# Vandermode/TFPnP

Hardware: AMD Instinct MI355X
Metric: PnP-ADMM iters/sec (and images/sec) at env_batch=48, 256x256, 30 inner iters (higher is better)
Workload: dtype f32 (v_mfma_f32_32x32x2_f32; Winograd F(2x2,3x3) on the layers with cout % 32 == 0); 1 GPU; CS-MRI ADMM 256x256 env_batch=48/GPU radial x4 sigma_n=15, 6 solver calls x 5 inner iters + PSNR reward, no early stop; global_batch=48, parallelism=single GPU

## Files before the change

### tfpnp_amd/csrc/api.hip

```cpp
#include <cstring>

#include "common.h"
#include "conv3x3.h"
#include "conv_hs.h"

namespace pnpx {

static thread_local std::string g_err;

void set_error(const char* fmt, ...) {
  char buf[1024];
  va_list ap;
  va_start(ap, fmt);
  vsnprintf(buf, sizeof(buf), fmt, ap);
  va_end(ap);
  g_err = buf;
}

int hip_fail(hipError_t e, const char* what, const char* file, int line) {
  set_error("HIP error %d (%s) at %s:%d in %s", (int)e, hipGetErrorString(e), file, line, what);
  return PNPX_ERR_HIP;
}

int ctx_scratch(pnpx_ctx* ctx, size_t bytes, void** out) {
  if (ctx->scratch.bytes < bytes) {
    PNPX_HIP(hipDeviceSynchronize());
    if (ctx->scratch.p) PNPX_HIP(hipFree(ctx->scratch.p));
    ctx->scratch = DeviceBuf();
    void* p = nullptr;
    hipError_t e = hipMalloc(&p, bytes);
    if (e != hipSuccess) {
      set_error("scratch allocation of %zu bytes failed: %s", bytes, hipGetErrorString(e));
      return PNPX_ERR_ALLOC;
    }
    ctx->scratch.p = p;
    ctx->scratch.bytes = bytes;
  }
  *out = ctx->scratch.p;
  return PNPX_OK;
}

struct LayerSpec {
  int cin, cout;
};
static void unet_layers(LayerSpec out[27]) {
  const int blocks[9][2] = {{2, 32},    {32, 64},   {64, 128}, {128, 256}, {256, 512},
                            {768, 256}, {384, 128}, {192, 64}, {96, 32}};
  for (int b = 0; b < 9; ++b)
    for (int j = 0; j < 3; ++j) out[3 * b + j] = LayerSpec{j == 0 ? blocks[b][0] : blocks[b][1], blocks[b][1]};
}

constexpr int DRUNET_MAX_SHIFT = 8;
static int drunet_rescale(pnpx_ctx* ctx) {
  PNPX_HIP(hipDeviceSynchronize());
  if (ctx->drunet.shift < DRUNET_MAX_SHIFT) ctx->drunet.shift += 4;
  else ctx->conv_mode = CONV_F32;
  *ctx->range_flag_host = 0;
  return PNPX_OK;
}

void range_guard_enter(pnpx_ctx* ctx) {
  if (!ctx->opt_range_guard || !ctx->range_flag_host) return;
  if (*static_cast<volatile unsigned*>(ctx->range_flag_host) == 0 || ctx->range_tripped) return;
  ctx->range_tripped = true;
  if (ctx->drunet.loaded && ctx->conv_mode == CONV_HS) {
    if (drunet_rescale(ctx) != PNPX_OK) ctx->conv_mode = CONV_F32;
  } else ctx->conv_mode = CONV_F32;
}

int range_guard_strict(pnpx_ctx* ctx, hipStream_t s, bool* rerun) {
  *rerun = false;
  PNPX_HIP(hipStreamSynchronize(s));
  if (*static_cast<volatile unsigned*>(ctx->range_flag_host) == 0) return PNPX_OK;
  if (ctx->conv_mode != CONV_HS || ctx->range_tripped) {
    set_error("half-split range guard: the call's result is invalid and no fallback is left (conv_mode %d)", ctx->conv_mode);
    return PNPX_ERR_RANGE;
  }
  if (ctx->drunet.loaded) PNPX_TRY(drunet_rescale(ctx));
  else {
    ctx->conv_mode = CONV_F32;
    *ctx->range_flag_host = 0;
  }
  *rerun = true;
  return PNPX_OK;
}

}

using namespace pnpx;

#define LOCK_CTX(ctx)                         \
  if (!(ctx)) {                               \
    pnpx::set_error("null context");          \
    return PNPX_ERR_ARG;                      \
  }                                           \
  std::lock_guard<std::mutex> _lk((ctx)->mu); \
  PNPX_HIP(hipSetDevice((ctx)->device))

extern "C" {

const char* pnpx_version(void) { return "pnpx 0.1 (gfx950)"; }
const char* pnpx_last_error(void) { return g_err.c_str(); }

int pnpx_ctx_create(int device, pnpx_ctx** out) {
  if (!out) {
    set_error("pnpx_ctx_create: null out");
    return PNPX_ERR_ARG;
  }
  int n = 0;
  PNPX_HIP(hipGetDeviceCount(&n));
  if (device < 0 || device >= n) {
    set_error("pnpx_ctx_create: device %d out of range (%d visible)", device, n);
    return PNPX_ERR_ARG;
  }
  PNPX_HIP(hipSetDevice(device));
  pnpx_ctx* c = new pnpx_ctx();
  c->device = device;
  void* h = nullptr;
  hipError_t e = hipHostMalloc(&h, 64, hipHostMallocMapped);
  if (e != hipSuccess) {
    delete c;
    return hip_fail(e, "hipHostMalloc(range flag)", __FILE__, __LINE__);
  }
  c->range_flag_host = static_cast<unsigned*>(h);
  *c->range_flag_host = 0;
  void* d = nullptr;
  e = hipHostGetDevicePointer(&d, h, 0);
  if (e != hipSuccess) {
    (void)hipHostFree(h);
    delete c;
    return hip_fail(e, "hipHostGetDevicePointer(range flag)", __FILE__, __LINE__);
  }
  c->range_flag_dev = static_cast<unsigned*>(d);
  *out = c;
  return PNPX_OK;
}

int pnpx_ctx_destroy(pnpx_ctx* ctx) {
  if (!ctx) return PNPX_OK;
  (void)hipSetDevice(ctx->device);
  (void)hipDeviceSynchronize();
  if (ctx->weights.p) (void)hipFree(ctx->weights.p);
  for (pnpx::UNetArena* a : {&ctx->arena, &ctx->arena_grad})
    if (a->buf.p) (void)hipFree(a->buf.p);
  policy_free(ctx);
  pnpx::critic_free(ctx);
  pnpx::drunet_free(ctx);
  pnpx::train_cache_free(ctx);
  if (ctx->scratch.p) (void)hipFree(ctx->scratch.p);
  for (auto& t : ctx->twiddle)
    if (t.second) (void)hipFree(t.second);
  for (auto e : ctx->events) (void)hipEventDestroy(e);
  if (ctx->range_flag_host) (void)hipHostFree(ctx->range_flag_host);
  for (hipStream_t st : ctx->side_streams) (void)hipStreamDestroy(st);
  for (hipEvent_t ev : ctx->ev_pool) (void)hipEventDestroy(ev);
  delete ctx;
  return PNPX_OK;
}

size_t pnpx_policy_num_params(int num_inputs, int n_det, int spi_head) {
  return policy_num_params(num_inputs, n_det, spi_head);
}

int pnpx_policy_load(pnpx_ctx* ctx, const float* params_host, size_t n_params, int num_inputs, int n_det,
                     int spi_head) {
  LOCK_CTX(ctx);
  return policy_load(ctx, params_host, n_params, num_inputs, n_det, spi_head);
}

int pnpx_policy_forward(pnpx_ctx* ctx, const float* ob, float* probs, float* det, int B, int H, int W,
                        void* stream) {
  LOCK_CTX(ctx);
  if (!ob || !probs || !det) {
    set_error("pnpx_policy_forward: null pointer");
    return PNPX_ERR_ARG;
  }
  return policy_forward(ctx, ob, probs, det, B, H, W, static_cast<hipStream_t>(stream));
}

size_t pnpx_critic_num_params(int num_inputs) {
  return (num_inputs >= 1 && num_inputs <= 64) ? critic_num_params(num_inputs) : 0;
}

int pnpx_critic_load(pnpx_ctx* ctx, const float* params_host, size_t n_params, int num_inputs) {
  LOCK_CTX(ctx);
  return critic_load(ctx, params_host, n_params, num_inputs);
}

int pnpx_critic_forward(pnpx_ctx* ctx, const float* ob, float* value, int B, int H, int W, void* stream) {
  LOCK_CTX(ctx);
  if (!ob || !value) {
    set_error("pnpx_critic_forward: null pointer");
    return PNPX_ERR_ARG;
  }
  return critic_forward(ctx, ob, value, B, H, W, static_cast<hipStream_t>(stream));
}

int pnpx_critic_backward(pnpx_ctx* ctx, const float* ob, const float* grad_value, float* grad_ob, int B, int H, int W,
                         void* stream) {
  LOCK_CTX(ctx);
  if (!ob || !grad_value || !grad_ob) {
    set_error("pnpx_critic_backward: null pointer");
    return PNPX_ERR_ARG;
  }
  return critic_backward(ctx, ob, grad_value, grad_ob, B, H, W, static_cast<hipStream_t>(stream));
}

int pnpx_ctx_reserve(pnpx_ctx* ctx, int B, int H, int W) {
  LOCK_CTX(ctx);
  if (B <= 0 || H < 16 || W < 16) {
    set_error("pnpx_ctx_reserve: need B > 0 and H, W >= 16");
    return PNPX_ERR_SHAPE;
  }
  return ctx_reserve_unet(ctx, B, H, W);
}

int pnpx_ctx_set_option(pnpx_ctx* ctx, const char* key, int value) {
  LOCK_CTX(ctx);
  auto is = [&](const char* k) { return key && !std::strcmp(key, k); };
  if (is("conv_mode") && (value == CONV_F32 || value == CONV_HS)) {
    ctx->conv_mode = value;
    return PNPX_OK;
  }
  if (is("drunet_shift") && value >= 0 && value <= 8 && (value & 3) == 0) {
    ctx->drunet.shift = value;
    return PNPX_OK;
  }
  if (is("subbatch") && value >= 0) {
    ctx->opt_subbatch = value;
    return PNPX_OK;
  }
  if (is("fuse_pool") && (value == 0 || value == 1)) {
    ctx->opt_fuse_pool = value;
    return PNPX_OK;
  }
  if (is("fuse_outc") && (value == 0 || value == 1)) {
    ctx->opt_fuse_outc = value;
    return PNPX_OK;
  }
  if (is("fuse_first") && (value == 0 || value == 1)) {
    ctx->opt_fuse_first = value;
    return PNPX_OK;
  }
  if (is("policy_s2_hs") && (value == 0 || value == 1)) {
    PNPX_HIP(hipDeviceSynchronize());
    ctx->opt_policy_s2_hs = value;
    ctx->policy.capB = ctx->policy.capH = ctx->policy.capW = 0;
    return PNPX_OK;
  }
  if (is("fold_first") && (value == 0 || value == 1)) {
    ctx->opt_fold_first = value;
    return PNPX_OK;
  }
  if (is("fft_tile") && value >= 0 && value <= 8192) {
    ctx->opt_fft_tile = value;
    return PNPX_OK;
  }
  if (is("fp32_winograd") && (value == 0 || value == 1)) {
    ctx->opt_fp32_winograd = value;
    return PNPX_OK;
  }
  if (is("fp32_chains") && value >= 0 && value <= 8) {
    ctx->opt_fp32_chains = value;
    return PNPX_OK;
  }
  if (is("fp32_fuse_up") && (value == 0 || value == 1)) {
    ctx->opt_fp32_fuse_up = value;
    return PNPX_OK;
  }
  if (is("fp32_ksplit") && value >= 0 && value <= 2) {
    ctx->opt_fp32_ksplit = value;
    return PNPX_OK;
  }
  if (is("fp32_ksplit_rule") && value >= 1 && value < 256) {
    ctx->opt_ksplit_rule = value;
    return PNPX_OK;
  }
  if (is("fp32_wino8_layers") && value >= 0 && value < (1 << 27)) {
    ctx->opt_fp32_wino8 = value;
    return PNPX_OK;
  }
  if (is("fft_fast") && (value == 0 || value == 1)) {
    ctx->opt_fft_fast = value;
    return PNPX_OK;
  }
  if (is("fft_affine") && (value == 0 || value == 1)) {
    ctx->opt_fft_affine = value;
    return PNPX_OK;
  }
  if (is("chains") && value >= 0 && value <= 8) {
    ctx->opt_chains = value;
    return PNPX_OK;
  }
  if (is("wreg") && value >= 0 && value <= 2) {
    ctx->opt_wreg = value;
    return PNPX_OK;
  }
  if (is("fuse_up") && (value >= 0 && value <= 2)) {
    ctx->opt_fuse_up = value;
    return PNPX_OK;
  }
  if (is("range_guard") && value >= 0 && value <= 2) {
    PNPX_HIP(hipDeviceSynchronize());
    ctx->opt_range_guard = value;
    ctx->range_tripped = false;
    *ctx->range_flag_host = 0;
    return PNPX_OK;
  }
  if (is("train_cache_gb") && value >= -1) {
    ctx->opt_train_cache_gb = value;
    ctx->train_alloc_failed = false;
    ctx->train_budget_bytes = 0;
    if (value == 0) pnpx::train_cache_free(ctx);
    return PNPX_OK;
  }
  if (is("train_cache_release")) {
    pnpx::train_cache_free(ctx);
    ctx->train_alloc_failed = false;
    ctx->train_budget_bytes = 0;
    return PNPX_OK;
  }
  set_error("pnpx_ctx_set_option: unknown option '%s' or bad value %d", key ? key : "(null)", value);
  return PNPX_ERR_ARG;
}

int pnpx_ctx_get_option(pnpx_ctx* ctx, const char* key, int* value) {
  LOCK_CTX(ctx);
  auto is = [&](const char* k) { return key && !std::strcmp(key, k); };
  if (!value) {
    set_error("pnpx_ctx_get_option: null value pointer");
    return PNPX_ERR_ARG;
  }
  if (is("conv_mode")) *value = ctx->conv_mode;
  else if (is("drunet_shift")) *value = ctx->drunet.shift;
  else if (is("subbatch")) *value = ctx->opt_subbatch;
  else if (is("fuse_pool")) *value = ctx->opt_fuse_pool;
  else if (is("fuse_outc")) *value = ctx->opt_fuse_outc;
  else if (is("fuse_first")) *value = ctx->opt_fuse_first;
  else if (is("fuse_up")) *value = ctx->opt_fuse_up;
  else if (is("wreg")) *value = ctx->opt_wreg;
  else if (is("chains")) *value = ctx->opt_chains;
  else if (is("fold_first")) *value = ctx->opt_fold_first;
  else if (is("policy_s2_hs")) *value = ctx->opt_policy_s2_hs;
  else if (is("fft_affine")) *value = ctx->opt_fft_affine;
  else if (is("fft_fast")) *value = ctx->opt_fft_fast;
  else if (is("fp32_winograd")) *value = ctx->opt_fp32_winograd;
  else if (is("fp32_wino8_layers")) *value = ctx->opt_fp32_wino8;
  else if (is("fp32_fuse_up")) *value = ctx->opt_fp32_fuse_up;
  else if (is("fp32_ksplit")) *value = ctx->opt_fp32_ksplit;
  else if (is("fp32_ksplit_rule")) *value = ctx->opt_ksplit_rule;
  else if (is("fp32_chains")) *value = ctx->opt_fp32_chains;
  else if (is("fft_tile")) *value = ctx->opt_fft_tile;
  else if (is("range_guard")) *value = ctx->opt_range_guard;
  else if (is("train_cache_gb")) *value = ctx->opt_train_cache_gb;
  else {
    set_error("pnpx_ctx_get_option: unknown option '%s'", key ? key : "(null)");
    return PNPX_ERR_ARG;
  }
  return PNPX_OK;
}

int pnpx_ctx_status(pnpx_ctx* ctx) {
  LOCK_CTX(ctx);
  range_guard_enter(ctx);
  if (ctx->range_tripped) {
    if (ctx->drunet.loaded)
      set_error("half-split range guard tripped: an activation of an earlier DRUNet call left the f16 hi/lo range (|v| >= 4095 "
                "or NaN); that call's output is invalid.  The context now runs %s (the bias-free network is positively "
                "homogeneous: inputs scaled by 2^-%d, the tail multiplies back; a trip at 2^-8 selects exact fp32); acknowledge "
                "with pnpx_ctx_set_option(ctx, \"range_guard\", 1)", ctx->conv_mode == CONV_HS ? "re-scaled passes" : "conv_mode 0",
                ctx->drunet.shift);
    else
    set_error("half-split range guard tripped: an activation of an earlier call left the f16 hi/lo range (|v| >= 4095 or "
              "NaN); that call's output is invalid.  The context now runs conv_mode 0 (exact fp32 MFMA); re-arm with "
              "pnpx_ctx_set_option(ctx, \"range_guard\", 1)");
    return PNPX_ERR_RANGE;
  }
  return PNPX_OK;
}

size_t pnpx_ctx_bytes(const pnpx_ctx* ctx) {
  if (!ctx) return 0;
  size_t n = ctx->weights.bytes + ctx->arena.buf.bytes + ctx->arena_grad.buf.bytes + ctx->scratch.bytes +
             ctx->drunet.weights.bytes + ctx->drunet.arena.bytes + ctx->drunet.arena_grad.bytes + ctx->drunet.f32_weights.bytes +
             ctx->drunet.f32_arena.bytes + ctx->drunet.f32_weights_bwd.bytes + ctx->drunet.f32_arena_grad.bytes +
             ctx->policy.weights.bytes + ctx->policy.arena.bytes + ctx->critic.weights.bytes + ctx->critic.arena.bytes;
  for (const auto& sl : ctx->train_ring) n += sl.arena.buf.bytes + sl.pre.bytes;
  return n;
}

size_t pnpx_unet_num_params(void) {
  LayerSpec L[27];
  unet_layers(L);
  size_t n = 0;
  for (int i = 0; i < 27; ++i) n += (size_t)L[i].cin * L[i].cout * 9 + L[i].cout;
  return n + 32 + 1;
}

size_t pnpx_drunet_num_params(int nb) { return (nb >= 1 && nb <= 8) ? pnpx::drunet_num_params(nb) : 0; }

int pnpx_drunet_load(pnpx_ctx* ctx, const float* params_host, size_t n_params, int nb) {
  LOCK_CTX(ctx);
  return pnpx::drunet_load(ctx, params_host, n_params, nb);
}

int pnpx_unet_load(pnpx_ctx* ctx, const float* params_host, size_t n_params) {
  LOCK_CTX(ctx);
  pnpx::drunet_free(ctx);
  if (!params_host || n_params != pnpx_unet_num_params()) {
    set_error("pnpx_unet_load: expected %zu parameters, got %zu", pnpx_unet_num_params(), n_params);
    return PNPX_ERR_ARG;
  }
  LayerSpec L[27];
  unet_layers(L);
  std::vector<float> host;
  size_t woff[27], boff[27];
  auto align = [&]() { host.resize((host.size() + 255) & ~(size_t)255, 0.f); };
  const float* src = params_host;
  for (int i = 0; i < 27; ++i) {
    const int mt = conv_pack_mt(L[i].cout), cc = conv_pack_cc(L[i].cin);
    align();
    woff[i] = host.size();
    host.resize(host.size() + (size_t)L[i].cin * L[i].cout * 9);
    pack_conv_weights(src, L[i].cout, L[i].cin, mt, cc, host.data() + woff[i]);
    src += (size_t)L[i].cin * L[i].cout * 9;
    align();
    boff[i] = host.size();
    host.insert(host.end(), src, src + L[i].cout);
    src += L[i].cout;
    ctx->conv[i].cin = L[i].cin;
    ctx->conv[i].cout = L[i].cout;
    ctx->conv[i].mt = mt;
    ctx->conv[i].cc = cc;
  }
  size_t uoff[27];
  {
    const float* wsrc = params_host;
    for (int i = 0; i < 27; ++i) {
      uoff[i] = 0;
      if (conv3x3_wino_packs(L[i].cout, L[i].cin)) {
        align();
        uoff[i] = host.size();
        host.resize(host.size() + conv3x3_wino_floats(L[i].cout, L[i].cin));
        pack_conv_weights_wino(wsrc, L[i].cout, L[i].cin, host.data() + uoff[i]);
      }
      wsrc += (size_t)L[i].cin * L[i].cout * 9 + L[i].cout;
    }
  }
  size_t hoff[27];
  float hscale[27];
  for (int i = 0; i < 27; ++i) {
    const int mt = conv_hs_mt(L[i].cout);
    const int cin_pad = (L[i].cin + 15) / 16 * 16;
    align();
    hoff[i] = host.size();
    const size_t n16 = (size_t)L[i].cout * cin_pad * 9 * 2;
    host.resize(host.size() + (n16 + 1) / 2, 0.f);
    const float* wsrc = params_host;
    for (int k = 0; k < i; ++k) wsrc += (size_t)L[k].cin * L[k].cout * 9 + L[k].cout;
    hscale[i] = pack_conv_weights_hs(wsrc, L[i].cout, L[i].cin, mt, reinterpret_cast<uint16_t*>(host.data() + hoff[i]));
    ctx->conv_hs[i].cin = L[i].cin;
    ctx->conv_hs[i].cout = L[i].cout;
    ctx->conv_hs[i].cin_pad = cin_pad;
    ctx->conv_hs[i].mt = mt;
    ctx->conv_hs[i].inv_scale = 1.0f / (hscale[i] * HS_ASCALE);
  }
  size_t toff[27];
  for (int i = 0; i < 27; ++i) {
    const int cout_pad = (L[i].cin + 31) / 32 * 32;
    const int mt = (cout_pad % 64 == 0) ? 64 : 32;
    align();
    toff[i] = host.size();
    host.resize(host.size() + (size_t)cout_pad * L[i].cout * 9);
    const float* wsrc = params_host;
    for (int k = 0; k < i; ++k) wsrc += (size_t)L[k].cin * L[k].cout * 9 + L[k].cout;
    pack_conv_weights_transposed(wsrc, L[i].cout, L[i].cin, cout_pad, mt, 8, host.data() + toff[i]);
    ctx->conv_bwd[i].cin = L[i].cout;
    ctx->conv_bwd[i].cout = cout_pad;
    ctx->conv_bwd[i].mt = mt;
    ctx->conv_bwd[i].cc = 8;
  }
  size_t thoff[27], tuoff[27];
  float thscale[27];
  {
    std::vector<float> wt;
    for (int i = 0; i < 27; ++i) {
      const int cin_t = L[i].cout;
      const int cout_t = (L[i].cin + 31) / 32 * 32;
      const int mt = (cout_t % 64 == 0) ? 64 : 32;
      const float* wsrc = params_host;
      for (int k = 0; k < i; ++k) wsrc += (size_t)L[k].cin * L[k].cout * 9 + L[k].cout;
      wt.assign((size_t)cout_t * cin_t * 9, 0.f);
      for (int ci = 0; ci < L[i].cin; ++ci)
        for (int co = 0; co < cin_t; ++co)
          for (int tap = 0; tap < 9; ++tap)
            wt[((size_t)ci * cin_t + co) * 9 + tap] = wsrc[((size_t)co * L[i].cin + ci) * 9 + (8 - tap)];
      align();
      thoff[i] = host.size();
      const size_t n16 = (size_t)cout_t * cin_t * 9 * 2;
      host.resize(host.size() + (n16 + 1) / 2, 0.f);
      thscale[i] = pack_conv_weights_hs(wt.data(), cout_t, cin_t, mt, reinterpret_cast<uint16_t*>(host.data() + thoff[i]));
      tuoff[i] = 0;
      if (conv3x3_wino_packs(cout_t, cin_t)) {
        align();
        tuoff[i] = host.size();
        host.resize(host.size() + conv3x3_wino_floats(cout_t, cin_t));
        pack_conv_weights_wino(wt.data(), cout_t, cin_t, host.data() + tuoff[i]);
      }
      ctx->conv_hs_bwd[i].cin = cin_t;
      ctx->conv_hs_bwd[i].cout = cout_t;
      ctx->conv_hs_bwd[i].cin_pad = cin_t;
      ctx->conv_hs_bwd[i].mt = mt;
      ctx->conv_hs_bwd[i].inv_scale = 1.0f / (thscale[i] * HS_ASCALE);
    }
  }
  align();
  const size_t oc0 = host.size();
  host.insert(host.end(), params_host, params_host + 32 * 2 * 9);
  align();
  const size_t ozero = host.size();
  host.resize(host.size() + 768, 0.f);
  align();
  const size_t ow = host.size();
  host.insert(host.end(), src, src + 32);
  src += 32;
  align();
  const size_t ob = host.size();
  host.push_back(*src);
  host.resize(host.size() + 1024, 0.f);
  PNPX_HIP(hipDeviceSynchronize());
  if (ctx->weights.p) PNPX_HIP(hipFree(ctx->weights.p));
  ctx->weights = DeviceBuf();
  ctx->has_weights = false;
  void* p = nullptr;
  hipError_t e = hipMalloc(&p, host.size() * sizeof(float));
  if (e != hipSuccess) {
    set_error("weight allocation of %zu bytes failed: %s", host.size() * sizeof(float), hipGetErrorString(e));
    return PNPX_ERR_ALLOC;
  }
  PNPX_HIP(hipMemcpy(p, host.data(), host.size() * sizeof(float), hipMemcpyHostToDevice));
  float* d = static_cast<float*>(p);
  for (int i = 0; i < 27; ++i) {
    ctx->conv[i].w = d + woff[i];
    ctx->conv[i].b = d + boff[i];
    ctx->conv_wino_u[i] = uoff[i] ? d + uoff[i] : nullptr;
    ctx->conv_wino_u_bwd[i] = tuoff[i] ? d + tuoff[i] : nullptr;
    ctx->conv_hs[i].w = reinterpret_cast<char*>(d + hoff[i]);
    ctx->conv_bwd[i].w = d + toff[i];
    ctx->conv_bwd[i].b = nullptr;
    ctx->conv_hs_bwd[i].w = reinterpret_cast<char*>(d + thoff[i]);
  }
  ctx->conv0_w = d + oc0;
  ctx->zero_bias = d + ozero;
  ctx->outc_w = d + ow;
  ctx->outc_b = d + ob;
  ctx->weights.p = p;
  ctx->weights.bytes = host.size() * sizeof(float);
  ctx->has_weights = true;
  pnpx::train_cache_free(ctx);
  return PNPX_OK;
}

int pnpx_unet_denoise(pnpx_ctx* ctx, const float* x, const float* sigma, float* out, float* out_preclamp, int B,
                      int H, int W, void* stream) {
  LOCK_CTX(ctx);
  return pnpx::guarded(ctx, static_cast<hipStream_t>(stream), [&]() -> int {
  if (!x || !sigma || !out) {
    set_error("pnpx_unet_denoise: null pointer");
    return PNPX_ERR_ARG;
  }
  return unet_denoise(ctx, x, sigma, 1, out, out_preclamp, B, H, W, static_cast<hipStream_t>(stream), nullptr);
  });
}

int pnpx_unet_denoise_backward(pnpx_ctx* ctx, const float* x, const float* sigma, const float* grad_out, float* grad_x,
                               float* grad_sigma, int B, int H, int W, void* stream) {
  LOCK_CTX(ctx);
  return pnpx::guarded(ctx, static_cast<hipStream_t>(stream), [&]() -> int {
  if (!x || !sigma || !grad_out || !grad_x || !grad_sigma) {
    set_error("pnpx_unet_denoise_backward: null pointer");
    return PNPX_ERR_ARG;
  }
  return unet_denoise_backward(ctx, x, sigma, 1, grad_out, grad_x, grad_sigma, B, H, W, static_cast<hipStream_t>(stream));
  });
}

int pnpx_unet_denoise_train(pnpx_ctx* ctx, const float* x, const float* sigma, float* out, int B, int H, int W,
                            unsigned long long* ticket, void* stream) {
  LOCK_CTX(ctx);
  return pnpx::guarded(ctx, static_cast<hipStream_t>(stream), [&]() -> int {
    if (!x || !sigma || !out || !ticket) {
      set_error("pnpx_unet_denoise_train: null pointer");
      return PNPX_ERR_ARG;
    }
    return unet_denoise_train(ctx, x, sigma, 1, out, B, H, W, static_cast<hipStream_t>(stream), ticket);
  });
}

int pnpx_unet_denoise_backward_ticket(pnpx_ctx* ctx, const float* x, const float* sigma, const float* grad_out,
                                      float* grad_x, float* grad_sigma, int B, int H, int W, unsigned long long ticket,
                                      void* stream) {
  LOCK_CTX(ctx);
  return pnpx::guarded(ctx, static_cast<hipStream_t>(stream), [&]() -> int {
    if (!x || !sigma || !grad_out || !grad_x || !grad_sigma) {
      set_error("pnpx_unet_denoise_backward_ticket: null pointer");
      return PNPX_ERR_ARG;
    }
    return unet_denoise_backward_ticket(ctx, x, sigma, 1, grad_out, grad_x, grad_sigma, B, H, W,
                                        static_cast<hipStream_t>(stream), ticket);
  });
}

int pnpx_unet_profile(pnpx_ctx* ctx, const float* x, const float* sigma, float* out, int B, int H, int W,
                      void* stream, int cap, float* ms_out, double* flops_out, const char** names_out, int* n_out) {
  LOCK_CTX(ctx);
  if (!x || !sigma || !out || !ms_out || !flops_out || !names_out || !n_out || cap <= 0) {
    set_error("pnpx_unet_profile: null pointer");
    return PNPX_ERR_ARG;
  }
  hipStream_t s = static_cast<hipStream_t>(stream);
  PNPX_TRY(unet_denoise(ctx, x, sigma, 1, out, nullptr, B, H, W, s, nullptr));
  while (ctx->events.size() < 1024) {
    hipEvent_t e;
    PNPX_HIP(hipEventCreate(&e));
    ctx->events.push_back(e);
  }
  ProfileSink sink;
  sink.events = &ctx->events;
  PNPX_TRY(unet_denoise(ctx, x, sigma, 1, out, nullptr, B, H, W, s, &sink));
  PNPX_HIP(hipStreamSynchronize(s));
  int n = sink.n < cap ? sink.n : cap;
  for (int i = 0; i < n; ++i) {
    float ms = 0.f;
    PNPX_HIP(hipEventElapsedTime(&ms, ctx->events[i], ctx->events[i + 1]));
    ms_out[i] = ms;
    flops_out[i] = sink.flops[i];
    names_out[i] = sink.names[i];
  }
  *n_out = n;
  return PNPX_OK;
}

int pnpx_fft2(pnpx_ctx* ctx, const float* in, float* out, int n_img, int H, int W, int inverse, int centered,
              void* stream) {
  LOCK_CTX(ctx);
  if (!in || !out) {
    set_error("pnpx_fft2: null pointer");
    return PNPX_ERR_ARG;
  }
  return fft2(ctx, in, out, n_img, H, W, inverse != 0, centered != 0, static_cast<hipStream_t>(stream));
}
// ... 3 lines not shown
```

### tfpnp_amd/csrc/common.h

```cpp
#pragma once
#include <hip/hip_runtime.h>

#include <cstdarg>
#include <cstdint>
#include <cstdio>
#include <map>
#include <mutex>
#include <string>
#include <vector>

#include "pnpx.h"

namespace pnpx {

void set_error(const char* fmt, ...);
int hip_fail(hipError_t e, const char* what, const char* file, int line);

#define PNPX_HIP(expr)                                                       \
  do {                                                                       \
    hipError_t _e = (expr);                                                  \
    if (_e != hipSuccess) return ::pnpx::hip_fail(_e, #expr, __FILE__, __LINE__); \
  } while (0)
#define PNPX_TRY(expr)          \
  do {                          \
    int _s = (expr);            \
    if (_s != PNPX_OK) return _s; \
  } while (0)
#define PNPX_LAUNCH_CHECK() PNPX_HIP(hipGetLastError())

constexpr int PADL = 4;
__host__ __device__ inline int padded_w(int W) { return W + 2 * PADL; }
__host__ __device__ inline int padded_h(int H) { return H + 2; }

struct ActDesc {
  size_t off = 0;
  int C = 0, H = 0, W = 0;
  size_t per_image() const { return (size_t)C * padded_h(H) * padded_w(W); }
};

struct ConvLayer {
  int cin = 0, cout = 0;
  int mt = 0, cc = 0;
  float* w = nullptr;
  float* b = nullptr;
};

struct DeviceBuf {
  void* p = nullptr;
  size_t bytes = 0;
};

struct UNetArena {
  DeviceBuf buf;
  int capB = 0, capH = 0, capW = 0, mode = -1;
};

struct ConvLayerHsDev {
  int cin = 0, cout = 0, cin_pad = 0, mt = 0;
  char* w = nullptr;
  float inv_scale = 1.f;
};

enum ConvMode { CONV_F32 = 0, CONV_HS = 1 };

struct PolStep;
struct PolicyConv {
  const float* w = nullptr;
  const float* bias = nullptr;
  const PolStep* steps = nullptr;
  const int* nsteps = nullptr;
  int cin = 0;
  int cout = 0;
  int split_c = 0;
};
struct PolicyNet {
  bool loaded = false;
  int num_inputs = 0, cin_pad = 0, n_det = 0, spi_head = 0;
  PolicyConv conv[17];
  ConvLayerHsDev conv_hs[12];
  const float* bias_hs[12] = {};
  ConvLayerHsDev s2_hs[4][2];
  const float* s2_bias[4][2] = {};
  ConvLayerHsDev stem_hs;
  const float* stem_hs_bias = nullptr;
  const float* fc_sm_w = nullptr;
  const float* fc_sm_b = nullptr;
  const float* fc_det_w = nullptr;
  const float* fc_det_b = nullptr;
  const float* fc_det2_w = nullptr;
  const float* fc_det2_b = nullptr;
  DeviceBuf weights;
  DeviceBuf arena;
  int capB = 0, capH = 0, capW = 0;
};

struct CriticNet {
  bool loaded = false;
  int num_inputs = 0, cin_pad = 0;
  ConvLayerHsDev fwd[21], bwd[21];
  const float* bias[21] = {};
  float alpha[21] = {};
  const float* fc_w = nullptr;
  const float* fc_b = nullptr;
  const float* zero = nullptr;
  float fc_wmax = 0.f;
  DeviceBuf weights, arena;
  int capB = 0, capH = 0, capW = 0;
};

int launch_chains(const pnpx_ctx* ctx, int B, int H, int W);
void join_side_streams_after_failure(pnpx_ctx* ctx);
struct DruNet {
  bool loaded = false;
  int nb = 0;
  std::vector<ConvLayerHsDev> layers;
  std::vector<int> taps;
  const float* head_w = nullptr;
  const float* zero = nullptr;
  const float* e0 = nullptr;
  int shift = 0;
  std::vector<ConvLayerHsDev> layers_bwd;
  const float* tail_bwd_w = nullptr;
  DeviceBuf weights, arena, arena_grad;
  std::vector<float> params_host;
  bool f32_ready = false;
  std::vector<ConvLayer> f32_layers;
  std::vector<const float*> f32_wino;
  DeviceBuf f32_weights, f32_arena;
  int f32_capB = 0, f32_capH = 0, f32_capW = 0;
  bool f32_arena_keeps = false;
  bool f32_bwd_ready = false;
  std::vector<ConvLayer> f32_layers_bwd;
  std::vector<const float*> f32_wino_bwd;
  DeviceBuf f32_weights_bwd, f32_arena_grad;
  int f32_gcapB = 0, f32_gcapH = 0, f32_gcapW = 0;
  int capB = 0, capH = 0, capW = 0;
  bool arena_keeps = false;
  int gcapB = 0, gcapH = 0, gcapW = 0;
};

}

struct pnpx_ctx {
  int device = 0;
  std::mutex mu;
  bool has_weights = false;
  pnpx::ConvLayer conv[27];
  pnpx::ConvLayerHsDev conv_hs[27];
  int conv_mode = pnpx::CONV_F32;
  int opt_subbatch = 24;
  int opt_fuse_pool = 1;
  int opt_fuse_outc = 1;
  int opt_fuse_first = 1;
  int opt_fuse_up = 1;
  int opt_policy_s2_hs = 1;
  int opt_fold_first = 0;
  int opt_fft_tile = 0;
  int opt_fft_fast = 1;
  int opt_fft_affine = 1;
  int opt_chains = 0;
  std::vector<hipStream_t> side_streams;
  std::vector<hipEvent_t> ev_pool;
  size_t ev_next = 0;
  int opt_wreg = 2;
  int opt_range_guard = 1;
  int opt_train_cache_gb = -1;
  size_t train_budget_bytes = 0;
  unsigned* range_flag_host = nullptr;
  unsigned* range_flag_dev = nullptr;
  bool range_tripped = false;
  float* conv_wino_u[27] = {};
  float* conv_wino_u_bwd[27] = {};
  int opt_fp32_winograd = 1;
  int opt_fp32_wino8 = (1 << 27) - 1;
  int opt_fp32_chains = 2;
  int opt_fp32_ksplit = 1;
  int opt_ksplit_rule = 1;
  int opt_fp32_fuse_up = 1;
  pnpx::ConvLayer conv_bwd[27];
  pnpx::ConvLayerHsDev conv_hs_bwd[27];
  float* zero_bias = nullptr;
  float* conv0_w = nullptr;
  float* outc_w = nullptr;
  float* outc_b = nullptr;
  pnpx::DeviceBuf weights;
  pnpx::UNetArena arena, arena_grad;
  struct TrainSlot {
    pnpx::UNetArena arena;
    pnpx::DeviceBuf pre;
    unsigned long long ticket = 0;
    int B = 0;
  };
  std::vector<TrainSlot> train_ring;
  unsigned long long train_counter = 0;
  int train_H = 0, train_W = 0, train_mode = -1;
  bool train_alloc_failed = false;
  pnpx::PolicyNet policy;
  pnpx::CriticNet critic;
  pnpx::DruNet drunet;
  pnpx::DeviceBuf scratch;
  std::map<int, float2*> twiddle;
  std::vector<hipEvent_t> events;
};

namespace pnpx {

int chain_event(pnpx_ctx* ctx, hipEvent_t* ev);
int chain_streams(pnpx_ctx* ctx, int chains);
template <class F>
int fan_out_chains(pnpx_ctx* ctx, int chains, int B, hipStream_t s, F&& run_slice) {
  PNPX_TRY(chain_streams(ctx, chains));
  hipEvent_t fork = nullptr, joins[16] = {};
  PNPX_TRY(chain_event(ctx, &fork));
  PNPX_HIP(hipEventRecord(fork, s));
  auto fail = [&](int rc) {
    join_side_streams_after_failure(ctx);
    return rc;
  };
  auto hip = [&](hipError_t e, const char* what) { return e == hipSuccess ? PNPX_OK : hip_fail(e, what, __FILE__, __LINE__); };
  for (int c = chains - 1; c >= 0; --c) {
    const int lo = (int)((long long)B * c / chains), hi = (int)((long long)B * (c + 1) / chains);
    hipStream_t st = c ? ctx->side_streams[c - 1] : s;
    int rc = c ? hip(hipStreamWaitEvent(st, fork, 0), "hipStreamWaitEvent(fork)") : PNPX_OK;
    if (rc == PNPX_OK) rc = run_slice(lo, hi, st);
    if (rc == PNPX_OK && c) rc = chain_event(ctx, &joins[c]);
    if (rc == PNPX_OK && c) rc = hip(hipEventRecord(joins[c], st), "hipEventRecord(join)");
    if (rc != PNPX_OK) return fail(rc);
  }
  for (int c = 1; c < chains; ++c) {
    const int rc = hip(hipStreamWaitEvent(s, joins[c], 0), "hipStreamWaitEvent(join)");
    if (rc != PNPX_OK) return fail(rc);
  }
  return PNPX_OK;
}

int ctx_reserve_unet(pnpx_ctx* ctx, int B, int H, int W);
int reserve_arena(pnpx_ctx* ctx, UNetArena& ar, int mode, int B, int H, int W, size_t extra_bytes);
int ctx_scratch(pnpx_ctx* ctx, size_t bytes, void** out);
int ctx_twiddle(pnpx_ctx* ctx, int N, const float2** out);
void range_guard_enter(pnpx_ctx* ctx);
int range_guard_strict(pnpx_ctx* ctx, hipStream_t s, bool* rerun);
template <class F>
int guarded(pnpx_ctx* ctx, hipStream_t s, F&& body) {
  range_guard_enter(ctx);
  int st = body();
  for (int attempt = 0; attempt < 4 && st == PNPX_OK && ctx->opt_range_guard == 2 && ctx->conv_mode == CONV_HS; ++attempt) {
    bool rerun = false;
    PNPX_TRY(range_guard_strict(ctx, s, &rerun));
    if (!rerun) break;
    st = body();
  }
  return st;
}

struct ProfileSink {
  std::vector<hipEvent_t>* events = nullptr;
  std::vector<const char*> names;
  std::vector<double> flops;
  int n = 0;
};

int unet_denoise(pnpx_ctx* ctx, const float* x, const float* sigma, int sigma_stride, float* out, float* out_pre,
                 int B, int H, int W, hipStream_t s, ProfileSink* prof, UNetArena* arena = nullptr, int mode = -1,
                 bool keep_all = false);
int unet_denoise_backward(pnpx_ctx* ctx, const float* x, const float* sigma, int sigma_stride, const float* grad_out,
                          float* grad_x, float* grad_sigma, int B, int H, int W, hipStream_t s,
                          UNetArena* cached = nullptr, const float* cached_pre = nullptr);
size_t unet_arena_bytes(int mode, int B, int H, int W);
void train_cache_free(pnpx_ctx* ctx);
int unet_denoise_train(pnpx_ctx* ctx, const float* x, const float* sigma, int sigma_stride, float* out, int B, int H,
                       int W, hipStream_t s, unsigned long long* ticket);
int unet_denoise_backward_ticket(pnpx_ctx* ctx, const float* x, const float* sigma, int sigma_stride,
                                 const float* grad_out, float* grad_x, float* grad_sigma, int B, int H, int W,
                                 hipStream_t s, unsigned long long ticket);

size_t drunet_num_params(int nb);
int drunet_load(pnpx_ctx* ctx, const float* params, size_t n, int nb);
int drunet_denoise(pnpx_ctx* ctx, const float* x, const float* sigma, int sigma_stride, float* out, float* out_pre, int B,
                   int H, int W, hipStream_t s, bool keep_mids = false);
int drunet_denoise_backward(pnpx_ctx* ctx, const float* x, const float* sigma, int sigma_stride, const float* grad_out,
                            float* grad_x, float* grad_sigma, int B, int H, int W, hipStream_t s);
void drunet_free(pnpx_ctx* ctx);
int drunet_denoise_f32(pnpx_ctx* ctx, const float* x, const float* sigma, int sigma_stride, float* out, float* out_pre, int B, int H,
                       int W, hipStream_t s, bool keep_mids = false);
int drunet_denoise_backward_f32(pnpx_ctx* ctx, const float* x, const float* sigma, int sigma_stride, const float* grad_out, float* grad_x,
                                float* grad_sigma, int B, int H, int W, hipStream_t s);
void drunet_f32_free(pnpx_ctx* ctx);

size_t policy_num_params(int num_inputs, int n_det, int spi_head);
int policy_load(pnpx_ctx* ctx, const float* params, size_t n, int num_inputs, int n_det, int spi_head);
int policy_forward(pnpx_ctx* ctx, const float* ob, float* probs, float* det, int B, int H, int W, hipStream_t s);
void policy_free(pnpx_ctx* ctx);

size_t critic_num_params(int num_inputs);
int critic_load(pnpx_ctx* ctx, const float* params, size_t n, int num_inputs);
int critic_forward(pnpx_ctx* ctx, const float* ob, float* value, int B, int H, int W, hipStream_t s);
int critic_backward(pnpx_ctx* ctx, const float* ob, const float* grad_value, float* grad_ob, int B, int H, int W, hipStream_t s);
void critic_free(pnpx_ctx* ctx);

int fft2(pnpx_ctx* ctx, const float* in, float* out, int n_img, int H, int W, bool inverse, bool centered,
         hipStream_t s);

}
```

### tfpnp_amd/csrc/conv3x3.h

```cpp
#pragma once
#include "common.h"

namespace pnpx {

struct ConvArgs {
  const float* in0;
  const float* in1;
  const float* wpk;
  const float* bias;
  float* out;
  int C0, C1;
  int H, W, Hp, Wp;
  int tilesX, tilesY, nct;
  float slope;
  int mode;
  const float* dmask;
  const char* dmask_hs = nullptr;
  const float* res = nullptr;
};

int conv_pack_mt(int cout);
int conv_pack_cc(int cin);
void pack_conv_weights(const float* w, int cout, int cin, int mt, int cc, float* dst);
int launch_conv3x3(const ConvLayer& L, const float* in0, int C0, const float* in1, int C1, float* out, int B,
                   int H, int W, hipStream_t s);
int launch_conv3x3_act(const ConvLayer& L, const float* in0, int C0, const float* in1, int C1, float* out, int B,
                       int H, int W, float slope, const float* res, hipStream_t s);
int launch_conv1x1_act(const ConvLayer& L, const float* in0, float* out, int B, int H, int W, float slope, const float* res, hipStream_t s);
void pack_conv_weights_1x1(const float* w, int cout, int cin, float* dst);
int launch_conv3x3_grad(const ConvLayer& L, const float* gin, float* gout, const float* dmask, int B, int H, int W,
                        hipStream_t s, const char* dmask_hs = nullptr, float mask_slope = 0.2f);
bool conv3x3_wino_ok(int C0, int C1, int cout, int H, int W);
bool conv3x3_wino_packs(int cout, int cin);
size_t conv3x3_wino_floats(int cout, int cin);
void pack_conv_weights_wino(const float* w, int cout, int cin, float* dst);
int launch_conv3x3_wino(const float* u, const float* bias, int cout, const float* in0, int C0, const float* in1, int C1,
                        float* out, int B, int H, int W, hipStream_t s, float slope = 0.2f, const float* res = nullptr,
                        float* pool_out = nullptr);
bool conv3x3_wino_outc_ok(int cin, int cout, int H, int W);
int launch_conv3x3_wino_outc(const float* u, const float* bias, const float* in0, int cin, const float* outc_w, const float* outc_b,
                             const float* x_img, float* img, float* img_pre, int B, int H, int W, hipStream_t s);
bool conv3x3_wino8_ok(int C0, int C1, int cout, int H, int W);
int launch_conv3x3_wino8(const float* u, const float* bias, int cout, const float* in0, int C0, const float* in1, int C1,
                         float* out, int B, int H, int W, hipStream_t s, float slope = 0.2f, const float* res = nullptr,
                         float* pool_out = nullptr, float* ks_part = nullptr, int ks_rule = 1);
int conv3x3_wino8_ksplit(int C0, int C1, int cout, int H, int W, int rule = 1);
size_t conv3x3_wino8_ksplit_bytes_per_image();
int launch_conv3x3_wino8_grad(const float* u, const float* zero_bias, int cout, const float* gin, int cin, float* gout, const float* dmask,
                              float mask_slope, int B, int H, int W, hipStream_t s);
bool conv3x3_wino8_ups_ok(int C0, int C1, int cout, int H, int W);
int launch_conv3x3_wino8_ups(const float* u, const float* bias, int cout, const float* in0, int C0, const float* in1_lowres, int C1,
                             float* out, int B, int H, int W, hipStream_t s, float slope = 0.2f);
int launch_conv3x3_wino8_outc(const float* u, const float* bias, const float* in0, int cin, const float* outc_w, const float* outc_b,
                              const float* x_img, float* img, float* img_pre, int B, int H, int W, hipStream_t s);
void pack_conv_weights_transposed(const float* w, int cout, int cin, int cout_pad, int mt, int cc, float* dst);

}
```

### tfpnp_amd/csrc/conv3x3_wino8.hip

```cpp
#include <cmath>
#include <utility>
#include <vector>

#include "common.h"
#include "conv3x3.h"
#include "wino_common.h"

namespace pnpx {

namespace {

using namespace wino;

template <int CT_>
struct Cfg8 {
  static constexpr int CT = CT_;
  static constexpr int CK = (CT == 64) ? 16 : 8;
  static constexpr int HALVES = CK / 8;
  static constexpr int KS = CK / 2;
  static constexpr int RS = (CT == 64) ? 1 : 2;
  static constexpr int NSTG = 4 / RS;
  static constexpr int NPOS = 2 * RS;
  static constexpr int NM = NPOS * KS;
  static_assert(NM == 16, "the side-work schedule below is written for 16 MFMA slots per stage");
  static constexpr int RPXW = (CT == 64) ? 16 : 32;
  static constexpr int TX = RPXW / 2, NT = 8 * TX;
  static constexpr int RW = RPXW + 2, RPX = 18 * RW;
  static constexpr int RPXL = (CT == 64) ? 328 : RPX;
  static constexpr int RAW_ELEMS = CK * RPXL;
  static constexpr int RAW_INSTR = (RAW_ELEMS + 63) / 64;
  static constexpr int RAW_BYTES = RAW_INSTR * 256;
  static constexpr int RAW_PER_WAVE = (RAW_INSTR + 7) / 8;
  static constexpr int NRAW = RAW_INSTR / 8;
  static constexpr int UQ = 16 * CK * CT;
  static constexpr int USTG = RS * UQ;
  static constexpr int NUW = USTG / 8192;
  static constexpr int VROW = 16384;
  static constexpr int VSTG = RS * VROW;
  static constexpr int OFF_U = 0, OFF_V = 4 * USTG, OFF_RAW = OFF_V + 2 * VSTG;
  static constexpr int LDS_USED = OFF_RAW + 2 * RAW_BYTES;
  static constexpr int BAR = 12;
  static constexpr int NR = 11, NQP = (CT == 64) ? 12 : 20;
  static constexpr int QPLANE = NR * NQP * 16;
  static constexpr int ST_ELEMS = CK * NR * NQP;
  static constexpr int ST_INSTR = (ST_ELEMS + 63) / 64;
  static constexpr int ST_STRIDE = ST_INSTR * 256;
  static constexpr int ST_PER_WAVE = (ST_INSTR + 7) / 8, NSW = ST_INSTR / 8;
  static constexpr int OFF_ST = LDS_USED, OFF_TAB = OFF_ST + 2 * ST_STRIDE;
  static constexpr int LDS_USED_UPS = OFF_TAB + (18 + RW) * 16;
  static constexpr int NPOSI = 18 * RW;
};
constexpr int LDS_REQ8 = 160 * 1024;

#define WINO8_ACC \
  "a0", "a1", "a2", "a3", "a4", "a5", "a6", "a7", "a8", "a9", "a10", "a11", "a12", "a13", "a14", "a15", "a16", "a17", \
  "a18", "a19", "a20", "a21", "a22", "a23", "a24", "a25", "a26", "a27", "a28", "a29", "a30", "a31", "a32", "a33", \
  "a34", "a35", "a36", "a37", "a38", "a39", "a40", "a41", "a42", "a43", "a44", "a45", "a46", "a47", "a48", "a49", \
  "a50", "a51", "a52", "a53", "a54", "a55", "a56", "a57", "a58", "a59", "a60", "a61", "a62", "a63", "a64", "a65", \
  "a66", "a67", "a68", "a69", "a70", "a71", "a72", "a73", "a74", "a75", "a76", "a77", "a78", "a79", "a80", "a81", \
  "a82", "a83", "a84", "a85", "a86", "a87", "a88", "a89", "a90", "a91", "a92", "a93", "a94", "a95", "a96", "a97", \
  "a98", "a99", "a100", "a101", "a102", "a103", "a104", "a105", "a106", "a107", "a108", "a109", "a110", "a111", "a112", \
  "a113", "a114", "a115", "a116", "a117", "a118", "a119", "a120", "a121", "a122", "a123", "a124", "a125", "a126", "a127"
#ifdef WINO8_PRIO
#define WINO8_PRIO_UP "s_setprio 3\n\t"
#define WINO8_PRIO_DOWN "\n\ts_setprio 0"
#else
#define WINO8_PRIO_UP
#define WINO8_PRIO_DOWN
#endif
#define WINO8_MFMA(IDX, x, y) \
  asm volatile(WINO8_PRIO_UP "v_mfma_f32_32x32x2_f32 a[%2:%3], %0, %1, a[%2:%3]" WINO8_PRIO_DOWN ::"v"(x), "v"(y), "n"(16 * (IDX)), "n"(16 * (IDX) + 15) : WINO8_ACC)
#define WINO8_MFMA_FROM_ZERO(IDX, x, y) \
  asm volatile(WINO8_PRIO_UP "v_mfma_f32_32x32x2_f32 a[%2:%3], %0, %1, 0" WINO8_PRIO_DOWN ::"v"(x), "v"(y), "n"(16 * (IDX)), "n"(16 * (IDX) + 15) : WINO8_ACC)

#ifndef WINO8_ABL
#define WINO8_ABL 0
#endif
#ifdef WINO8_TRACE
__device__ unsigned long long wino8_trace_buf[2][2048];
__device__ __forceinline__ void wino8_stamp(int wave, int lane, int& n, int tag) {
  if (blockIdx.x == 0 && (wave & 3) == 0 && n < 2047) {
    const unsigned long long t = __builtin_readcyclecounter();
    if (lane == 0) wino8_trace_buf[wave >> 2][n] = (t << 8) | (unsigned)tag;
    n = __builtin_amdgcn_readfirstlane(n + 1);
    if (lane == 0) wino8_trace_buf[wave >> 2][2047] = n;
  }
}
#define WINO8_STAMP(tag) wino8_stamp(wave, lane, trace_n, tag)
#else
#define WINO8_STAMP(tag)
#endif

template <bool RAWDMA_, bool STDMA_, int IQ_>
struct StageKind {
  static constexpr bool RAWDMA = RAWDMA_, STDMA = STDMA_;
  static constexpr int IQ = IQ_;
};

using I0 = std::integral_constant<int, 0>;
using I1 = std::integral_constant<int, 1>;
using I2 = std::integral_constant<int, 2>;
using I3 = std::integral_constant<int, 3>;
using Yes = std::true_type;
using No = std::false_type;

template <int CT, bool FUSE_OUTC, bool RES, bool UPS, bool KSPLIT>
__global__ __launch_bounds__(512, 1) void conv3x3_wino8_f32_kernel(WinoArgs a) {
  static_assert(!FUSE_OUTC || CT == 32, "the fused out-conv needs all 32 couts of a pixel in one SIMD's wave pair");
  static_assert(!UPS || (!FUSE_OUTC && !RES), "the up-sampling instances are the UNet's plain decoder entries");
  static_assert(!KSPLIT || (CT == 64 && !FUSE_OUTC && !RES && !UPS), "K-split: the plain 64-cout instance (the deep levels' layers)");
  using C = Cfg8<CT>;
  constexpr int CK = C::CK, HALVES = C::HALVES, KS = C::KS, RS = C::RS, NSTG = C::NSTG, NPOS = C::NPOS;
  constexpr int TX = C::TX, NT = C::NT, RW = C::RW, RPX = C::RPX, RPXL = C::RPXL;
  constexpr int RAW_BYTES = C::RAW_BYTES, RAW_PER_WAVE = C::RAW_PER_WAVE;
  constexpr int UQ = C::UQ, USTG = C::USTG, NUW = C::NUW, VROW = C::VROW, VSTG = C::VSTG;
  constexpr int OFF_U = C::OFF_U, OFF_V = C::OFF_V, OFF_RAW = C::OFF_RAW, BAR = C::BAR;
  extern __shared__ __attribute__((aligned(16))) char lds[];
  const int tid = threadIdx.x, lane = tid & 63;
  const int wave = __builtin_amdgcn_readfirstlane(tid >> 6);
#ifdef WINO8_TRACE
  int trace_n = 0;
#endif
  const int sw = wave & 3;
  const int HpWp = a.Hp * a.Wp;
  const unsigned lds0 = (unsigned)(size_t)(lptr_t)lds;
  const int nregions = a.rx * a.ry * a.B;
  const int nx = (gridDim.x % 8 == 0 && nregions >= 32) ? 8 : 1;
  const int xcd = blockIdx.x % nx, slot = blockIdx.x / nx, nslot = gridDim.x / nx;

  struct Tile {
    int ct, b, x0, y0;
    const float* s0;
    const float* s1;
    const float* w;
    const float* s1u;
    int ok, rlo;
    int clo, c0;
    int item, g;
  };
  const int hpwp_lo = UPS ? (a.ups_h + 2) * (a.ups_w + 2 * PADL) : 0;
  auto decode = [&](int k) {
    Tile T;
    const int j = slot + nslot * k;
    const int vnct = KSPLIT ? a.nct * a.ksplit : a.nct;
    const int q = j / vnct;
    const int v = j - q * vnct;
    T.g = KSPLIT ? v / a.nct : 0;
    T.ct = KSPLIT ? v - T.g * a.nct : v;
    T.c0 = KSPLIT ? T.g * a.nch : 0;
    const int reg = nx * q + xcd;
    T.ok = reg < nregions;
    T.item = reg * a.nct + T.ct;
    T.rlo = T.clo = 0;
    T.s1u = nullptr;
    const int t1 = reg / a.rx;
    const int tx = reg - t1 * a.rx;
    const int t2 = t1 / a.ry;
    const int ty = t1 - t2 * a.ry;
    T.b = t2;
    T.x0 = tx * C::RPXW;
    T.y0 = ty * 16;
    const size_t pix = (size_t)T.y0 * a.Wp + T.x0 + (PADL - 1);
    T.s0 = a.in0 + (size_t)T.b * a.C0 * HpWp + pix;
    T.s1 = a.in1 + ((long long)T.b * a.C1 - a.C0) * (long long)HpWp + (long long)pix;
    T.w = a.u + ((size_t)T.ct * (KSPLIT ? a.nch_all : a.nch) + T.c0) * 4 * (UQ / 4);
    if (UPS) {
      const int ya = T.y0 > 0 ? T.y0 - 1 : 0, xa = T.x0 > 0 ? T.x0 - 1 : 0;
      const int rl = (int)(a.ups_sy * (float)ya), cl = (int)(a.ups_sx * (float)xa);
      const int rmax = a.ups_h + 1 - C::NR, cmax = a.ups_w + PADL - C::NQP;
      T.rlo = rl < rmax ? rl : rmax;
      T.clo = cl < cmax ? cl : cmax;
      T.s1u = a.in1 + ((long long)T.b * a.C1 - a.C0) * (long long)hpwp_lo + (long long)(T.rlo + 1) * (a.ups_w + 2 * PADL) + T.clo + PADL;
    }
    return T;
  };
  auto raw_of = [&](const Tile& X, int c) {
    const int ca = KSPLIT ? c + X.c0 : c;
    return ((CK * ca < a.C0) ? X.s0 : X.s1) + (size_t)CK * ca * HpWp;
  };

  const int wm = (CT == 64) ? (sw & 1) : 0, wn = (CT == 64) ? (sw >> 1) : sw;
  const int l31 = lane & 31, kg = lane >> 5;
  const int a_lane = ((kg * HALVES) * CT + wm * 32 + l31) * 16;
  const int b_lane = ((kg * HALVES) * NT + wn * 32 + l31) * 16;
  asm volatile("" ::: WINO8_ACC);

  auto wait_lds = [&]() { asm volatile("s_waitcnt lgkmcnt(0)" ::: "memory"); };
  auto barrier = [&]() { __builtin_amdgcn_s_barrier(); };
  auto sync_all = [&]() {
    asm volatile("s_waitcnt vmcnt(0) lgkmcnt(0)" ::: "memory");
    __builtin_amdgcn_s_barrier();
  };

  auto body = [&](auto role_tag) {
    constexpr int P = decltype(role_tag)::value;

    unsigned roff[RAW_PER_WAVE];
#pragma unroll
    for (int k = 0; k < RAW_PER_WAVE; ++k) {
      const int idx = (wave + 8 * k) * 64 + lane;
      const int c = idx / RPXL, r = idx - c * RPXL;
      const int hy = r / RW, hx = r - hy * RW;
      roff[k] = (c < CK && r < RPX) ? 4u * (unsigned)(c * HpWp + hy * a.Wp + hx) : 0u;
    }
    const unsigned uoff = lane * 16u;
    auto dma_u = [&](const float* src, int uslot) {
      if (WINO8_ABL & 4) return;
      const float* s = src + wave * 256;
#pragma unroll
      for (int k = 0; k < NUW; ++k) glds16(s + k * 2048, uoff, lds0 + OFF_U + uslot * USTG + (wave + 8 * k) * 1024);
    };
    auto dma_raw = [&](const float* src, int rbuf, int k0, int k1) {
      if (WINO8_ABL & 4) return;
      const unsigned dst = lds0 + OFF_RAW + rbuf * RAW_BYTES + wave * 256;
#pragma unroll
      for (int k = k0; k < k1; ++k)
        if (k < RAW_PER_WAVE) {
          if (k < C::NRAW || wave + 8 * k < C::RAW_INSTR) glds4(src, roff[k], dst + k * 2048);
        }
    };

    constexpr int NR = C::NR, NQP = C::NQP, QPLANE = C::QPLANE, ST_STRIDE = C::ST_STRIDE, SPW = C::ST_PER_WAVE;
    constexpr int OFF_ST = C::OFF_ST, OFF_TAB = C::OFF_TAB, NPOSI = C::NPOSI;
    unsigned soff[UPS ? SPW : 1];
    if (UPS) {
      const int wp_lo = a.ups_w + 2 * PADL;
#pragma unroll
      for (int k = 0; k < SPW; ++k) {
        const int idx = (wave + 8 * k) * 64 + lane;
        const int e = idx & 3, g = idx >> 2;
        const int q = g % NQP, g2 = g / NQP;
        const int rr = g2 % NR, Q = g2 / NR;
        soff[k] = (Q < CK / 4) ? 4u * (unsigned)((4 * Q + e) * hpwp_lo + rr * wp_lo + q) : 0u;
      }
    }
    auto dma_st = [&](const float* src, int sbuf) {
      if (!UPS || (WINO8_ABL & 4)) return;
      const unsigned dst = lds0 + OFF_ST + sbuf * ST_STRIDE + wave * 256;
#pragma unroll
      for (int k = 0; k < SPW; ++k)
        if (k < C::NSW || wave + 8 * k < C::ST_INSTR) glds4(src, soff[UPS ? k : 0], dst + k * 2048);
    };
    auto write_tables = [&](const Tile& X) {
      if (!UPS) return;
      if (tid < 18 + RW) {
        const bool row = tid < 18;
        const int i = row ? tid : tid - 18;
        const int g = (row ? X.y0 : X.x0) - 1 + i;
        const bool valid = g >= 0 && g < (row ? a.H : a.W);
        const float f = (row ? a.ups_sy : a.ups_sx) * (float)g;
        const int i0 = (int)f;
        const float l = f - (float)i0, h = 1.f - l;
        const int off = row ? (i0 - X.rlo) * NQP * 16 : (i0 - X.clo) * 16;
        f32x4 ent;
        ent[0] = __int_as_float(valid ? off : 0);
        ent[1] = valid ? h : 0.f;
        ent[2] = valid ? l : 0.f;
        ent[3] = 0.f;
        *reinterpret_cast<f32x4*>(lds + OFF_TAB + tid * 16) = ent;
      }
    };
    struct Ip {
      float hy, ly, hx, lx;
      int base;
      f32x4 v00, v01, v10, v11;
    };
    const int ipos = tid < NPOSI ? tid : NPOSI - 1;
    const int ipos_b = (512 + (tid >> 2) < NPOSI) ? 512 + (tid >> 2) : NPOSI - 1;
    auto interp_tables = [&](int pp, Ip& ip) {
      const int hyi = pp / RW, hxi = pp - hyi * RW;
      const f32x4 rt = *reinterpret_cast<const f32x4*>(lds + OFF_TAB + hyi * 16);
      const f32x4 ct = *reinterpret_cast<const f32x4*>(lds + OFF_TAB + (18 + hxi) * 16);
      ip.hy = rt[1];
      ip.ly = rt[2];
      ip.hx = ct[1];
      ip.lx = ct[2];
      ip.base = __float_as_int(rt[0]) + __float_as_int(ct[0]);
    };
    auto interp_slice = [&](auto q_tag, int sl, Ip& ip, int sbuf, int rbuf) {
      constexpr int Q = decltype(q_tag)::value;
      if (sl == 0) {
        interp_tables(ipos, ip);
      } else if (sl == 1) {
        const char* b = lds + OFF_ST + sbuf * ST_STRIDE + Q * QPLANE + ip.base;
        ip.v00 = *reinterpret_cast<const f32x4*>(b);
        ip.v01 = *reinterpret_cast<const f32x4*>(b + 16);
        ip.v10 = *reinterpret_cast<const f32x4*>(b + NQP * 16);
        ip.v11 = *reinterpret_cast<const f32x4*>(b + NQP * 16 + 16);
      } else {
        const int e = sl - 2;
        const float o = ip.hy * (ip.hx * ip.v00[e] + ip.lx * ip.v01[e]) + ip.ly * (ip.hx * ip.v10[e] + ip.lx * ip.v11[e]);
        *reinterpret_cast<float*>(lds + OFF_RAW + rbuf * RAW_BYTES + ((4 * Q + e) * RPXL + ipos) * 4) = o;
      }
    };
    auto interp_mini = [&](auto q_tag, int sl, Ip& ip, int sbuf, int rbuf) {
      constexpr int Q = decltype(q_tag)::value;
      const int e4 = (tid & 3) * 4;
      if (sl == 0) {
        interp_tables(ipos_b, ip);
      } else if (sl == 1) {
        const char* b = lds + OFF_ST + sbuf * ST_STRIDE + Q * QPLANE + ip.base + e4;
        ip.v00[0] = *reinterpret_cast<const float*>(b);
        ip.v01[0] = *reinterpret_cast<const float*>(b + 16);
        ip.v10[0] = *reinterpret_cast<const float*>(b + NQP * 16);
        ip.v11[0] = *reinterpret_cast<const float*>(b + NQP * 16 + 16);
      } else {
        const float o = ip.hy * (ip.hx * ip.v00[0] + ip.lx * ip.v01[0]) + ip.ly * (ip.hx * ip.v10[0] + ip.lx * ip.v11[0]);
        *reinterpret_cast<float*>(lds + OFF_RAW + rbuf * RAW_BYTES + (4 * Q * RPXL + ipos_b) * 4 + e4 * RPXL) = o;
      }
    };

    constexpr int TCH = (CT == 64) ? 2 : 4;
    const int cb = (CT == 64) ? (lane & 1) : 0;
    const int tt = (CT == 64) ? ((wave >> 2) * 32 + (lane >> 1)) : ((sw & 1) * 64 + lane);
    const int tkg = (CT == 64) ? (sw & 1) : (sw >> 1), thf = (CT == 64) ? (sw >> 1) : 0;
    const int tty = tt / TX, ttx = tt % TX;
    const int t_rd = (((tkg * (CK / 2) + thf * 4 + 2 * cb) * RPXL) + (2 * tty) * RW + 2 * ttx) * 4;
    const int t_wr = (((tkg * HALVES + thf) * NT) + tt) * 16 + cb * 8;
    struct Tr {
      float d[2][TCH][4];
      float r[4][TCH];
    };
    constexpr int NSL = 3 * TCH;
    auto transform_slice = [&](auto ta_tag, int sl, Tr& t, int rbuf, int vdst) {
      constexpr int A = decltype(ta_tag)::value;
      constexpr int RA = (A == 0) ? 0 : (A == 2 ? 2 : 1);
      constexpr int RB = (A == 0) ? 2 : (A == 1 ? 2 : (A == 2 ? 1 : 3));
      if (sl < TCH) {
        const int e = sl;
        const char* rb = lds + OFF_RAW + rbuf * RAW_BYTES + t_rd;
#pragma unroll
        for (int x = 0; x < 4; x += 2) {
          const f32x2 da = *reinterpret_cast<const f32x2*>(rb + (e * RPXL + RA * RW + x) * 4);
          const f32x2 db = *reinterpret_cast<const f32x2*>(rb + (e * RPXL + RB * RW + x) * 4);
          t.d[0][e][x] = da[0];
          t.d[0][e][x + 1] = da[1];
          t.d[1][e][x] = db[0];
          t.d[1][e][x + 1] = db[1];
        }
      } else if (sl < 2 * TCH) {
        const int e = sl - TCH;
#pragma unroll
        for (int x = 0; x < 4; ++x)
          t.r[x][e] = (A == 1) ? t.d[0][e][x] + t.d[1][e][x] : t.d[0][e][x] - t.d[1][e][x];
      } else if (CT == 64) {
        const int bb = (sl - 2 * TCH) >> 1, e = (sl - 2 * TCH) & 1;
        (void)e;
        if (((sl - 2 * TCH) & 1) == 0) return;
        f32x2 v;
#pragma unroll
        for (int q = 0; q < 2; ++q)
          v[q] = (bb == 0) ? t.r[0][q] - t.r[2][q] : (bb == 1) ? t.r[1][q] + t.r[2][q] : (bb == 2) ? t.r[2][q] - t.r[1][q] : t.r[1][q] - t.r[3][q];
        *reinterpret_cast<f32x2*>(lds + vdst + t_wr + bb * 4096) = v;
      } else {
        const int bb = sl - 2 * TCH;
        f32x4 v;
#pragma unroll
        for (int e = 0; e < 4; ++e)
          v[e] = (bb == 0) ? t.r[0][e] - t.r[2][e] : (bb == 1) ? t.r[1][e] + t.r[2][e] : (bb == 2) ? t.r[2][e] - t.r[1][e] : t.r[1][e] - t.r[3][e];
        *reinterpret_cast<f32x4*>(lds + vdst + t_wr + bb * 4096) = v;
      }
    };
    constexpr int NSLT = (CT == 64) ? 2 * TCH + 8 : NSL;
    auto vdst_of = [&](auto sn_tag) {
      constexpr int SN = decltype(sn_tag)::value;
      return OFF_V + ((CT == 64) ? (SN & 1) * VSTG : SN * VSTG + P * VROW);
    };

    f32x4 af[NPOS][HALVES], bf[NPOS][HALVES];
    auto read_operand = [&](auto s_tag, int uslot, int pos, int h) {
      constexpr int S = decltype(s_tag)::value;
      constexpr int VB = (CT == 64) ? (S & 1) : S;
      const int r = pos >> 1, b = 2 * P + (pos & 1);
      if (WINO8_ABL & 2) {
        af[pos][h] = bf[pos][h] = (f32x4){1.f, 1.f, 1.f, 1.f};
        return;
      }
      af[pos][h] = *reinterpret_cast<const f32x4*>(lds + OFF_U + uslot * USTG + r * UQ + b * (UQ / 4) + a_lane + h * (CT * 16));
      bf[pos][h] = *reinterpret_cast<const f32x4*>(lds + OFF_V + VB * VSTG + r * VROW + b * 4096 + b_lane + h * (NT * 16));
    };

    struct Side {
      int t_rbuf;
      int u_cur, u_next;
      const float* u_src;
      int u_dst;
      const float* raw_src;
      int raw_buf;
      const float* st_src;
      int st_buf;
      int i_sbuf, i_rbuf;
    };
    auto stage = [&](auto s_tag, auto zero_tag, auto wait_tag, auto prefetch_tag, auto kind_tag, const Side& sd) {
      using K = decltype(kind_tag);
      constexpr int S = decltype(s_tag)::value;
      constexpr bool PREFETCH = decltype(prefetch_tag)::value;
      constexpr int SN = (S + 1) % NSTG;
      constexpr bool ZERO = decltype(zero_tag)::value;
      constexpr int WAITN = decltype(wait_tag)::value;
      constexpr bool HALOST = (CT == 64) ? (S == 0) : (S == 1);
      constexpr bool RAWST = HALOST && K::RAWDMA;
      constexpr bool STST = UPS && HALOST && K::STDMA;
      constexpr int IQ = UPS ? K::IQ : -1;
      using IQt = std::integral_constant<int, IQ < 0 ? 0 : IQ>;
      Ip ipa, ipb;
      auto islice = [&](int q) {
        if (IQ >= 0) interp_slice(IQt{}, q, ipa, sd.i_sbuf, sd.i_rbuf);
      };
      auto imini = [&](int q) {
        if (IQ >= 0 && CT == 32) interp_mini(IQt{}, q, ipb, sd.i_sbuf, sd.i_rbuf);
      };
      using TA = std::integral_constant<int, (CT == 64) ? SN : 2 * SN + P>;
      using SNt = std::integral_constant<int, SN>;
      Tr t;
      auto operand = [&](int pos, int h) { read_operand(s_tag, sd.u_cur, pos, h); };
      auto tslice = [&](int q) {
        if (!(WINO8_ABL & 1)) transform_slice(TA{}, q, t, sd.t_rbuf, vdst_of(SNt{}));
      };
      auto side = [&](int sl) {
        if (CT == 64) {
          if (sl == 0) operand(0, 1);
          else if (sl == 1) operand(1, 1);
          if (sl < 2) tslice(sl);
          if (sl == 2) dma_u(sd.u_src, sd.u_dst);
          if (RAWST && sl >= 3 && sl < 9) dma_raw(sd.raw_src, sd.raw_buf, 2 * (sl - 3), 2 * (sl - 3) + 2);
          if (STST && sl == 9) dma_st(sd.st_src, sd.st_buf);
          if (IQ < 0) {
            if (sl == 4) tslice(2);
            if (sl == 5) tslice(3);
            if (sl >= 6 && sl < 10) tslice(5 + 2 * (sl - 6));
          } else {
            if (sl == 3) tslice(2), tslice(3);
            if (sl == 4) tslice(5), tslice(7);
            if (sl == 5) tslice(9), tslice(11), islice(0);
            if (sl == 6) islice(1);
            if (sl >= 8 && sl < 12) islice(2 + (sl - 8));
          }
        } else {
          if (sl == 0) tslice(0);
          else if (sl == 1) operand(2, 0);
          else if (sl == 2) tslice(1);
          else if (sl == 3) operand(3, 0);
          else if (sl == 4) tslice(4), tslice(2);
          else if (sl == 5) tslice(5), tslice(3);
          else if (sl == 6) tslice(6), tslice(7);
          else if (sl == 7) tslice(8), tslice(9), islice(0);
          else if (sl == 8) tslice(10), tslice(11), islice(1);
          else if (sl == 9) islice(2), islice(3), imini(0);
          else if (sl == 10) islice(4), islice(5), imini(1), dma_u(sd.u_src, sd.u_dst);
          else if (sl == 11) imini(2);
          if (RAWST && sl >= 6 && sl < 11) dma_raw(sd.raw_src, sd.raw_buf, 2 * (sl - 6), 2 * (sl - 6) + 2);
          if (STST && sl == 9) dma_st(sd.st_src, sd.st_buf);
        }
        if (sl == BAR) {
          if (!(WINO8_ABL & 8)) {
            WINO8_STAMP(32 + S);
            asm volatile("s_waitcnt vmcnt(%0) lgkmcnt(0)" ::"n"(WAITN) : "memory");
            WINO8_STAMP(48 + S);
            barrier();
          }
          WINO8_STAMP(S);
          if (PREFETCH) {
            read_operand(SNt{}, sd.u_next, 0, 0);
            read_operand(SNt{}, sd.u_next, 1, 0);
          }
        }
      };
#pragma unroll
      for (int pair = 0; pair < NPOS / 2; ++pair)
#pragma unroll
        for (int m = 0; m < KS; ++m)
#pragma unroll
          for (int bl = 0; bl < 2; ++bl) {
            const int pos = 2 * pair + bl;
            const int sl = pair * (2 * KS) + m * 2 + bl;
            const float x = af[pos][m >> 2][m & 3], y = bf[pos][m >> 2][m & 3];
            const bool from_zero = ZERO && m == 0;
            if (!(WINO8_ABL & 16)) switch (pos) {
              case 0: if (from_zero) WINO8_MFMA_FROM_ZERO(2 * (RS * S) + 0, x, y); else WINO8_MFMA(2 * (RS * S) + 0, x, y); break;
              case 1: if (from_zero) WINO8_MFMA_FROM_ZERO(2 * (RS * S) + 1, x, y); else WINO8_MFMA(2 * (RS * S) + 1, x, y); break;
              case 2: if (from_zero) WINO8_MFMA_FROM_ZERO((2 * (RS * S) + 2) & 7, x, y); else WINO8_MFMA((2 * (RS * S) + 2) & 7, x, y); break;
              default: if (from_zero) WINO8_MFMA_FROM_ZERO((2 * (RS * S) + 3) & 7, x, y); else WINO8_MFMA((2 * (RS * S) + 3) & 7, x, y); break;
            }
            side(sl);
            __builtin_amdgcn_sched_barrier(0);
          }
    };

    auto epilogue = [&](const Tile& T, int xsend, int xrecv, int zoff) {
      const int tile = wn * 32 + l31, ty = tile / TX, tx = tile % TX;
      const int cbase = T.ct * CT + wm * 32 + 4 * kg;
      float* ob = a.out + ((size_t)T.b * a.Cout) * HpWp + (size_t)(T.y0 + 2 * ty + 1) * a.Wp + T.x0 + 2 * tx + PADL;
      const int Hp_pool = padded_h(a.H / 2), Wp_pool = padded_w(a.W / 2);
      const size_t HpWp_pool = (size_t)Hp_pool * Wp_pool;
      float* pb = a.pool ? a.pool + (size_t)T.b * a.Cout * HpWp_pool + (size_t)(T.y0 / 2 + ty + 1) * Wp_pool + T.x0 / 2 + tx + PADL : nullptr;
      constexpr int R0 = 8 * P;
      constexpr int RX = 8 - R0;
      WINO8_STAMP(16);
      asm volatile("s_nop 15\n\ts_nop 15" ::: "memory", WINO8_ACC);
      float bias_r[8];
#pragma unroll
      for (int j = 0; j < 8; ++j) bias_r[j] = a.bias[cbase + ((R0 + j) & 3) + 8 * ((R0 + j) >> 2)];
      auto column_sums = [&](auto r_tag) {
        constexpr int R = decltype(r_tag)::value;
        f32x4 sv;
        static_for<2>([&](auto bl_tag) {
          constexpr int BL = decltype(bl_tag)::value;
          float m0, m1, m2, m3;
          asm volatile("v_accvgpr_read_b32 %0, a[%1]" : "=v"(m0) : "n"(16 * (0 + BL) + R) : WINO8_ACC);
          asm volatile("v_accvgpr_read_b32 %0, a[%1]" : "=v"(m1) : "n"(16 * (2 + BL) + R) : WINO8_ACC);
          asm volatile("v_accvgpr_read_b32 %0, a[%1]" : "=v"(m2) : "n"(16 * (4 + BL) + R) : WINO8_ACC);
          asm volatile("v_accvgpr_read_b32 %0, a[%1]" : "=v"(m3) : "n"(16 * (6 + BL) + R) : WINO8_ACC);
          sv[BL] = (m0 + m1) + m2;
          sv[2 + BL] = (m1 - m2) - m3;
        });
        return sv;
      };
      f32x4 theirs[8];
      {
        char* xs = lds + xsend + lane * 16;
        static_for<8>([&](auto j_tag) {
          *reinterpret_cast<f32x4*>(xs + decltype(j_tag)::value * 1024) = column_sums(std::integral_constant<int, RX + decltype(j_tag)::value>{});
        });
        wait_lds();
        barrier();
        WINO8_STAMP(17);
        const char* xr = lds + xrecv + lane * 16;
#pragma unroll
        for (int j = 0; j < 8; ++j) theirs[j] = *reinterpret_cast<const f32x4*>(xr + j * 1024);
      }
      f32x2 rs0[RES ? 4 : 1], rs1[RES ? 4 : 1];
      auto load_res = [&](int j0) {
        const float* rb = a.res + (ob - a.out);
#pragma unroll
        for (int q = 0; q < 4; ++q) {
          const float* rp = rb + (size_t)(cbase + ((R0 + j0 + q) & 3) + 8 * ((R0 + j0 + q) >> 2)) * HpWp;
          rs0[RES ? q : 0] = *reinterpret_cast<const f32x2*>(rp);
          rs1[RES ? q : 0] = *reinterpret_cast<const f32x2*>(rp + a.Wp);
        }
      };
      float ow[8];
      float s00 = 0.f, s01 = 0.f, s10 = 0.f, s11 = 0.f;
      if (FUSE_OUTC) {
#pragma unroll
        for (int j = 0; j < 8; ++j) ow[j] = a.outc_w[cbase + ((R0 + j) & 3) + 8 * ((R0 + j) >> 2)];
      }
      wait_lds();
      float* const part_tile = KSPLIT ? a.part + ((size_t)T.item * a.ksplit * 8 + wave) * 2048 + lane * 4 : nullptr;
      float* const part_mine = KSPLIT ? part_tile + (size_t)T.g * (8 * 2048) : nullptr;
      static_for<8>([&](auto j_tag) {
        constexpr int j = decltype(j_tag)::value;
        constexpr int R = R0 + j;
        if (RES && (j & 3) == 0) load_res(j);
        const int co = cbase + (R & 3) + 8 * (R >> 2);
        const f32x4 mine = column_sums(std::integral_constant<int, R>{});
        const f32x4 lo = (P == 0) ? mine : theirs[j], hi = (P == 0) ? theirs[j] : mine;
        const float bias = bias_r[j];
        float y00 = (lo[0] + lo[1]) + hi[0], y01 = (lo[1] - hi[0]) - hi[1];
        float y10 = (lo[2] + lo[3]) + hi[2], y11 = (lo[3] - hi[2]) - hi[3];
        if (KSPLIT) {
          *reinterpret_cast<f32x4*>(part_mine + j * 256) = (f32x4){y00, y01, y10, y11};
          return;
        }
        y00 += bias;
        y01 += bias;
        y10 += bias;
        y11 += bias;
        y00 = fmaxf(y00, y00 * a.slope);
        y01 = fmaxf(y01, y01 * a.slope);
        y10 = fmaxf(y10, y10 * a.slope);
        y11 = fmaxf(y11, y11 * a.slope);
        if (RES) {
          const f32x2 r0 = rs0[RES ? (j & 3) : 0], r1 = rs1[RES ? (j & 3) : 0];
          if (a.res_mask) {
            y00 *= r0[0] > 0.f ? 1.f : a.mask_slope;
            y01 *= r0[1] > 0.f ? 1.f : a.mask_slope;
            y10 *= r1[0] > 0.f ? 1.f : a.mask_slope;
            y11 *= r1[1] > 0.f ? 1.f : a.mask_slope;
          } else {
            y00 += r0[0];
            y01 += r0[1];
            y10 += r1[0];
            y11 += r1[1];
          }
        }
        if (FUSE_OUTC) {
          s00 = fmaf(ow[j], y00, s00);
          s01 = fmaf(ow[j], y01, s01);
          s10 = fmaf(ow[j], y10, s10);
          s11 = fmaf(ow[j], y11, s11);
        } else {
          float* o = ob + (size_t)co * HpWp;
          *reinterpret_cast<f32x2*>(o) = (f32x2){y00, y01};
          *reinterpret_cast<f32x2*>(o + a.Wp) = (f32x2){y10, y11};
          if (a.pool) pb[(size_t)co * HpWp_pool] = fmaxf(fmaxf(y00, y01), fmaxf(y10, y11));
        }
      });
      WINO8_STAMP(19);
      if (FUSE_OUTC) {
        s00 += __shfl_xor(s00, 32);
        s01 += __shfl_xor(s01, 32);
        s10 += __shfl_xor(s10, 32);
        s11 += __shfl_xor(s11, 32);
        char* zb = lds + zoff + lane * 16;
        if (P == 1) {
          *reinterpret_cast<f32x4*>(zb) = (f32x4){s00, s01, s10, s11};
          wait_lds();
        }
        barrier();
        f32x4 o = {0.f, 0.f, 0.f, 0.f};
        if (P == 0) {
          o = *reinterpret_cast<const f32x4*>(zb);
          wait_lds();
        }
        barrier();
        if (P == 0) {
          s00 += o[0];
          s01 += o[1];
          s10 += o[2];
          s11 += o[3];
          const size_t px0 = ((size_t)T.b * a.H + T.y0 + 2 * ty) * a.W + T.x0 + 2 * tx;
          const float ob0 = a.outc_b[0];
          const f32x2 xi0 = *reinterpret_cast<const f32x2*>(a.x_img + px0), xi1 = *reinterpret_cast<const f32x2*>(a.x_img + px0 + a.W);
          const float v00 = xi0[0] + (s00 + ob0), v01 = xi0[1] + (s01 + ob0), v10 = xi1[0] + (s10 + ob0), v11 = xi1[1] + (s11 + ob0);
          *reinterpret_cast<f32x2*>(a.img_pre + px0) = (f32x2){v00, v01};
          *reinterpret_cast<f32x2*>(a.img_pre + px0 + a.W) = (f32x2){v10, v11};
          *reinterpret_cast<f32x2*>(a.img + px0) = (f32x2){fminf(fmaxf(v00, 0.f), 1.f), fminf(fmaxf(v01, 0.f), 1.f)};
          *reinterpret_cast<f32x2*>(a.img + px0 + a.W) = (f32x2){fminf(fmaxf(v10, 0.f), 1.f), fminf(fmaxf(v11, 0.f), 1.f)};
        }
      } else {
        barrier();
      }
      WINO8_STAMP(20);
    };

    constexpr int NST = KSPLIT ? 8 : (FUSE_OUTC ? (P == 0 ? 4 : 0) : 16);
    constexpr int NRAW = C::NRAW;

    int k = 0;
    Tile T = decode(0);
    if (!T.ok) return;
    WINO8_STAMP(14);
    if (CT == 64) {
      dma_raw(raw_of(T, 0), 0, 0, RAW_PER_WAVE);
      dma_u(T.w, 0);
      dma_u(T.w + (UQ / 4), 1);
      dma_u(T.w + 2 * (UQ / 4), 2);
    } else {
      dma_raw(T.s0, 0, 0, RAW_PER_WAVE);
      dma_raw(raw_of(T, 1), 1, 0, RAW_PER_WAVE);
      dma_u(T.w, 0);
      dma_u(T.w + (USTG / 4), 1);
      dma_u(T.w + 2 * (USTG / 4), 2);
    }
    sync_all();
    {
      Tr t;
#pragma unroll
      for (int sl = 0; sl < NSLT; ++sl) transform_slice(std::integral_constant<int, (CT == 64) ? 0 : P>{}, sl, t, 0, vdst_of(I0{}));
    }
    sync_all();
    WINO8_STAMP(15);
    read_operand(I0{}, 0, 0, 0);
    read_operand(I0{}, 0, 1, 0);

    auto chunk = [&](auto first_tag, auto k1_tag, auto k2_tag, auto k3_tag, const float* w_c, const float* nu, const float* nu2,
                     const float* nraw, const float* nst, int cc) {
      constexpr int EPI = decltype(first_tag)::value ? NST : 0;
      constexpr bool K1 = UPS && decltype(k1_tag)::value, K2 = UPS && decltype(k2_tag)::value, K3 = UPS && decltype(k3_tag)::value;
      constexpr int NSW = C::NSW;
      using Pre = Yes;
      const int rcur = cc & 1, rnext = rcur ^ 1;
      if constexpr (CT == 64) {
        using S0k = StageKind<!K1, K2, K1 ? 1 : -1>;
        using S1k = StageKind<false, false, K1 ? 2 : -1>;
        using S2k = StageKind<false, false, K1 ? 3 : -1>;
        using S3k = StageKind<false, false, K2 ? 0 : -1>;
        constexpr int HALO = (K1 ? 0 : NRAW) + (K2 ? NSW : 0);
        stage(I0{}, first_tag, std::integral_constant<int, NUW + EPI + NUW + HALO>{}, Yes{}, S0k{},
              Side{rcur, 0, 1, w_c + 3 * (UQ / 4), 3, nraw, rnext, nst, rcur, rnext, rnext});
        stage(I1{}, first_tag, std::integral_constant<int, EPI + NUW + HALO + NUW>{}, Yes{}, S1k{},
              Side{rcur, 1, 2, nu, 0, nullptr, 0, nullptr, 0, rnext, rnext});
        stage(I2{}, first_tag, std::integral_constant<int, 2 * NUW>{}, Yes{}, S2k{}, Side{rcur, 2, 3, nu + (UQ / 4), 1, nullptr, 0, nullptr, 0, rnext, rnext});
        stage(I3{}, first_tag, std::integral_constant<int, 2 * NUW>{}, Pre{}, S3k{}, Side{rnext, 3, 0, nu + 2 * (UQ / 4), 2, nullptr, 0, nullptr, 0, rcur, rcur});
      } else {
        using S0k = StageKind<false, false, K1 ? 1 : -1>;
        using S1k = StageKind<!K2, K3, K2 ? 0 : -1>;
        const int u0 = 2 * rcur, n0 = 2 * rnext;
        stage(I0{}, first_tag, std::integral_constant<int, NUW + EPI>{}, Yes{}, S0k{},
              Side{rcur, u0, u0 + 1, nu + (USTG / 4), n0 + 1, nullptr, 0, nullptr, 0, rnext, rnext});
        stage(I1{}, first_tag, std::integral_constant<int, 2 * NUW + EPI + (K2 ? 0 : NRAW) + (K3 ? NSW : 0)>{}, Pre{}, S1k{},
              Side{rnext, u0 + 1, n0, nu2, u0, nraw, rcur, nst, rnext, rcur, rcur});
      }
    };

    int cc = 0;
    for (;;) {
      Tile Tn = decode(k + 1);
      const bool more = Tn.ok;
      if (!more) Tn = T;
      for (int c = 0; c < a.nch; ++c, ++cc) {
        const float* w_c = T.w + (size_t)c * 4 * (UQ / 4);
        const float* nu = (c + 1 < a.nch) ? w_c + 4 * (UQ / 4) : Tn.w;
        const float* nu2 = (c + 2 < a.nch) ? w_c + 8 * (UQ / 4) : Tn.w + (size_t)(c + 2 - a.nch) * 4 * (UQ / 4);
        constexpr int AH = (CT == 64) ? 1 : 2;
        const float* nraw = (c + AH < a.nch) ? raw_of(T, c + AH) : raw_of(Tn, c + AH - a.nch);
        if constexpr (!UPS) {
          if (c == 0) chunk(Yes{}, No{}, No{}, No{}, w_c, nu, nu2, nraw, nullptr, cc);
          else chunk(No{}, No{}, No{}, No{}, w_c, nu, nu2, nraw, nullptr, cc);
        } else {
          const int cu = a.C0 / CK;
          auto ups = [&](int j) { return c + j < a.nch && c + j >= cu; };
          const bool k1 = ups(1), k2 = ups(2), k3 = (CT == 32) && ups(3);
          const float* nst = T.s1u + (size_t)CK * (c + AH + 1) * hpwp_lo;
          if (c == 0) {
            write_tables(T);
            chunk(Yes{}, No{}, No{}, No{}, w_c, nu, nu2, nraw, nst, cc);
          } else if constexpr (CT == 64) {
            if (!k1 && !k2) chunk(No{}, No{}, No{}, No{}, w_c, nu, nu2, nraw, nst, cc);
            else if (!k1 && k2) chunk(No{}, No{}, Yes{}, No{}, w_c, nu, nu2, nraw, nst, cc);
            else if (k1 && k2) chunk(No{}, Yes{}, Yes{}, No{}, w_c, nu, nu2, nraw, nst, cc);
            else chunk(No{}, Yes{}, No{}, No{}, w_c, nu, nu2, nraw, nst, cc);
          } else {
            if (!k1 && !k2 && !k3) chunk(No{}, No{}, No{}, No{}, w_c, nu, nu2, nraw, nst, cc);
            else if (!k1 && !k2) chunk(No{}, No{}, No{}, Yes{}, w_c, nu, nu2, nraw, nst, cc);
            else if (!k1 && k3) chunk(No{}, No{}, Yes{}, Yes{}, w_c, nu, nu2, nraw, nst, cc);
            else if (k1 && k2 && k3) chunk(No{}, Yes{}, Yes{}, Yes{}, w_c, nu, nu2, nraw, nst, cc);
            else if (k1 && k2) chunk(No{}, Yes{}, Yes{}, No{}, w_c, nu, nu2, nraw, nst, cc);
            else if (k1) chunk(No{}, Yes{}, No{}, No{}, w_c, nu, nu2, nraw, nst, cc);
            else chunk(No{}, No{}, Yes{}, No{}, w_c, nu, nu2, nraw, nst, cc);
          }
        }
      }
      const int rl = (cc - 1) & 1;
      const int bufA = (CT == 64) ? ((sw < 2) ? OFF_U + 3 * USTG + sw * 8192 : OFF_V + VSTG + (sw - 2) * 8192) : OFF_V + VSTG + sw * 8192;
      const int bufB = (CT == 64) ? ((sw < 2) ? OFF_RAW + rl * RAW_BYTES + sw * 8192 : C::LDS_USED + (sw - 2) * 8192)
                                  : ((sw < 1) ? OFF_U + (2 * rl + 1) * USTG : C::LDS_USED + (sw - 1) * 8192);
      static_assert(C::LDS_USED + (CT == 64 ? 2 : 3) * 8192 <= LDS_REQ8 && 2 * 8192 <= RAW_BYTES && USTG >= 8192, "exchange buffers");
      epilogue(T, P == 1 ? bufA : bufB, P == 1 ? bufB : bufA, bufB);
      if (!more) break;
      T = Tn;
      ++k;
    }
    sync_all();
  };

  if (wave < 4) body(I0{});
  else body(I1{});
}

__global__ __launch_bounds__(512) void wino8_ksplit_finish_kernel(WinoArgs a) {
  using C = Cfg8<64>;
  const int item = blockIdx.x, tid = threadIdx.x, lane = tid & 63, wave = tid >> 6;
  const int reg = item / a.nct, ct = item - reg * a.nct;
  const int t1 = reg / a.rx, txr = reg - t1 * a.rx, b = t1 / a.ry, tyr = t1 - b * a.ry;
  const int x0 = txr * C::RPXW, y0 = tyr * 16;
  const int P = wave >> 2, sw = wave & 3, wm = sw & 1, wn = sw >> 1, l31 = lane & 31, kg = lane >> 5;
  const int tile = wn * 32 + l31, ty = tile / C::TX, tx = tile % C::TX;
  const int cbase = ct * 64 + wm * 32 + 4 * kg;
  const size_t HpWp = (size_t)a.Hp * a.Wp;
  float* ob = a.out + ((size_t)b * a.Cout) * HpWp + (size_t)(y0 + 2 * ty + 1) * a.Wp + x0 + 2 * tx + PADL;
  const int Hp_pool = padded_h(a.H / 2), Wp_pool = padded_w(a.W / 2);
  const size_t HpWp_pool = (size_t)Hp_pool * Wp_pool;
  float* pb = a.pool ? a.pool + (size_t)b * a.Cout * HpWp_pool + (size_t)(y0 / 2 + ty + 1) * Wp_pool + x0 / 2 + tx + PADL : nullptr;
  const float* part = a.part + ((size_t)item * a.ksplit * 8 + wave) * 2048 + lane * 4;
#pragma unroll
  for (int j = 0; j < 8; ++j) {
    const int R = 8 * P + j;
    const int co = cbase + (R & 3) + 8 * (R >> 2);
    f32x4 y = *reinterpret_cast<const f32x4*>(part + j * 256);
    for (int g = 1; g < a.ksplit; ++g) {
      const f32x4 pg = *reinterpret_cast<const f32x4*>(part + (size_t)g * (8 * 2048) + j * 256);
      y[0] += pg[0];
      y[1] += pg[1];
      y[2] += pg[2];
      y[3] += pg[3];
    }
    const float bias = a.bias[co];
    float y00 = y[0] + bias, y01 = y[1] + bias, y10 = y[2] + bias, y11 = y[3] + bias;
    y00 = fmaxf(y00, y00 * a.slope);
    y01 = fmaxf(y01, y01 * a.slope);
    y10 = fmaxf(y10, y10 * a.slope);
    y11 = fmaxf(y11, y11 * a.slope);
    float* o = ob + (size_t)co * HpWp;
    *reinterpret_cast<f32x2*>(o) = (f32x2){y00, y01};
    *reinterpret_cast<f32x2*>(o + a.Wp) = (f32x2){y10, y11};
    if (a.pool) pb[(size_t)co * HpWp_pool] = fmaxf(fmaxf(y00, y01), fmaxf(y10, y11));
  }
}

}

static int wino8_ct(int C0, int C1, int cout, int H, int W) {
  if (C0 <= 0 || H < 16 || H % 16 != 0) return 0;
  if (cout % 64 == 0) return (C0 % 16 == 0 && C1 % 16 == 0 && W % 16 == 0) ? 64 : 0;
  if (cout % 32 == 0) return (C0 % 8 == 0 && C1 % 8 == 0 && W % 32 == 0 && C0 + C1 >= 16) ? 32 : 0;
  return 0;
}
bool conv3x3_wino8_ok(int C0, int C1, int cout, int H, int W) { return wino8_ct(C0, C1, cout, H, W) != 0; }

int conv3x3_wino8_ksplit(int C0, int C1, int cout, int H, int W, int rule) {
  if (wino8_ct(C0, C1, cout, H, W) != 64 || rule <= 0) return 1;
  const int t = (H / 16) * (W / 16) * (cout / 64), nch = (C0 + C1) / 16;
  const int g8 = rule == 1 ? 4 : (rule & 15), g16 = rule == 1 ? 2 : ((rule >> 4) & 15);
  int g = t <= 8 ? g8 : (t <= 16 ? g16 : 1);
  if (g != 1 && g != 2 && g != 4) g = 1;
  while (g > 1 && g * t > 32) g /= 2;
  while (g > 1 && (nch % g != 0 || nch / g < 4)) g /= 2;
  return g;
}
size_t conv3x3_wino8_ksplit_bytes_per_image() { return (size_t)32 * 8 * 2048 * sizeof(float); }

template <int CT, bool FUSE_OUTC, bool RES, bool UPS = false, bool KSPLIT = false>
static int launch_wino8(WinoArgs a, hipStream_t s) {
  using C = Cfg8<CT>;
  static_assert(C::LDS_USED <= LDS_REQ8 && C::LDS_USED_UPS <= LDS_REQ8, "LDS budget");
  a.nct = a.Cout / CT;
  a.nch = (a.C0 + a.C1) / C::CK;
  a.nch_all = a.nch;
  if (KSPLIT) a.nch /= a.ksplit;
  else a.ksplit = 1;
  a.rx = a.W / C::RPXW;
  a.ry = a.H / 16;
  static std::once_flag attr_once[64];
  int dev = 0;
  PNPX_HIP(hipGetDevice(&dev));
  if (dev >= 0 && dev < 64) {
    hipError_t e = hipSuccess;
    std::call_once(attr_once[dev], [&] {
      e = hipFuncSetAttribute(reinterpret_cast<const void*>(&conv3x3_wino8_f32_kernel<CT, FUSE_OUTC, RES, UPS, KSPLIT>), hipFuncAttributeMaxDynamicSharedMemorySize, LDS_REQ8);
    });
    PNPX_HIP(e);
  }
  const int vnct = a.nct * a.ksplit;
  const long long nreg = (long long)a.rx * a.ry * a.B, ntiles = nreg * vnct;
  long long grid = 256;
  if (grid >= ntiles) grid = ntiles;
  else if ((grid / 8) % vnct != 0 && grid >= 8LL * vnct) grid -= grid % (8 * vnct);
  hipLaunchKernelGGL((conv3x3_wino8_f32_kernel<CT, FUSE_OUTC, RES, UPS, KSPLIT>), dim3((unsigned)grid), dim3(512), LDS_REQ8, s, a);
  PNPX_LAUNCH_CHECK();
  if (KSPLIT) {
    hipLaunchKernelGGL(wino8_ksplit_finish_kernel, dim3((unsigned)(nreg * a.nct)), dim3(512), 0, s, a);
    PNPX_LAUNCH_CHECK();
  }
  return PNPX_OK;
}

int launch_conv3x3_wino8_outc(const float* u, const float* bias, const float* in0, int cin, const float* outc_w, const float* outc_b,
                              const float* x_img, float* img, float* img_pre, int B, int H, int W, hipStream_t s) {
  if (wino8_ct(cin, 0, 32, H, W) != 32) {
    set_error("conv3x3_wino8_outc: unsupported geometry (%d -> 32 channels, %d x %d)", cin, H, W);
    return PNPX_ERR_SHAPE;
  }
  WinoArgs a{};
  a.in0 = in0;
  a.in1 = in0;
  a.u = u;
  a.bias = bias;
  a.out = nullptr;
  a.outc_w = outc_w;
  a.outc_b = outc_b;
  a.x_img = x_img;
  a.img = img;
  a.img_pre = img_pre ? img_pre : img;
  a.B = B;
  a.H = H;
  a.W = W;
  a.Hp = padded_h(H);
  a.Wp = padded_w(W);
  a.C0 = cin;
  a.C1 = 0;
  a.Cout = 32;
  a.slope = 0.2f;
  return launch_wino8<32, true, false>(a, s);
}

bool conv3x3_wino8_ups_ok(int C0, int C1, int cout, int H, int W) {
  const int ct = wino8_ct(C0, C1, cout, H, W);
  if (!ct || C1 <= 0 || H % 2 || W % 2) return false;
  const int h = H / 2, w = W / 2;
  if (ct == 64) return C0 / 16 >= 3 && h + 1 >= Cfg8<64>::NR && w + PADL >= Cfg8<64>::NQP;
  return C0 / 8 >= 4 && h + 1 >= Cfg8<32>::NR && w + PADL >= Cfg8<32>::NQP;
}

int launch_conv3x3_wino8_ups(const float* u, const float* bias, int cout, const float* in0, int C0, const float* in1_lowres, int C1,
                             float* out, int B, int H, int W, hipStream_t s, float slope) {
  if (!conv3x3_wino8_ups_ok(C0, C1, cout, H, W)) {
    set_error("conv3x3_wino8_ups: unsupported geometry (%d + up(%d) -> %d channels, %d x %d)", C0, C1, cout, H, W);
    return PNPX_ERR_SHAPE;
  }
  WinoArgs a{};
  a.in0 = in0;
  a.in1 = in1_lowres;
  a.u = u;
  a.bias = bias;
  a.out = out;
  a.B = B;
  a.H = H;
  a.W = W;
  a.Hp = padded_h(H);
  a.Wp = padded_w(W);
  a.C0 = C0;
  a.C1 = C1;
  a.Cout = cout;
  a.slope = slope;
  a.ups_h = H / 2;
  a.ups_w = W / 2;
  a.ups_sy = (H > 1) ? (float)(H / 2 - 1) / (float)(H - 1) : 0.f;
  a.ups_sx = (W > 1) ? (float)(W / 2 - 1) / (float)(W - 1) : 0.f;
  return wino8_ct(C0, C1, cout, H, W) == 64 ? launch_wino8<64, false, false, true>(a, s) : launch_wino8<32, false, false, true>(a, s);
}

int launch_conv3x3_wino8_grad(const float* u, const float* zero_bias, int cout, const float* gin, int cin, float* gout, const float* dmask,
                              float mask_slope, int B, int H, int W, hipStream_t s) {
  const int ct = wino8_ct(cin, 0, cout, H, W);
  if (!ct) {
    set_error("conv3x3_wino8_grad: unsupported geometry (%d -> %d channels, %d x %d)", cin, cout, H, W);
    return PNPX_ERR_SHAPE;
  }
  WinoArgs a{};
  a.in0 = gin;
  a.in1 = gin;
  a.u = u;
  a.bias = zero_bias;
  a.res = dmask;
  a.res_mask = 1;
  a.mask_slope = mask_slope;
  a.out = gout;
  a.B = B;
  a.H = H;
  a.W = W;
  a.Hp = padded_h(H);
  a.Wp = padded_w(W);
  a.C0 = cin;
  a.C1 = 0;
  a.Cout = cout;
  a.slope = 1.0f;
  if (dmask) return ct == 64 ? launch_wino8<64, false, true>(a, s) : launch_wino8<32, false, true>(a, s);
  return ct == 64 ? launch_wino8<64, false, false>(a, s) : launch_wino8<32, false, false>(a, s);
}

int launch_conv3x3_wino8(const float* u, const float* bias, int cout, const float* in0, int C0, const float* in1, int C1,
                         float* out, int B, int H, int W, hipStream_t s, float slope, const float* res, float* pool_out, float* ks_part,
                         int ks_rule) {
  const int ct = wino8_ct(C0, C1, cout, H, W);
  if (!ct) {
    set_error("conv3x3_wino8: unsupported geometry (%d + %d -> %d channels, %d x %d)", C0, C1, cout, H, W);
    return PNPX_ERR_SHAPE;
  }
  WinoArgs a{};
  a.in0 = in0;
  a.in1 = in1 ? in1 : in0;
  a.u = u;
  a.bias = bias;
  a.res = res;
  a.pool = pool_out;
  a.out = out;
  a.B = B;
  a.H = H;
  a.W = W;
  a.Hp = padded_h(H);
  a.Wp = padded_w(W);
  a.C0 = C0;
  a.C1 = C1;
  a.Cout = cout;
  a.slope = slope;
  if (res) return ct == 64 ? launch_wino8<64, false, true>(a, s) : launch_wino8<32, false, true>(a, s);
  const int g = ks_part ? conv3x3_wino8_ksplit(C0, C1, cout, H, W, ks_rule) : 1;
  if (g > 1) {
    a.ksplit = g;
    a.part = ks_part;
    return launch_wino8<64, false, false, false, true>(a, s);
  }
  return ct == 64 ? launch_wino8<64, false, false>(a, s) : launch_wino8<32, false, false>(a, s);
}

}

#ifdef WINO8_TRACE
extern "C" int pnpx_debug_wino8_trace(unsigned long long* host_out) {
  return (int)hipMemcpyFromSymbol(host_out, HIP_SYMBOL(pnpx::wino8_trace_buf), sizeof(unsigned long long) * 2 * 2048);
}
#endif
```

### tfpnp_amd/csrc/drunet_f32.hip

```cpp
#include <cstring>
#include <vector>

#include "common.h"
#include "conv3x3.h"
#include "conv_first.h"
#include "grad_common.h"

namespace pnpx {

namespace {

constexpr int NC[4] = {64, 128, 256, 512};

inline dim3 g1(size_t n) { return dim3((unsigned)((n + 255) / 256)); }

__global__ void f32_prep_kernel(const float* __restrict__ x, const float* __restrict__ sigma, int sigma_stride, float* __restrict__ dst,
                                int H, int W, int Hp, int Wp) {
  const int b = blockIdx.z, y = blockIdx.y;
  const int xx = blockIdx.x * blockDim.x + threadIdx.x;
  if (xx >= W) return;
  float* d = dst + (size_t)b * 2 * Hp * Wp + (size_t)(y + 1) * Wp + xx + PADL;
  d[0] = x[((size_t)b * H + y) * W + xx];
  d[(size_t)Hp * Wp] = sigma[(size_t)b * sigma_stride];
}
// ... 59 lines not shown
  std::vector<LayerDesc> L;
  L.push_back({0, 2, NC[0]});
  auto res = [&](int c) {
    for (int i = 0; i < nb; ++i) {
      L.push_back({1, c, c});
      L.push_back({2, c, c});
    }
  };
  for (int l = 0; l < 3; ++l) {
    res(NC[l]);
    L.push_back({3, NC[l], NC[l + 1]});
  }
  res(NC[3]);
  for (int l = 2; l >= 0; --l) {
    L.push_back({4, NC[l + 1], NC[l]});
    res(NC[l]);
  }
  L.push_back({5, NC[0], 1});
  return L;
}

size_t plane(int C, int h, int w) { return (size_t)C * padded_h(h) * padded_w(w); }

struct Plan {
  size_t in2, S[4], P[4], Q[4], M[4], U[4], DT[4], T32, total;
  std::vector<size_t> MK[4];
};
Plan plan_of(int B, int H, int W, int nb_keep = 0) {
  Plan P{};
  size_t off = 0;
  auto add = [&](size_t& o, size_t floats_per_image) {
    o = off;
    off += floats_per_image * B;
    off = (off + 63) & ~(size_t)63;
  };
  add(P.in2, plane(2, H, W));
  for (int l = 0; l < 4; ++l) {
    const int h = H >> l, w = W >> l, c = NC[l];
    add(P.S[l], plane(c, h, w));
    add(P.P[l], plane(c, h, w));
    add(P.Q[l], plane(c, h, w));
    add(P.M[l], plane(c, h, w));
    if (l <= 2) add(P.U[l], plane(c, h, w));
    if (l >= 1) add(P.DT[l], plane(2 * c, h, w));
  }
  add(P.T32, plane(32, H, W));
  for (int l = 0; l < 4 && nb_keep > 0; ++l) {
    P.MK[l].resize(l == 3 ? nb_keep : 2 * nb_keep);
    for (size_t& o : P.MK[l]) add(o, plane(NC[l], H >> l, W >> l));
  }
  P.total = off + 4096;
  return P;
}

void layer_w3(const LayerDesc& d, const float* w, int* cin_o, int* cout_o, std::vector<float>& w3) {
  int cin = d.cin, cout = d.cout;
  if (d.kind == 3) {
    cin = 4 * d.cin;
    w3.assign((size_t)cout * cin * 9, 0.f);
    for (int co = 0; co < cout; ++co)
      for (int ci = 0; ci < d.cin; ++ci)
        for (int ph = 0; ph < 4; ++ph) w3[((size_t)co * cin + ph * d.cin + ci) * 9 + 4] = w[((size_t)co * d.cin + ci) * 4 + ph];
  } else if (d.kind == 4) {
    cout = 4 * d.cout;
    w3.assign((size_t)cout * cin * 9, 0.f);
    for (int ci = 0; ci < cin; ++ci)
      for (int co = 0; co < d.cout; ++co)
        for (int ph = 0; ph < 4; ++ph) w3[((size_t)(ph * d.cout + co) * cin + ci) * 9 + 4] = w[((size_t)ci * d.cout + co) * 4 + ph];
  } else if (d.kind == 5) {
    cout = 32;
    w3.assign((size_t)cout * cin * 9, 0.f);
    std::memcpy(w3.data(), w, sizeof(float) * (size_t)cin * 9);
  } else {
    w3.assign(w, w + (size_t)cout * cin * 9);
  }
  *cin_o = cin;
  *cout_o = cout;
}

int prepare_weights(pnpx_ctx* ctx) {
  DruNet& N = ctx->drunet;
  if (N.f32_ready) return PNPX_OK;
  const std::vector<LayerDesc> L = layers_of(N.nb);
  std::vector<float> host, w3;
  auto align = [&]() { host.resize((host.size() + 63) & ~(size_t)63, 0.f); };
  std::vector<size_t> woff(L.size()), uoff(L.size(), 0);
  std::vector<ConvLayer> lay(L.size());
  const float* src = N.params_host.data();
  for (size_t i = 0; i < L.size(); ++i) {
    const LayerDesc& d = L[i];
    const size_t np = (size_t)d.cin * d.cout * ((d.kind == 3 || d.kind == 4) ? 4 : 9);
    int cin, cout;
    layer_w3(d, src, &cin, &cout, w3);
    src += np;
    const int cc = conv_pack_cc(cin), mt = (cc == 2) ? 32 : conv_pack_mt(cout);
    align();
    woff[i] = host.size();
    if (d.kind == 3 || d.kind == 4) {
      std::vector<float> w1((size_t)cout * cin);
      for (size_t q = 0; q < w1.size(); ++q) w1[q] = w3[q * 9 + 4];
      host.resize(host.size() + w1.size());
      pack_conv_weights_1x1(w1.data(), cout, cin, host.data() + woff[i]);
    } else {
      host.resize(host.size() + (size_t)cout * cin * 9);
      pack_conv_weights(w3.data(), cout, cin, mt, cc, host.data() + woff[i]);
    }
    lay[i].cin = cin;
    lay[i].cout = cout;
    lay[i].mt = mt;
    lay[i].cc = cc;
    if ((d.kind == 1 || d.kind == 2) && conv3x3_wino_packs(cout, cin)) {
      align();
      uoff[i] = host.size();
      host.resize(host.size() + conv3x3_wino_floats(cout, cin));
      pack_conv_weights_wino(w3.data(), cout, cin, host.data() + uoff[i]);
    }
  }
  align();
  const size_t zoff = host.size();
  host.resize(host.size() + 1024 + 4096, 0.f);
  void* p = nullptr;
  hipError_t e = hipMalloc(&p, host.size() * sizeof(float));
  if (e != hipSuccess) {
    set_error("DRUNet fp32 weight allocation of %zu bytes failed: %s", host.size() * sizeof(float), hipGetErrorString(e));
    return PNPX_ERR_ALLOC;
  }
  PNPX_HIP(hipMemcpy(p, host.data(), host.size() * sizeof(float), hipMemcpyHostToDevice));
  float* d = static_cast<float*>(p);
  N.f32_wino.assign(L.size(), nullptr);
  for (size_t i = 0; i < L.size(); ++i) {
    lay[i].w = d + woff[i];
    lay[i].b = d + zoff;
    if (uoff[i]) N.f32_wino[i] = d + uoff[i];
  }
  N.f32_layers = lay;
  N.f32_weights.p = p;
  N.f32_weights.bytes = host.size() * sizeof(float);
  N.f32_ready = true;
  return PNPX_OK;
}

__global__ __launch_bounds__(256) void f32_tail_mask_kernel(const float* __restrict__ g_out, const float* __restrict__ pre, float* __restrict__ g_pre,
                                                            size_t n) {
  const size_t i = (size_t)blockIdx.x * blockDim.x + threadIdx.x;
  if (i >= n) return;
  const float p = pre[i];
  g_pre[i] = (p >= 0.f && p <= 1.f) ? g_out[i] : 0.f;
}
__global__ __launch_bounds__(256) void f32_input_grad_kernel(const float* __restrict__ g_in0, int Cg, float* __restrict__ gx,
                                                             float* __restrict__ part, int H, int W) {
  const int b = blockIdx.y, chunk = blockIdx.x;
  const int n = H * W, per = (n + SIG_CHUNKS - 1) / SIG_CHUNKS;
  const int lo = chunk * per, hi = min(n, lo + per);
  const int Hp = padded_h(H), Wp = padded_w(W);
  const float* g0 = g_in0 + (size_t)b * Cg * Hp * Wp;
  const float* g1c = g0 + (size_t)Hp * Wp;
  float acc = 0.f;
  for (int i = lo + threadIdx.x; i < hi; i += blockDim.x) {
    const int y = i / W, x = i - y * W;
    const size_t o = (size_t)(y + 1) * Wp + x + PADL;
    gx[(size_t)b * n + i] = g0[o];
    acc += g1c[o];
  }
  for (int off = 32; off > 0; off >>= 1) acc += __shfl_down(acc, off, 64);
  __shared__ float w[4];
  if ((threadIdx.x & 63) == 0) w[threadIdx.x >> 6] = acc;
  __syncthreads();
  if (threadIdx.x == 0) part[b * SIG_CHUNKS + chunk] = (w[0] + w[1]) + (w[2] + w[3]);
}

int prepare_weights_bwd(pnpx_ctx* ctx) {
  DruNet& N = ctx->drunet;
  if (N.f32_bwd_ready) return PNPX_OK;
  const std::vector<LayerDesc> L = layers_of(N.nb);
  std::vector<float> host, w3, wa;
  auto align = [&]() { host.resize((host.size() + 63) & ~(size_t)63, 0.f); };
  std::vector<size_t> woff(L.size(), 0), uoff(L.size(), 0);
  std::vector<ConvLayer> lay(L.size());
  const float* src = N.params_host.data();
  for (size_t i = 0; i < L.size(); ++i) {
    const LayerDesc& d = L[i];
    const size_t np = (size_t)d.cin * d.cout * ((d.kind == 3 || d.kind == 4) ? 4 : 9);
    int cin, cout;
    layer_w3(d, src, &cin, &cout, w3);
    src += np;
    if (d.kind == 5) continue;
    const int ca_in = cout, ca_out = (cin < 32) ? 32 : cin;
    wa.assign((size_t)ca_out * ca_in * 9, 0.f);
    for (int ci = 0; ci < cin; ++ci)
      for (int co = 0; co < cout; ++co)
        for (int tap = 0; tap < 9; ++tap) wa[((size_t)ci * ca_in + co) * 9 + tap] = w3[((size_t)co * cin + ci) * 9 + (8 - tap)];
    align();
    woff[i] = host.size();
    const int mt = conv_pack_mt(ca_out);
    if (d.kind == 3 || d.kind == 4) {
      std::vector<float> w1((size_t)ca_out * ca_in);
      for (size_t q = 0; q < w1.size(); ++q) w1[q] = wa[q * 9 + 4];
      host.resize(host.size() + w1.size());
      pack_conv_weights_1x1(w1.data(), ca_out, ca_in, host.data() + woff[i]);
    } else {
      host.resize(host.size() + (size_t)ca_out * ca_in * 9);
      pack_conv_weights(wa.data(), ca_out, ca_in, mt, 8, host.data() + woff[i]);
    }
    lay[i].cin = ca_in;
    lay[i].cout = ca_out;
    lay[i].mt = (d.kind == 3 || d.kind == 4) ? 64 : mt;
    lay[i].cc = 8;
    if ((d.kind == 1 || d.kind == 2) && conv3x3_wino_packs(ca_out, ca_in)) {
      align();
      uoff[i] = host.size();
      host.resize(host.size() + conv3x3_wino_floats(ca_out, ca_in));
      pack_conv_weights_wino(wa.data(), ca_out, ca_in, host.data() + uoff[i]);
    }
  }
  align();
  const size_t zoff = host.size();
  host.resize(host.size() + 1024 + 4096, 0.f);
  void* p = nullptr;
  hipError_t e = hipMalloc(&p, host.size() * sizeof(float));
  if (e != hipSuccess) {
    set_error("DRUNet fp32 adjoint-weight allocation of %zu bytes failed: %s", host.size() * sizeof(float), hipGetErrorString(e));
    return PNPX_ERR_ALLOC;
  }
  PNPX_HIP(hipMemcpy(p, host.data(), host.size() * sizeof(float), hipMemcpyHostToDevice));
  float* d = static_cast<float*>(p);
  N.f32_wino_bwd.assign(L.size(), nullptr);
  for (size_t i = 0; i < L.size(); ++i) {
    lay[i].w = d + woff[i];
    lay[i].b = d + zoff;
    if (uoff[i]) N.f32_wino_bwd[i] = d + uoff[i];
  }
  N.f32_layers_bwd = lay;
  N.f32_weights_bwd.p = p;
  N.f32_weights_bwd.bytes = host.size() * sizeof(float);
  N.f32_bwd_ready = true;
  return PNPX_OK;
}

}

void drunet_f32_free(pnpx_ctx* ctx) {
  DruNet& N = ctx->drunet;
  if (N.f32_weights.p) (void)hipFree(N.f32_weights.p);
  if (N.f32_arena.p) (void)hipFree(N.f32_arena.p);
  N.f32_weights = DeviceBuf();
  N.f32_arena = DeviceBuf();
  N.f32_ready = false;
  N.f32_capB = N.f32_capH = N.f32_capW = 0;
  N.f32_arena_keeps = false;
  if (N.f32_weights_bwd.p) (void)hipFree(N.f32_weights_bwd.p);
  if (N.f32_arena_grad.p) (void)hipFree(N.f32_arena_grad.p);
  N.f32_weights_bwd = DeviceBuf();
  N.f32_arena_grad = DeviceBuf();
  N.f32_bwd_ready = false;
  N.f32_gcapB = N.f32_gcapH = N.f32_gcapW = 0;
}

int drunet_denoise_f32(pnpx_ctx* ctx, const float* x, const float* sigma, int sigma_stride, float* out, float* out_pre, int B, int H,
                       int W, hipStream_t s, bool keep_mids) {
  DruNet& N = ctx->drunet;
  if (B <= 0 || H < 8 || W < 8 || (H & 7) || (W & 7)) {
    set_error("DRUNet: need B > 0 and H, W positive multiples of 8 (three 2x2 strided convolutions; got B=%d H=%d W=%d)", B, H, W);
    return PNPX_ERR_SHAPE;
  }
  PNPX_TRY(prepare_weights(ctx));
  if (B > N.f32_capB || H != N.f32_capH || W != N.f32_capW || (keep_mids && !N.f32_arena_keeps)) {
    const bool keeps = keep_mids;
    const int nb_img = (!keeps && H == N.f32_capH && W == N.f32_capW && N.f32_capB > B) ? N.f32_capB : B;
    const Plan Pl = plan_of(nb_img, H, W, keeps ? N.nb : 0);
    PNPX_HIP(hipDeviceSynchronize());
    if (N.f32_arena.bytes < Pl.total * sizeof(float)) {
      if (N.f32_arena.p) PNPX_HIP(hipFree(N.f32_arena.p));
      N.f32_arena = DeviceBuf();
      N.f32_capB = N.f32_capH = N.f32_capW = 0;
      void* p = nullptr;
      hipError_t e = hipMalloc(&p, Pl.total * sizeof(float));
      if (e != hipSuccess) {
        set_error("DRUNet fp32 arena allocation of %zu bytes failed: %s", Pl.total * sizeof(float), hipGetErrorString(e));
        return PNPX_ERR_ALLOC;
      }
      N.f32_arena.p = p;
      N.f32_arena.bytes = Pl.total * sizeof(float);
    }
    PNPX_HIP(hipMemset(N.f32_arena.p, 0, N.f32_arena.bytes));
    N.f32_capB = nb_img;
    N.f32_capH = H;
    N.f32_capW = W;
    N.f32_arena_keeps = keeps;
  }
  const Plan Pl = plan_of(N.f32_capB, H, W, N.f32_arena_keeps ? N.nb : 0);
  float* const A = static_cast<float*>(N.f32_arena.p);
  const std::vector<LayerDesc> L = layers_of(N.nb);
  size_t li = 0;

  auto conv = [&](const float* in, float* outp, int h, int w, float slope, const float* res) -> int {
    const ConvLayer& Lc = N.f32_layers[li];
    const float* u = N.f32_wino[li];
    const int kind = L[li].kind;
    ++li;
    if (kind == 3 || kind == 4) return launch_conv1x1_act(Lc, in, outp, B, h, w, slope, res, s);
    if (u && ctx->opt_fp32_winograd && conv3x3_wino_ok(Lc.cin, 0, Lc.cout, h, w))
    {
      if (ctx->opt_fp32_wino8 && conv3x3_wino8_ok(Lc.cin, 0, Lc.cout, h, w))
        return launch_conv3x3_wino8(u, Lc.b, Lc.cout, in, Lc.cin, nullptr, 0, outp, B, h, w, s, slope, res, nullptr);
      return launch_conv3x3_wino(u, Lc.b, Lc.cout, in, Lc.cin, nullptr, 0, outp, B, h, w, s, slope, res, nullptr);
    }
    return launch_conv3x3_act(Lc, in, Lc.cin, nullptr, 0, outp, B, h, w, slope, res, s);
  };
  auto resblocks = [&](int l, int dec, float* cur, float** result) -> int {
    const int h = H >> l, w = W >> l;
    float* pq[2] = {A + Pl.P[l], A + Pl.Q[l]};
    int k = 0;
    for (int i = 0; i < N.nb; ++i) {
      float* mid = keep_mids ? A + Pl.MK[l][dec * N.nb + i] : A + Pl.M[l];
      PNPX_TRY(conv(cur, mid, h, w, 0.f, nullptr));
      float* dst = pq[k];
      if (dst == cur) dst = pq[k ^= 1];
      PNPX_TRY(conv(mid, dst, h, w, 1.f, cur));
      cur = dst;
      k ^= 1;
    }
    *result = cur;
    return PNPX_OK;
  };

  hipLaunchKernelGGL(f32_prep_kernel, dim3((W + 63) / 64, H, B), dim3(64), 0, s, x, sigma, sigma_stride, A + Pl.in2, H, W, padded_h(H),
                     padded_w(W));
  PNPX_LAUNCH_CHECK();
  PNPX_TRY(conv(A + Pl.in2, A + Pl.S[0], H, W, 1.f, nullptr));
  float* cur = A + Pl.S[0];
  for (int l = 0; l < 3; ++l) {
    PNPX_TRY(resblocks(l, 0, cur, &cur));
    const int h = H >> l, w = W >> l;
    const size_t n = (size_t)B * 4 * NC[l] * (h / 2) * (w / 2);
    hipLaunchKernelGGL(f32_s2d_kernel, g1(n), dim3(256), 0, s, cur, A + Pl.DT[l + 1], NC[l], h, w, n);
    PNPX_LAUNCH_CHECK();
    PNPX_TRY(conv(A + Pl.DT[l + 1], A + Pl.S[l + 1], h / 2, w / 2, 1.f, nullptr));
    cur = A + Pl.S[l + 1];
  }
  PNPX_TRY(resblocks(3, 0, cur, &cur));
  for (int l = 2; l >= 0; --l) {
    const int h = H >> (l + 1), w = W >> (l + 1);
    const size_t na = (size_t)B * NC[l + 1] * h * w;
    hipLaunchKernelGGL(f32_add_kernel, g1(na), dim3(256), 0, s, cur, A + Pl.S[l + 1], A + Pl.M[l + 1], h, w, na);
    PNPX_LAUNCH_CHECK();
    PNPX_TRY(conv(A + Pl.M[l + 1], A + Pl.DT[l + 1], h, w, 1.f, nullptr));
    const size_t nd = (size_t)B * NC[l] * (2 * h) * (2 * w);
    hipLaunchKernelGGL(f32_d2s_kernel, g1(nd), dim3(256), 0, s, A + Pl.DT[l + 1], A + Pl.U[l], NC[l], h, w, nd);
    PNPX_LAUNCH_CHECK();
    PNPX_TRY(resblocks(l, 1, A + Pl.U[l], &cur));
  }
  {
    const size_t na = (size_t)B * NC[0] * H * W;
    hipLaunchKernelGGL(f32_add_kernel, g1(na), dim3(256), 0, s, cur, A + Pl.S[0], A + Pl.M[0], H, W, na);
    PNPX_LAUNCH_CHECK();
  }
  PNPX_TRY(conv(A + Pl.M[0], A + Pl.T32, H, W, 1.f, nullptr));
  hipLaunchKernelGGL(f32_out_kernel, dim3((W + 63) / 64, H, B), dim3(64), 0, s, A + Pl.T32, out, out_pre, H, W);
  PNPX_LAUNCH_CHECK();
  if (li != L.size()) {
    set_error("DRUNet fp32: internal layer walk mismatch (%zu of %zu)", li, L.size());
    return PNPX_ERR_ARG;
  }
  return PNPX_OK;
}

int drunet_denoise_backward_f32(pnpx_ctx* ctx, const float* x, const float* sigma, int sigma_stride, const float* grad_out, float* grad_x,
                                float* grad_sigma, int B, int H, int W, hipStream_t s) {
  DruNet& N = ctx->drunet;
  const size_t npix = (size_t)B * H * W;
  void* sp;
  PNPX_TRY(ctx_scratch(ctx, (3 * npix + (size_t)B * SIG_CHUNKS) * sizeof(float) + 8192, &sp));
  float* out_tmp = static_cast<float*>(sp);
  float* pre = out_tmp + npix;
  float* g_pre = pre + npix;
  float* part = g_pre + npix;
  PNPX_TRY(drunet_denoise_f32(ctx, x, sigma, sigma_stride, out_tmp, pre, B, H, W, s, true));
  PNPX_TRY(prepare_weights_bwd(ctx));
  const Plan F = plan_of(N.f32_capB, H, W, N.nb);
  const float* const FA = static_cast<const float*>(N.f32_arena.p);
  if (B > N.f32_gcapB || H != N.f32_gcapH || W != N.f32_gcapW) {
    const int nb_img = (H == N.f32_gcapH && W == N.f32_gcapW && N.f32_gcapB > B) ? N.f32_gcapB : B;
    const Plan Gp = plan_of(nb_img, H, W);
    PNPX_HIP(hipDeviceSynchronize());
    if (N.f32_arena_grad.bytes < Gp.total * sizeof(float)) {
      if (N.f32_arena_grad.p) PNPX_HIP(hipFree(N.f32_arena_grad.p));
      N.f32_arena_grad = DeviceBuf();
      N.f32_gcapB = N.f32_gcapH = N.f32_gcapW = 0;
      void* p = nullptr;
      hipError_t e = hipMalloc(&p, Gp.total * sizeof(float));
      if (e != hipSuccess) {
        set_error("DRUNet fp32 gradient arena allocation of %zu bytes failed: %s", Gp.total * sizeof(float), hipGetErrorString(e));
        return PNPX_ERR_ALLOC;
      }
      N.f32_arena_grad.p = p;
      N.f32_arena_grad.bytes = Gp.total * sizeof(float);
    }
    PNPX_HIP(hipMemset(N.f32_arena_grad.p, 0, N.f32_arena_grad.bytes));
    N.f32_gcapB = nb_img;
    N.f32_gcapH = H;
    N.f32_gcapW = W;
  }
  const Plan G = plan_of(N.f32_gcapB, H, W);
  float* const GA = static_cast<float*>(N.f32_arena_grad.p);
  const int nb = N.nb;
  const std::vector<LayerDesc> L = layers_of(nb);
  auto idx_down = [&](int l) { return 1 + l * (2 * nb + 1); };
  auto idx_strided = [&](int l) { return idx_down(l) + 2 * nb; };
  const int idx_body = 1 + 3 * (2 * nb + 1);
  auto idx_convT = [&](int l) { return idx_body + 2 * nb + (2 - l) * (2 * nb + 1); };
  auto idx_up = [&](int l) { return idx_convT(l) + 1; };

  auto conv = [&](int li, const float* in, float* outp, int h, int w, const float* dmask, const float* res) -> int {
    const ConvLayer& Lc = N.f32_layers_bwd[li];
    const int kind = L[li].kind;
    if (kind == 3 || kind == 4) return launch_conv1x1_act(Lc, in, outp, B, h, w, 1.f, res, s);
    const float* u = N.f32_wino_bwd[li];
    if (u && ctx->opt_fp32_winograd && ctx->opt_fp32_wino8 && conv3x3_wino8_ok(Lc.cin, 0, Lc.cout, h, w)) {
      if (dmask) return launch_conv3x3_wino8_grad(u, Lc.b, Lc.cout, in, Lc.cin, outp, dmask, 0.f, B, h, w, s);
      return launch_conv3x3_wino8(u, Lc.b, Lc.cout, in, Lc.cin, nullptr, 0, outp, B, h, w, s, 1.f, res, nullptr);
    }
    if (dmask) return launch_conv3x3_grad(Lc, in, outp, dmask, B, h, w, s, nullptr, 0.f);
    return launch_conv3x3_act(Lc, in, Lc.cin, nullptr, 0, outp, B, h, w, 1.f, res, s);
  };
  auto resblocks_bwd = [&](int l, int dec, int idx0, float* cur, float** result) -> int {
    const int h = H >> l, w = W >> l;
    float* pq[2] = {GA + G.P[l], GA + G.Q[l]};
    int k = 0;
    for (int i = nb - 1; i >= 0; --i) {
      const float* mid = FA + F.MK[l][dec * nb + i];
      PNPX_TRY(conv(idx0 + 2 * i + 1, cur, GA + G.M[l], h, w, mid, nullptr));
      float* dst = pq[k];
      if (dst == cur) dst = pq[k ^= 1];
      PNPX_TRY(conv(idx0 + 2 * i, GA + G.M[l], dst, h, w, nullptr, cur));
      cur = dst;
      k ^= 1;
    }
    *result = cur;
    return PNPX_OK;
  };
  auto add = [&](const float* a, const float* b, float* o, int l) -> int {
    const int h = H >> l, w = W >> l;
    const size_t n = (size_t)B * NC[l] * h * w;
    hipLaunchKernelGGL(f32_add_kernel, g1(n), dim3(256), 0, s, a, b, o, h, w, n);
    PNPX_LAUNCH_CHECK();
    return PNPX_OK;
  };

  hipLaunchKernelGGL(f32_tail_mask_kernel, g1(npix), dim3(256), 0, s, grad_out, pre, g_pre, npix);
  PNPX_LAUNCH_CHECK();
  hipLaunchKernelGGL(conv_first_f32_kernel, dim3((H * (W / 4) + 255) / 256, NC[0] / 8, B), dim3(256), 0, s, g_pre, N.zero, 0, N.tail_bwd_w,
                     N.zero, GA + G.S[0], H, W, 1.0f);
  PNPX_LAUNCH_CHECK();
  float* cur = GA + G.S[0];
  for (int l = 0; l <= 2; ++l) {
    PNPX_TRY(resblocks_bwd(l, 1, idx_up(l), cur, &cur));
    const int h = H >> l, w = W >> l;
    const size_t n = (size_t)B * 4 * NC[l] * (h / 2) * (w / 2);
    hipLaunchKernelGGL(f32_s2d_kernel, g1(n), dim3(256), 0, s, cur, GA + G.DT[l + 1], NC[l], h, w, n);
    PNPX_LAUNCH_CHECK();
    PNPX_TRY(conv(idx_convT(l), GA + G.DT[l + 1], GA + G.S[l + 1], h / 2, w / 2, nullptr, nullptr));
    cur = GA + G.S[l + 1];
  }
  PNPX_TRY(resblocks_bwd(3, 0, idx_body, cur, &cur));
  PNPX_TRY(add(cur, GA + G.S[3], GA + G.M[3], 3));
  for (int l = 2; l >= 0; --l) {
    const int h = H >> (l + 1), w = W >> (l + 1);
    PNPX_TRY(conv(idx_strided(l), GA + G.M[l + 1], GA + G.DT[l + 1], h, w, nullptr, nullptr));
    const size_t n = (size_t)B * NC[l] * (2 * h) * (2 * w);
    hipLaunchKernelGGL(f32_d2s_kernel, g1(n), dim3(256), 0, s, GA + G.DT[l + 1], GA + G.U[l], NC[l], h, w, n);
    PNPX_LAUNCH_CHECK();
    PNPX_TRY(resblocks_bwd(l, 0, idx_down(l), GA + G.U[l], &cur));
    PNPX_TRY(add(cur, GA + G.S[l], GA + G.M[l], l));
  }
  PNPX_TRY(conv(0, GA + G.M[0], GA + G.T32, H, W, nullptr, nullptr));
  hipLaunchKernelGGL(f32_input_grad_kernel, dim3(SIG_CHUNKS, B), dim3(256), 0, s, GA + G.T32, 32, grad_x, part, H, W);
  PNPX_LAUNCH_CHECK();
  hipLaunchKernelGGL(sigma_grad_final_kernel, dim3((B + 63) / 64), dim3(64), 0, s, part, grad_sigma, B);
  PNPX_LAUNCH_CHECK();
  return PNPX_OK;
}

}
```

### tfpnp_amd/csrc/unet.hip

```cpp
#include <cstdlib>

#include "common.h"
#include "conv3x3.h"
#include "conv_hs.h"
#include "conv_first.h"
#include "hs_rec.h"
#include "unet_plan.h"

namespace pnpx {

__global__ void prep_input_kernel(const float* __restrict__ x, const float* __restrict__ sigma, int sigma_stride,
                                  float* __restrict__ dst, int H, int W, int Hp, int Wp) {
  const int b = blockIdx.z;
  const int y = blockIdx.y;
  const int xx = blockIdx.x * blockDim.x + threadIdx.x;
  if (xx >= W) return;
  const float v = x[((size_t)b * H + y) * W + xx];
  float* d = dst + (size_t)b * 2 * Hp * Wp + (size_t)(y + 1) * Wp + xx + PADL;
  d[0] = v;
  d[(size_t)Hp * Wp] = sigma[(size_t)b * sigma_stride];
}

__global__ __launch_bounds__(256) void maxpool2_kernel(const float* __restrict__ src, float* __restrict__ dst,
                                                       size_t n_out, int H, int W) {
// ... 245 lines not shown

size_t unet_arena_bytes(int mode, int B, int H, int W) { return make_plan(mode, B, H, W).total; }

void train_cache_free(pnpx_ctx* ctx) {
  (void)hipDeviceSynchronize();
  for (auto& sl : ctx->train_ring) {
    if (sl.arena.buf.p) (void)hipFree(sl.arena.buf.p);
    if (sl.pre.p) (void)hipFree(sl.pre.p);
  }
  ctx->train_ring.clear();
  ctx->train_H = ctx->train_W = 0;
  ctx->train_mode = -1;
}

static pnpx_ctx::TrainSlot* train_slot_acquire(pnpx_ctx* ctx, int B, int H, int W) {
  if (ctx->opt_train_cache_gb == 0 || ctx->train_alloc_failed) return nullptr;
  const int mode = ctx->conv_mode;
  int capB = B;
  for (const auto& sl : ctx->train_ring) capB = sl.arena.capB > capB ? sl.arena.capB : capB;
  const size_t per = unet_arena_bytes(mode, capB, H, W) + sizeof(float) * (size_t)capB * H * W;
  if (ctx->opt_train_cache_gb < 0 && ctx->train_budget_bytes == 0) {
    size_t free_b = 0, total_b = 0;
    if (hipMemGetInfo(&free_b, &total_b) != hipSuccess) {
      (void)hipGetLastError();
      free_b = 0;
    }
    size_t held = 0;
    for (const auto& sl : ctx->train_ring) held += sl.arena.buf.bytes + sl.pre.bytes;
    ctx->train_budget_bytes = std::min<size_t>((free_b + held) / 4, (size_t)96 << 30);
    if (ctx->train_budget_bytes == 0) ctx->train_budget_bytes = 1;
  }
  const size_t budget = ctx->opt_train_cache_gb < 0 ? ctx->train_budget_bytes : ((size_t)ctx->opt_train_cache_gb << 30);
  size_t n = budget / per;
  if (n == 0) return nullptr;
  if (n > 64) n = 64;
  if (H != ctx->train_H || W != ctx->train_W || mode != ctx->train_mode || n != ctx->train_ring.size()) {
    train_cache_free(ctx);
    ctx->train_ring.resize(n);
    ctx->train_H = H;
    ctx->train_W = W;
    ctx->train_mode = mode;
  }
  pnpx_ctx::TrainSlot& sl = ctx->train_ring[ctx->train_counter % ctx->train_ring.size()];
  sl.ticket = 0;
  const size_t need = sizeof(float) * (size_t)B * H * W;
  if (sl.pre.bytes < need) {
    (void)hipDeviceSynchronize();
    if (sl.pre.p) (void)hipFree(sl.pre.p);
    sl.pre = DeviceBuf();
    void* q = nullptr;
    if (hipMalloc(&q, need) != hipSuccess) {
      (void)hipGetLastError();
      ctx->train_alloc_failed = true;
      train_cache_free(ctx);
      return nullptr;
    }
    sl.pre.p = q;
    sl.pre.bytes = need;
  }
  return &sl;
}

int unet_denoise_train(pnpx_ctx* ctx, const float* x, const float* sigma, int sigma_stride, float* out, int B, int H,
                       int W, hipStream_t s, unsigned long long* ticket) {
  *ticket = 0;
  if (ctx->drunet.loaded)
    return unet_denoise(ctx, x, sigma, sigma_stride, out, nullptr, B, H, W, s, nullptr);
  if (pnpx_ctx::TrainSlot* sl = train_slot_acquire(ctx, B, H, W)) {
    const int st = unet_denoise(ctx, x, sigma, sigma_stride, out, static_cast<float*>(sl->pre.p), B, H, W, s, nullptr,
                                &sl->arena, ctx->conv_mode, true);
    if (st == PNPX_OK) {
      sl->ticket = *ticket = ++ctx->train_counter;
      sl->B = B;
      return PNPX_OK;
    }
    if (st != PNPX_ERR_ALLOC) return st;
    ctx->train_alloc_failed = true;
    train_cache_free(ctx);
  }
  return unet_denoise(ctx, x, sigma, sigma_stride, out, nullptr, B, H, W, s, nullptr);
}

int unet_denoise_backward_ticket(pnpx_ctx* ctx, const float* x, const float* sigma, int sigma_stride,
                                 const float* grad_out, float* grad_x, float* grad_sigma, int B, int H, int W,
                                 hipStream_t s, unsigned long long ticket) {
  if (ticket != 0 && !ctx->train_ring.empty() && H == ctx->train_H && W == ctx->train_W) {
    pnpx_ctx::TrainSlot& sl = ctx->train_ring[(ticket - 1) % ctx->train_ring.size()];
    if (sl.ticket == ticket && sl.B == B)
      return unet_denoise_backward(ctx, x, sigma, sigma_stride, grad_out, grad_x, grad_sigma, B, H, W, s, &sl.arena,
                                   static_cast<const float*>(sl.pre.p));
  }
  return unet_denoise_backward(ctx, x, sigma, sigma_stride, grad_out, grad_x, grad_sigma, B, H, W, s);
}

int ctx_reserve_unet(pnpx_ctx* ctx, int B, int H, int W) {
  return reserve_arena(ctx, ctx->arena, ctx->conv_mode, B, H, W, 0);
}

namespace {

struct Recorder {
  ProfileSink* sink;
  hipStream_t s;
  int mark(const char* name, double flops) {
    if (!sink) return PNPX_OK;
    if ((size_t)sink->n + 1 >= sink->events->size()) return PNPX_OK;
    PNPX_HIP(hipEventRecord((*sink->events)[sink->n + 1], s));
    sink->names.push_back(name);
    sink->flops.push_back(flops);
    sink->n++;
    return PNPX_OK;
  }
  void credit(double flops) {
    if (sink && !sink->flops.empty()) sink->flops.back() += flops;
  }
};

inline dim3 g1d(size_t n) { return dim3((unsigned)((n + 255) / 256)); }

}

static int unet_forward_hs(pnpx_ctx* ctx, UNetArena& ar, const UNetPlan& P, const float* x, const float* sigma,
                           int sigma_stride, float* out, float* out_pre, int B, int H, int W, hipStream_t s,
                           Recorder& rec, bool keep_all, int b_base = 0, int share = 1) {
  char* A = static_cast<char*>(ar.buf.p);
  auto bpi = [&](const Act& d) { return act_bytes_per_image(CONV_HS, d.C, d.H, d.W); };
  auto at = [&](const Act& d, int b0) { return A + d.off + (size_t)(b0 + b_base) * bpi(d); };
  auto rat = [&](const Act& d, int b0) { return reinterpret_cast<HsRec*>(at(d, b0)); };
  const bool no_pool_fuse = !ctx->opt_fuse_pool, no_outc_fuse = keep_all || !ctx->opt_fuse_outc;
  unsigned* const range_flag = ctx->opt_range_guard ? ctx->range_flag_dev : nullptr;
  const int sub_default = ctx->opt_subbatch;
  auto sub_of = [&](int level) {
    if (sub_default <= 0 || level > 1) return B;
    const int sb = sub_default * (level == 1 ? 2 : 1) * (256 * 256) / ((H * W) > 0 ? (H * W) : 1);
    return sb < 1 ? 1 : (sb > B ? B : sb);
  };
  auto pool_fused = [&](int l) { return !no_pool_fuse && l < 4 && conv_hs_can_pool(P.x[l].H, P.x[l].W); };

  const size_t npix = (size_t)B * H * W;
  const bool first_fused = ctx->opt_fuse_first != 0;
  if (!first_fused) {
    hipLaunchKernelGGL(prep_input_hs_kernel, g1d(npix), dim3(256), 0, s, x, sigma, sigma_stride, rat(P.in0, 0), H, W, npix);
    PNPX_LAUNCH_CHECK();
    PNPX_TRY(rec.mark("prep_input", 0));
  }

  auto conv = [&](int li, const Act& i0, const Act* i1, const Act& o, int b0, int nb, const ConvHsFuse& fuse) -> int {
    const ConvLayer& L = ctx->conv[li];
    const ConvLayerHsDev& D = ctx->conv_hs[li];
    ConvLayerHs Lh;
    Lh.cin = D.cin;
    Lh.cout = D.cout;
    Lh.cin_pad = D.cin_pad;
    Lh.mt = D.mt;
    Lh.w = D.w;
    Lh.b = L.b;
    Lh.inv_scale = D.inv_scale;
    ConvHsFuse fz = fuse;
    fz.range_flag = range_flag;
    fz.wreg = ctx->opt_wreg;
    fz.share = share;
    PNPX_TRY(launch_conv_hs(Lh, at(i0, b0), i0.C / 8, i1 ? at(*i1, b0) : nullptr, i1 ? i1->C / 8 : 0, at(o, b0), nb, o.H,
                            o.W, fz, s));
    return rec.mark("conv3x3", 2.0 * 9.0 * L.cin * L.cout * (double)o.H * o.W * nb);
  };
  auto block = [&](int li, const Act& i0, const Act* i1, int lvl, const Act& o, int b0, int nb,
                   const ConvHsFuse& fuse, const ConvHsFuse& first_fuse = ConvHsFuse()) -> int {
    const Act& ta = i1 ? P.da[lvl] : P.a[lvl];
    const Act& tb = i1 ? P.db[lvl] : P.b[lvl];
    bool folded = false;
    if (li == 0 && first_fused && ctx->opt_fold_first && !keep_all) {
      const ConvLayerHsDev& D1 = ctx->conv_hs[1];
      ConvLayerHs L1;
      L1.cin = D1.cin;
      L1.cout = D1.cout;
      L1.mt = D1.mt;
      ConvHsFuse f1;
      f1.wreg = ctx->opt_wreg;
      if (conv_hs_can_fold_first(L1, ta.C / 8, nb, H, W, f1)) {
        f1.first_x = x + (size_t)b0 * H * W;
        f1.first_sigma = sigma + (size_t)b0 * sigma_stride;
        f1.first_sigma_stride = sigma_stride;
        f1.first_w = ctx->conv0_w;
        f1.first_b = ctx->conv[0].b;
        f1.first_zero = ctx->zero_bias;
        f1.first_slope = 0.2f;
        PNPX_TRY(conv(1, ta, nullptr, tb, b0, nb, f1));
        rec.credit(2.0 * 9.0 * 2 * 32 * (double)H * W * nb);
        folded = true;
      }
    }
    if (folded) {
    } else if (li == 0 && first_fused) {
      hipLaunchKernelGGL(conv_first_hs_kernel, dim3((H * W + 255) / 256, 4, nb), dim3(256), 0, s, x + (size_t)b0 * H * W,
                         sigma + (size_t)b0 * sigma_stride, sigma_stride, ctx->conv0_w, ctx->conv[0].b, rat(ta, b0), H, W,
                         0.2f, HS_ASCALE);
      PNPX_LAUNCH_CHECK();
      PNPX_TRY(rec.mark("conv3x3", 2.0 * 9.0 * 2 * 32 * (double)H * W * nb));
    } else
    PNPX_TRY(conv(li, i0, i1, ta, b0, nb, first_fuse));
    if (!folded) PNPX_TRY(conv(li + 1, ta, nullptr, tb, b0, nb, ConvHsFuse()));
    return conv(li + 2, tb, nullptr, o, b0, nb, fuse);
  };

  for (int l = 0; l < 5; ++l) {
    const Act& in = (l == 0) ? P.in0 : P.p[l];
    const int sb = sub_of(l);
    for (int b0 = 0; b0 < B; b0 += sb) {
      const int nb = (B - b0 < sb) ? (B - b0) : sb;
      if (l > 0 && !pool_fused(l - 1)) {
        const Act& src = P.x[l - 1];
        const size_t n_pool = (size_t)nb * (src.C / 8) * (src.H / 2) * (src.W / 2);
        hipLaunchKernelGGL(maxpool2_hs_kernel, g1d(n_pool), dim3(256), 0, s, rat(src, b0), rat(P.p[l], b0), n_pool, src.H,
                           src.W);
        PNPX_LAUNCH_CHECK();
        PNPX_TRY(rec.mark("maxpool2", 0));
      }
      ConvHsFuse f;
      if (pool_fused(l)) f.pool_out = at(P.p[l + 1], b0);
      PNPX_TRY(block(3 * l, in, nullptr, l, P.x[l], b0, nb, f));
    }
  }
  const Act* below = &P.x[4];
  for (int l = 3; l >= 0; --l) {
    const int h = below->H, w = below->W;
    const float sy = (2 * h > 1) ? (float)(h - 1) / (float)(2 * h - 1) : 0.f;
    const float sx = (2 * w > 1) ? (float)(w - 1) / (float)(2 * w - 1) : 0.f;
    const int sb = sub_of(l);
    for (int b0 = 0; b0 < B; b0 += sb) {
      const int nb = (B - b0 < sb) ? (B - b0) : sb;
      ConvHsFuse f;
      ConvHsFuse f_first;
      bool ups_fused = false;
      if (ctx->opt_fuse_up >= (l == 0 ? 1 : 2)) {
        const ConvLayerHsDev& D0 = ctx->conv_hs[15 + 3 * (3 - l)];
        ConvLayerHs L0;
        L0.cout = D0.cout;
        L0.mt = D0.mt;
        ups_fused = P.u[l].H == 2 * h && P.u[l].W == 2 * w && P.x[l].H == 2 * h && P.x[l].W == 2 * w &&
                    conv_hs_can_fuse_upsample(L0, P.x[l].C / 8, below->C / 8, 2 * h, 2 * w);
      }
      if (ups_fused) {
        f_first.ups_h = h;
        f_first.ups_w = w;
      } else {
        const unsigned nbg = (unsigned)(nb * (below->C / 8));
        const int Wo = 2 * w, Ho = 2 * h;
        if (Wo > 32) {
          hipLaunchKernelGGL((upsample2x_hs_kernel<64, 4>), dim3((Wo + 63) / 64, (Ho + 15) / 16, nbg), dim3(256), 0, s,
                             rat(*below, b0), rat(P.u[l], b0), h, w, P.u[l].H, P.u[l].W, sy, sx);
        } else {
          hipLaunchKernelGGL((upsample2x_hs_kernel<32, 2>), dim3((Wo + 31) / 32, (Ho + 15) / 16, nbg), dim3(256), 0, s,
                             rat(*below, b0), rat(P.u[l], b0), h, w, P.u[l].H, P.u[l].W, sy, sx);
        }
        PNPX_LAUNCH_CHECK();
        PNPX_TRY(rec.mark("upsample2x", 0));
      }
      if (l == 0 && !no_outc_fuse) {
        f.outc_w = ctx->outc_w;
        f.outc_b = ctx->outc_b;
        f.x_in = x + (size_t)b0 * H * W;
        f.out_img = out + (size_t)b0 * H * W;
        f.out_pre = out_pre ? out_pre + (size_t)b0 * H * W : nullptr;
      }
      PNPX_TRY(block(15 + 3 * (3 - l), P.x[l], ups_fused ? below : &P.u[l], l, P.y[l], b0, nb, f, f_first));
    }
    below = &P.y[l];
  }
  if (no_outc_fuse) {
    hipLaunchKernelGGL(outc_residual_hs_kernel, g1d(npix), dim3(256), 0, s, rat(P.y[0], 0), x, ctx->outc_w, ctx->outc_b,
                       out, out_pre, H, W, npix);
    PNPX_LAUNCH_CHECK();
    PNPX_TRY(rec.mark("outc_residual_clamp", 2.0 * 32 * (double)H * W * B));
  }
  return PNPX_OK;
}

static int unet_forward_f32(pnpx_ctx* ctx, UNetArena& ar, const UNetPlan& P, const float* x, const float* sigma, int sigma_stride, float* out,
                            float* out_pre, int B, int H, int W, hipStream_t s, Recorder& rec, bool keep_all, bool level_chains, int b_base = 0, int B_call = 0) {
  if (B_call <= 0) B_call = B;
  char* A = static_cast<char*>(ar.buf.p);
  auto fptr = [&](const Act& d) { return reinterpret_cast<float*>(A + d.off + (size_t)b_base * act_bytes_per_image(CONV_F32, d.C, d.H, d.W)); };
  float* const ks_part0 = reinterpret_cast<float*>(A + P.ks_part + (size_t)b_base * P.ks_part_per_image);
  auto ks_on = [&](int cout, int h, int w) {
    if (ctx->opt_fp32_ksplit == 2) return true;
    return ctx->opt_fp32_ksplit == 1 && (long long)(h / 16) * (w / 16) * (cout / 64) * B_call < 256;
  };
  const bool first_valu = ctx->opt_fuse_first && W % 4 == 0 && ctx->conv[0].cout == 32;
  if (!first_valu) {
    hipLaunchKernelGGL(prep_input_kernel, dim3((W + 63) / 64, H, B), dim3(64), 0, s, x, sigma, sigma_stride, fptr(P.in0), H,
                       W, padded_h(H), padded_w(W));
    PNPX_LAUNCH_CHECK();
    PNPX_TRY(rec.mark("prep_input", 0));
  }
  auto conv = [&](int li, const Act& i0, const Act* i1, const Act& o, const Act* pooled = nullptr, bool* pooled_done = nullptr) -> int {
    const ConvLayer& L = ctx->conv[li];
    const int C1 = i1 ? i1->C : 0;
    if (pooled_done) *pooled_done = false;
    if (ctx->opt_fp32_winograd && ctx->conv_wino_u[li] && conv3x3_wino_ok(i0.C, C1, L.cout, o.H, o.W)) {
      const bool w8 = ((ctx->opt_fp32_wino8 >> li) & 1) && conv3x3_wino8_ok(i0.C, C1, L.cout, o.H, o.W);
      if (w8) {
        const bool ks = ks_on(L.cout, o.H, o.W);
        PNPX_TRY(launch_conv3x3_wino8(ctx->conv_wino_u[li], L.b, L.cout, fptr(i0), i0.C, i1 ? fptr(*i1) : nullptr, C1, fptr(o), B, o.H, o.W, s, 0.2f,
                                      nullptr, pooled ? fptr(*pooled) : nullptr, ks ? ks_part0 : nullptr, ctx->opt_ksplit_rule));
      }
      else
        PNPX_TRY(launch_conv3x3_wino(ctx->conv_wino_u[li], L.b, L.cout, fptr(i0), i0.C, i1 ? fptr(*i1) : nullptr, C1, fptr(o), B, o.H, o.W, s, 0.2f,
                                     nullptr, pooled ? fptr(*pooled) : nullptr));
      if (pooled_done) *pooled_done = pooled != nullptr;
      return rec.mark("conv3x3_wino", 2.0 * 9.0 * L.cin * L.cout * (double)o.H * o.W * B);
    } else {
      PNPX_TRY(launch_conv3x3(L, fptr(i0), i0.C, i1 ? fptr(*i1) : nullptr, C1, fptr(o), B, o.H, o.W, s));
    }
    return rec.mark("conv3x3", 2.0 * 9.0 * L.cin * L.cout * (double)o.H * o.W * B);
  };
  auto block = [&](int li, const Act& i0, const Act* i1, int lvl, const Act& o, const Act* pooled = nullptr, bool* pooled_done = nullptr) -> int {
    const Act& ta = i1 ? P.da[lvl] : P.a[lvl];
    const Act& tb = i1 ? P.db[lvl] : P.b[lvl];
    if (li == 0 && first_valu) {
      hipLaunchKernelGGL(conv_first_f32_kernel, dim3((H * (W / 4) + 255) / 256, 4, B), dim3(256), 0, s, x, sigma, sigma_stride, ctx->conv0_w,
                         ctx->conv[0].b, fptr(ta), H, W, 0.2f);
      PNPX_LAUNCH_CHECK();
      PNPX_TRY(rec.mark("conv3x3", 2.0 * 9.0 * 2 * 32 * (double)H * W * B));
    } else
    PNPX_TRY(conv(li, i0, i1, ta));
    PNPX_TRY(conv(li + 1, ta, nullptr, tb));
    return conv(li + 2, tb, nullptr, o, pooled, pooled_done);
  };
  bool pooled = false;
  PNPX_TRY(block(0, P.in0, nullptr, 0, P.x[0], &P.p[1], &pooled));
  for (int l = 1; l < 5; ++l) {
    const Act& src = P.x[l - 1];
    if (!pooled) {
      const size_t n_pool = (size_t)B * src.C * (src.H / 2) * (src.W / 2);
      hipLaunchKernelGGL(maxpool2_kernel, g1d(n_pool), dim3(256), 0, s, fptr(src), fptr(P.p[l]), n_pool, src.H, src.W);
      PNPX_LAUNCH_CHECK();
      PNPX_TRY(rec.mark("maxpool2", 0));
    }
    if (l == 4 && level_chains && B >= 2) {
      const Act& o4 = P.x[4];
      bool all8 = ctx->opt_fp32_winograd != 0;
      for (int li = 12; li < 15; ++li)
        all8 = all8 && ctx->conv_wino_u[li] && ((ctx->opt_fp32_wino8 >> li) & 1) && conv3x3_wino8_ok(ctx->conv[li].cin, 0, ctx->conv[li].cout, o4.H, o4.W);
      const long long ntiles = (long long)(o4.H / 16) * (o4.W / 16) * B * (ctx->conv[13].cout / 64);
      if (all8 && ntiles > 256 && ntiles < 768 && ntiles % 256 != 0) {
        PNPX_TRY(fan_out_chains(ctx, 2, B, s, [&](int lo, int hi, hipStream_t st) -> int {
          auto slice = [&](int li, const Act& i, const Act& o) -> int {
            const ConvLayer& L = ctx->conv[li];
            return launch_conv3x3_wino8(ctx->conv_wino_u[li], L.b, L.cout, fptr(i) + (size_t)lo * i.C * padded_h(i.H) * padded_w(i.W), i.C, nullptr, 0,
                                        fptr(o) + (size_t)lo * o.C * padded_h(o.H) * padded_w(o.W), hi - lo, o.H, o.W, st, 0.2f, nullptr, nullptr,
                                        ks_on(o.C, o.H, o.W) ? ks_part0 + (size_t)lo * (P.ks_part_per_image / sizeof(float)) : nullptr,
                                        ctx->opt_ksplit_rule);
          };
          PNPX_TRY(slice(12, P.p[4], P.a[4]));
          PNPX_TRY(slice(13, P.a[4], P.b[4]));
          return slice(14, P.b[4], P.x[4]);
        }));
        pooled = false;
        continue;
      }
    }
    PNPX_TRY(block(3 * l, P.p[l], nullptr, l, P.x[l], l < 4 ? &P.p[l + 1] : nullptr, &pooled));
  }
  const Act* below = &P.x[4];
  for (int l = 3; l >= 0; --l) {
    const int h = below->H, w = below->W;
    const float sy = (2 * h > 1) ? (float)(h - 1) / (float)(2 * h - 1) : 0.f;
    const float sx = (2 * w > 1) ? (float)(w - 1) / (float)(2 * w - 1) : 0.f;
    const size_t n_up = (size_t)B * below->C * (2 * h) * (2 * w);
    const int li0 = 15 + 3 * (3 - l);
    const bool entry_splits = ks_on(ctx->conv[li0].cout, 2 * h, 2 * w) &&
                              conv3x3_wino8_ksplit(P.x[l].C, below->C, ctx->conv[li0].cout, 2 * h, 2 * w, ctx->opt_ksplit_rule) > 1;
    const bool ups_fused = !entry_splits && ctx->opt_fp32_fuse_up && ctx->opt_fp32_winograd && ctx->conv_wino_u[li0] && ((ctx->opt_fp32_wino8 >> li0) & 1) &&
                           P.x[l].H == 2 * h && P.x[l].W == 2 * w && conv3x3_wino8_ups_ok(P.x[l].C, below->C, ctx->conv[li0].cout, 2 * h, 2 * w);
    if (ups_fused) {
    } else if ((2 * w) % 4 == 0 && (size_t)B * below->C <= 65535) {
      const int quads = w / 2, bx = quads >= 64 ? 64 : quads, by = 256 / bx;
      hipLaunchKernelGGL(upsample2x_v4_kernel, dim3((quads + bx - 1) / bx, (2 * h + by * UPS_ROWS - 1) / (by * UPS_ROWS), B * below->C), dim3(bx, by), 0, s,
                         fptr(*below), fptr(P.u[l]), h, w, P.u[l].H, P.u[l].W, sy, sx);
    } else {
      hipLaunchKernelGGL(upsample2x_kernel, g1d(n_up), dim3(256), 0, s, fptr(*below), fptr(P.u[l]), n_up, h, w, P.u[l].H,
                         P.u[l].W, sy, sx);
    }
    if (!ups_fused) {
      PNPX_LAUNCH_CHECK();
      PNPX_TRY(rec.mark("upsample2x", 0));
    }
    auto entry = [&](const Act& ta) -> int {
      if (!ups_fused) return conv(li0, P.x[l], &P.u[l], ta);
      const ConvLayer& L = ctx->conv[li0];
      PNPX_TRY(launch_conv3x3_wino8_ups(ctx->conv_wino_u[li0], L.b, L.cout, fptr(P.x[l]), P.x[l].C, fptr(*below), below->C, fptr(ta), B, 2 * h, 2 * w, s));
      return rec.mark("conv3x3_wino", 2.0 * 9.0 * L.cin * L.cout * (double)(2 * h) * (2 * w) * B);
    };
    const bool fuse_outc = l == 0 && !keep_all && ctx->opt_fuse_outc && ctx->opt_fp32_winograd && ctx->conv_wino_u[26] &&
                           conv3x3_wino_outc_ok(ctx->conv[26].cin, ctx->conv[26].cout, H, W);
    if (fuse_outc) {
      PNPX_TRY(entry(P.da[0]));
      PNPX_TRY(conv(25, P.da[0], nullptr, P.db[0]));
      const bool w8 = ((ctx->opt_fp32_wino8 >> 26) & 1) && conv3x3_wino8_ok(ctx->conv[26].cin, 0, ctx->conv[26].cout, H, W);
      PNPX_TRY((w8 ? launch_conv3x3_wino8_outc : launch_conv3x3_wino_outc)(ctx->conv_wino_u[26], ctx->conv[26].b, fptr(P.db[0]), ctx->conv[26].cin,
                                                                          ctx->outc_w, ctx->outc_b, x, out, out_pre, B, H, W, s));
      return rec.mark("conv3x3_wino", 2.0 * 9.0 * ctx->conv[26].cin * ctx->conv[26].cout * (double)H * W * B);
    }
    PNPX_TRY(entry(P.da[l]));
    PNPX_TRY(conv(li0 + 1, P.da[l], nullptr, P.db[l]));
    PNPX_TRY(conv(li0 + 2, P.db[l], nullptr, P.y[l]));
    below = &P.y[l];
  }
  hipLaunchKernelGGL(outc_residual_kernel, dim3((W + 63) / 64, H, B), dim3(64), 0, s, fptr(P.y[0]), x, ctx->outc_w,
                     ctx->outc_b, out, out_pre, H, W);
  PNPX_LAUNCH_CHECK();
  PNPX_TRY(rec.mark("outc_residual_clamp", 2.0 * 32 * (double)H * W * B));
  return PNPX_OK;
}

int launch_chains(const pnpx_ctx* ctx, int B, int H, int W) {
  int n = ctx->opt_chains;
  if (n == 0) {
    const long long q = (long long)B * H * W / (256 * 256);
    n = (q >= 5 && q != 8) ? 2 : 1;
  }
  if (n > 8) n = 8;
  return n > B ? B : (n < 1 ? 1 : n);
}

void join_side_streams_after_failure(pnpx_ctx* ctx) {
  for (hipStream_t st : ctx->side_streams) (void)hipStreamSynchronize(st);
}
int chain_streams(pnpx_ctx* ctx, int chains) {
  if (chains > 16) {
    set_error("launch chains: at most 16 slices");
    return PNPX_ERR_ARG;
  }
  while ((int)ctx->side_streams.size() < chains - 1) {
    hipStream_t st = nullptr;
    PNPX_HIP(hipStreamCreateWithFlags(&st, hipStreamNonBlocking));
    ctx->side_streams.push_back(st);
  }
  return PNPX_OK;
}
int chain_event(pnpx_ctx* ctx, hipEvent_t* ev) {
  constexpr size_t POOL = 256;
  if (ctx->ev_pool.size() < POOL) {
    hipEvent_t e = nullptr;
    PNPX_HIP(hipEventCreateWithFlags(&e, hipEventDisableTiming));
    ctx->ev_pool.push_back(e);
    *ev = e;
    return PNPX_OK;
  }
  *ev = ctx->ev_pool[ctx->ev_next++ % POOL];
  return PNPX_OK;
}

int unet_denoise(pnpx_ctx* ctx, const float* x, const float* sigma, int sigma_stride, float* out, float* out_pre,
                 int B, int H, int W, hipStream_t s, ProfileSink* prof, UNetArena* arena, int mode, bool keep_all) {
  if (ctx->drunet.loaded) {
    if (arena || keep_all || prof) {
      set_error("the DRUNet denoiser keeps its activations in its own arena (drunet_denoise_backward re-computes them) and has no per-launch profile");
      return PNPX_ERR_ARG;
    }
    return drunet_denoise(ctx, x, sigma, sigma_stride, out, out_pre, B, H, W, s);
  }
  if (!ctx->has_weights) {
    set_error("denoiser called before pnpx_unet_load");
    return PNPX_ERR_NO_WEIGHTS;
  }
  if (B <= 0 || H < 16 || W < 16) {
    set_error("denoiser: need B > 0 and H, W >= 16 (four 2x2 poolings; got B=%d H=%d W=%d)", B, H, W);
    return PNPX_ERR_SHAPE;
  }
  UNetArena& ar = arena ? *arena : ctx->arena;
  if (mode < 0) mode = ctx->conv_mode;
  PNPX_TRY(reserve_arena(ctx, ar, mode, B, H, W, 0));
  const bool hs = (mode == CONV_HS);
  const UNetPlan P = make_plan(mode, ar.capB, H, W);
  Recorder rec{prof, s};
  if (prof) PNPX_HIP(hipEventRecord((*prof->events)[0], s));
  const int chains = hs && !prof ? launch_chains(ctx, B, H, W) : 1;
  if (chains > 1) {
    const size_t px = (size_t)H * W;
    return fan_out_chains(ctx, chains, B, s, [&](int lo, int hi, hipStream_t st) -> int {
      Recorder none{nullptr, st};
      return unet_forward_hs(ctx, ar, P, x + lo * px, sigma + (size_t)lo * sigma_stride, sigma_stride, out + lo * px,
                             out_pre ? out_pre + lo * px : nullptr, hi - lo, H, W, st, none, keep_all, lo, chains);
    });
  }
  if (hs) return unet_forward_hs(ctx, ar, P, x, sigma, sigma_stride, out, out_pre, B, H, W, s, rec, keep_all);

  if (!prof && ctx->opt_fp32_chains >= 2 && B >= ctx->opt_fp32_chains) {
    const size_t px = (size_t)H * W;
    return fan_out_chains(ctx, ctx->opt_fp32_chains, B, s, [&](int lo, int hi, hipStream_t st) -> int {
      Recorder none{nullptr, st};
      return unet_forward_f32(ctx, ar, P, x + lo * px, sigma + (size_t)lo * sigma_stride, sigma_stride, out + lo * px,
                              out_pre ? out_pre + lo * px : nullptr, hi - lo, H, W, st, none, keep_all, false, lo, B);
    });
  }
  return unet_forward_f32(ctx, ar, P, x, sigma, sigma_stride, out, out_pre, B, H, W, s, rec, keep_all, !prof && ctx->opt_fp32_chains == 1);
}

}
```

### tfpnp_amd/csrc/unet_bwd.hip

```cpp
#include "common.h"
#include "conv3x3.h"
#include "conv_hs.h"
#include "hs_rec.h"
#include "unet_plan.h"
#include "grad_common.h"

namespace pnpx {
namespace {

inline dim3 g1(size_t n) { return dim3((unsigned)((n + 255) / 256)); }

__device__ __forceinline__ float dlrelu(float a) { return a > 0.f ? 1.f : 0.2f; }

struct SavedAct {
  const void* p;
  int hs;
};
__device__ __forceinline__ float act_at(const SavedAct& A, size_t b, int C, int c, int H, int W, int y, int x) {
  if (A.hs) {
    const size_t rec = ((b * (C >> 3) + (c >> 3)) * (H + 2) + (y + 1)) * (size_t)(W + 2) + (x + 1);
    const _Float16* r = reinterpret_cast<const _Float16*>(static_cast<const char*>(A.p) + rec * 32);
    return (float)r[c & 7] + (float)r[8 + (c & 7)];
  }
  return static_cast<const float*>(A.p)[((b * C + c) * (size_t)padded_h(H) + (y + 1)) * padded_w(W) + x + PADL];
// ... 276 lines not shown
  }
  __syncthreads();
  const int xs = xs0 + (threadIdx.x % UB_T), ys = ys0 + (threadIdx.x / UB_T);
  if (xs >= w || ys >= h) return;
  auto window = [&](int ry, int rx, float v[8]) {
    HsRec r;
    r.hi = *reinterpret_cast<const h8v*>(&win[((rx & 1) * UB_W + ry) * (UB_W / 2) + (rx >> 1)]);
    r.lo = *reinterpret_cast<const h8v*>(&win[((2 + (rx & 1)) * UB_W + ry) * (UB_W / 2) + (rx >> 1)]);
    hs_unpack(r, v);
  };
  float wyv[7], wxv[7];
#pragma unroll
  for (int i = 0; i < 7; ++i) {
    const int yd = 2 * ys - 3 + i, xd = 2 * xs - 3 + i;
    wyv[i] = wxv[i] = 0.f;
    if (yd >= 0 && yd < H) {
      const float fy = sy * yd;
      const int y0 = (int)fy;
      const int y1 = y0 + (y0 < h - 1 ? 1 : 0);
      const float ly = fy - y0;
      if (y0 == ys) wyv[i] += 1.f - ly;
      if (y1 == ys) wyv[i] += ly;
    }
    if (xd >= 0 && xd < W) {
      const float fx = sx * xd;
      const int x0 = (int)fx;
      const int x1 = x0 + (x0 < w - 1 ? 1 : 0);
      const float lx = fx - x0;
      if (x0 == xs) wxv[i] += 1.f - lx;
      if (x1 == xs) wxv[i] += lx;
    }
  }
  float acc[8];
#pragma unroll
  for (int k = 0; k < 8; ++k) acc[k] = 0.f;
  const int oy = 2 * (ys - ys0), ox = 2 * (xs - xs0);
#pragma unroll
  for (int i = 0; i < 7; ++i) {
#pragma unroll
    for (int j = 0; j < 7; ++j) {
      if (wyv[i] != 0.f && wxv[j] != 0.f) {
        float v[8];
        window(oy + i, ox + j, v);
#pragma unroll
        for (int k = 0; k < 8; ++k) acc[k] += wyv[i] * wxv[j] * v[k];
      }
    }
  }
  const size_t r = ((b * Gs + g) * (h + 2) + (ys + 1)) * (size_t)(w + 2) + (xs + 1);
  float a[8];
  hs_unpack(src_act[r], a);
#pragma unroll
  for (int k = 0; k < 8; ++k) acc[k] *= dlrelu(a[k]);
  g_src[r] = hs_pack(acc);
}

__global__ __launch_bounds__(256) void skip_pool_merge_hs_kernel(const HsRec* __restrict__ gcat, int Gcat,
                                                                 const HsRec* __restrict__ g_pool,
                                                                 const HsRec* __restrict__ xact, HsRec* __restrict__ g_x,
                                                                 int G, int H, int W, size_t n) {
  const size_t i = (size_t)blockIdx.x * blockDim.x + threadIdx.x;
  if (i >= n) return;
  const int x = (int)(i % W);
  size_t t = i / W;
  const int y = (int)(t % H);
  t /= H;
  const int g = (int)(t % G);
  const size_t b = t / G;
  const size_t plane = (size_t)(H + 2) * (W + 2);
  const size_t r = (b * G + g) * plane + (size_t)(y + 1) * (W + 2) + (x + 1);
  float gv[8], a[8];
  if (gcat) {
    hs_unpack(gcat[(b * Gcat + g) * plane + (size_t)(y + 1) * (W + 2) + (x + 1)], gv);
  } else {
#pragma unroll
    for (int k = 0; k < 8; ++k) gv[k] = 0.f;
  }
  hs_unpack(xact[r], a);
  if (g_pool) {
    const int Ho = H / 2, Wo = W / 2, yo = y >> 1, xo = x >> 1;
    if (yo < Ho && xo < Wo) {
      const HsRec* w0 = xact + (b * G + g) * plane + (size_t)(2 * yo + 1) * (W + 2) + (2 * xo + 1);
      float v00[8], v01[8], v10[8], v11[8], gp[8];
      hs_unpack(w0[0], v00);
      hs_unpack(w0[1], v01);
      hs_unpack(w0[W + 2], v10);
      hs_unpack(w0[W + 3], v11);
      hs_unpack(g_pool[((b * G + g) * (Ho + 2) + (yo + 1)) * (size_t)(Wo + 2) + (xo + 1)], gp);
      const int me = (y & 1) * 2 + (x & 1);
#pragma unroll
      for (int k = 0; k < 8; ++k) {
        int arg = 0;
        float m = v00[k];
        if (v01[k] > m) { m = v01[k]; arg = 1; }
        if (v10[k] > m) { m = v10[k]; arg = 2; }
        if (v11[k] > m) { m = v11[k]; arg = 3; }
        if (arg == me) gv[k] += gp[k];
      }
    }
  }
#pragma unroll
  for (int k = 0; k < 8; ++k) gv[k] *= dlrelu(a[k]);
  g_x[r] = hs_pack(gv);
}

struct GradPlan {
  Act in0;
  Act a[5], b[5], x[5], p[5], y[4], cat[4];
  size_t total = 0;
};
GradPlan make_grad_plan(int mode, int capB, int H, int W) {
  GradPlan P;
  size_t off = 0;
  auto add = [&](Act& d, int C, int h, int w) {
    d.off = off;
    d.C = C;
    d.H = h;
    d.W = w;
    off += act_bytes_per_image(mode, C, h, w) * (size_t)capB;
    off = (off + 255) & ~(size_t)255;
  };
  add(P.in0, 32, H, W);
  for (int l = 0; l < 5; ++l) {
    const int h = H >> l, w = W >> l, c = 32 << l;
    add(P.a[l], c, h, w);
    add(P.b[l], c, h, w);
    add(P.x[l], c, h, w);
    if (l >= 1) add(P.p[l], c / 2, h, w);
    if (l <= 3) {
      add(P.y[l], c, h, w);
      add(P.cat[l], 3 * c, h, w);
    }
  }
  P.total = off + (1u << 20);
  return P;
}

}

int unet_denoise_backward(pnpx_ctx* ctx, const float* x, const float* sigma, int sigma_stride, const float* grad_out,
                          float* grad_x, float* grad_sigma, int B, int H, int W, hipStream_t s, UNetArena* cached,
                          const float* cached_pre) {
  if (ctx->drunet.loaded) {
    if (B <= 0 || !grad_out || !grad_x || !grad_sigma) {
      set_error("denoiser backward: need B > 0 and non-null gradients");
      return PNPX_ERR_ARG;
    }
    return drunet_denoise_backward(ctx, x, sigma, sigma_stride, grad_out, grad_x, grad_sigma, B, H, W, s);
  }
  if (!ctx->has_weights) {
    set_error("denoiser backward called before pnpx_unet_load");
    return PNPX_ERR_NO_WEIGHTS;
  }
  if (B <= 0 || H < 16 || W < 16) {
    set_error("denoiser backward: need B > 0 and H, W >= 16");
    return PNPX_ERR_SHAPE;
  }
  const size_t npix = (size_t)B * H * W;
  void* sp;
  PNPX_TRY(ctx_scratch(ctx, (3 * npix + (size_t)B * SIG_CHUNKS) * sizeof(float) + 8192, &sp));
  float* out_tmp = static_cast<float*>(sp);
  float* pre = out_tmp + npix;
  float* g_res = pre + npix;
  float* part = g_res + npix;
  float2* gscale = reinterpret_cast<float2*>(part + (((size_t)B * SIG_CHUNKS + 63) & ~(size_t)63));
  unsigned* gmax_bits = reinterpret_cast<unsigned*>(gscale + 1);

  const int fmode = cached ? cached->mode : ctx->conv_mode;
  const bool hs = (fmode == CONV_HS);
  UNetArena& fa = cached ? *cached : ctx->arena;
  if (cached) {
    if (!(B <= cached->capB && H == cached->capH && W == cached->capW && cached_pre)) {
      set_error("denoiser backward: the cached activations do not belong to a %dx%dx%d forward", B, H, W);
      return PNPX_ERR_ARG;
    }
    pre = const_cast<float*>(cached_pre);
  } else {
    PNPX_TRY(unet_denoise(ctx, x, sigma, sigma_stride, out_tmp, pre, B, H, W, s, nullptr, &ctx->arena, fmode, true));
  }
  const UNetPlan F = make_plan(fmode, fa.capB, H, W);
  char* FA = static_cast<char*>(fa.buf.p);

  {
    UNetArena& ga = ctx->arena_grad;
    if (!(B <= ga.capB && H == ga.capH && W == ga.capW && ga.mode == fmode)) {
      const bool same = (H == ga.capH && W == ga.capW);
      const int nb = same ? (B > ga.capB ? B : ga.capB) : B;
      const GradPlan GP = make_grad_plan(fmode, nb, H, W);
      PNPX_HIP(hipDeviceSynchronize());
      if (ga.buf.bytes < GP.total) {
        if (ga.buf.p) PNPX_HIP(hipFree(ga.buf.p));
        ga = UNetArena();
        void* p = nullptr;
        hipError_t e = hipMalloc(&p, GP.total);
        if (e != hipSuccess) {
          set_error("gradient arena allocation of %zu bytes failed: %s", GP.total, hipGetErrorString(e));
          return PNPX_ERR_ALLOC;
        }
        ga.buf.p = p;
        ga.buf.bytes = GP.total;
      }
      PNPX_HIP(hipMemset(ga.buf.p, 0, GP.total));
      PNPX_HIP(hipDeviceSynchronize());
      ga.capB = nb;
      ga.capH = H;
      ga.capW = W;
      ga.mode = fmode;
    }
  }
  const GradPlan G = make_grad_plan(fmode, ctx->arena_grad.capB, H, W);
  char* GA = static_cast<char*>(ctx->arena_grad.buf.p);

  if (hs) {
    PNPX_HIP(hipMemsetAsync(gmax_bits, 0, sizeof(unsigned), s));
    hipLaunchKernelGGL(absmax_kernel, dim3(512), dim3(256), 0, s, grad_out, npix, gmax_bits);
    hipLaunchKernelGGL(grad_scale_kernel, dim3(1), dim3(1), 0, s, gmax_bits, gscale);
    auto run_hs = [&](int lo, int B, hipStream_t s, int share) -> int {
    const size_t npix = (size_t)B * H * W, px0 = (size_t)lo * H * W;
    auto grec = [&](const Act& d) { return reinterpret_cast<HsRec*>(GA + d.off + (size_t)lo * act_bytes_per_image(CONV_HS, d.C, d.H, d.W)); };
    auto frec = [&](const Act& d) { return reinterpret_cast<const HsRec*>(FA + d.off + (size_t)lo * act_bytes_per_image(CONV_HS, d.C, d.H, d.W)); };
    hipLaunchKernelGGL(outc_bwd_hs_kernel, g1(npix * 4), dim3(256), 0, s, grad_out + px0, pre + px0, ctx->outc_w, frec(F.y[0]),
                       grec(G.y[0]), g_res + px0, gscale, H, W, npix * 4);
    PNPX_LAUNCH_CHECK();
    auto convH = [&](int li, const Act& gin, const Act& gout, const Act* saved) -> int {
      const ConvLayerHsDev& D = ctx->conv_hs_bwd[li];
      ConvLayerHs Lh;
      Lh.cin = D.cin;
      Lh.cout = D.cout;
      Lh.cin_pad = D.cin_pad;
      Lh.mt = D.mt;
      Lh.w = D.w;
      Lh.b = ctx->zero_bias;
      Lh.inv_scale = D.inv_scale;
      if (gin.C != D.cin || gout.C != D.cout) {
        set_error("backward: gradient tensor channels %d -> %d do not match adjoint layer %d (%d -> %d)", gin.C, gout.C,
                  li, D.cin, D.cout);
        return PNPX_ERR_SHAPE;
      }
      ConvHsFuse f;
      f.dmask = saved ? FA + saved->off + (size_t)lo * act_bytes_per_image(CONV_HS, saved->C, saved->H, saved->W) : nullptr;
      f.share = share;
      f.slope = saved ? 0.2f : 1.0f;
      f.range_flag = ctx->opt_range_guard ? ctx->range_flag_dev : nullptr;
      return launch_conv_hs(Lh, reinterpret_cast<const char*>(grec(gin)), gin.C / 8, nullptr, 0, reinterpret_cast<char*>(grec(gout)), B, gout.H,
                            gout.W, f, s);
    };
    for (int l = 0; l <= 3; ++l) {
      const int li = 15 + 3 * (3 - l);
      PNPX_TRY(convH(li + 2, G.y[l], G.b[l], &F.db[l]));
      PNPX_TRY(convH(li + 1, G.b[l], G.a[l], &F.da[l]));
      PNPX_TRY(convH(li, G.a[l], G.cat[l], nullptr));
      const Act& below_f = (l == 3) ? F.x[4] : F.y[l + 1];
      const Act& below_g = (l == 3) ? G.x[4] : G.y[l + 1];
      const int h = below_f.H, w = below_f.W, Gs = below_f.C / 8;
      const float sy = (2 * h > 1) ? (float)(h - 1) / (float)(2 * h - 1) : 0.f;
      const float sx = (2 * w > 1) ? (float)(w - 1) / (float)(2 * w - 1) : 0.f;
      hipLaunchKernelGGL(upsample_bwd_hs_kernel, dim3((w + UB_T - 1) / UB_T, (h + UB_T - 1) / UB_T, (unsigned)(B * Gs)), dim3(256),
                         0, s, grec(G.cat[l]), G.cat[l].C / 8, F.x[l].C / 8, frec(below_f), grec(below_g), Gs, h, w,
                         G.cat[l].H, G.cat[l].W, sy, sx);
      PNPX_LAUNCH_CHECK();
    }
    for (int l = 4; l >= 0; --l) {
      if (l < 4) {
        const size_t n = (size_t)B * (F.x[l].C / 8) * F.x[l].H * F.x[l].W;
        hipLaunchKernelGGL(skip_pool_merge_hs_kernel, g1(n), dim3(256), 0, s, grec(G.cat[l]), G.cat[l].C / 8,
                           grec(G.p[l + 1]), frec(F.x[l]), grec(G.x[l]), F.x[l].C / 8, F.x[l].H, F.x[l].W, n);
        PNPX_LAUNCH_CHECK();
      }
      PNPX_TRY(convH(3 * l + 2, G.x[l], G.b[l], &F.b[l]));
      PNPX_TRY(convH(3 * l + 1, G.b[l], G.a[l], &F.a[l]));
      PNPX_TRY(convH(3 * l, G.a[l], l == 0 ? G.in0 : G.p[l], nullptr));
    }
    hipLaunchKernelGGL(input_grad_hs_kernel, dim3(SIG_CHUNKS, B), dim3(256), 0, s, grec(G.in0), g_res + px0, grad_x + px0,
                       part + (size_t)lo * SIG_CHUNKS, gscale, H, W);
    PNPX_LAUNCH_CHECK();
    hipLaunchKernelGGL(sigma_grad_final_kernel, dim3((B + 63) / 64), dim3(64), 0, s, part + (size_t)lo * SIG_CHUNKS, grad_sigma + lo, B);
    PNPX_LAUNCH_CHECK();
    return PNPX_OK;
    };
    const int chains = launch_chains(ctx, B, H, W);
    if (chains <= 1) return run_hs(0, B, s, 1);
    return fan_out_chains(ctx, chains, B, s, [&](int lo, int hi, hipStream_t st) -> int { return run_hs(lo, hi - lo, st, chains); });
  }

  auto run = [&](int lo, int B, hipStream_t s) -> int {
  const size_t npix = (size_t)B * H * W, px0 = (size_t)lo * H * W;
  const float* const grad_out_s = grad_out + px0;
  const float* const pre_s = pre + px0;
  float* const g_res_s = g_res + px0;
  float* const grad_x_s = grad_x ? grad_x + px0 : nullptr;
  float* const part_s = part + (size_t)lo * SIG_CHUNKS;
  float* const grad_sigma_s = grad_sigma ? grad_sigma + lo : nullptr;
  auto gp = [&](const Act& d) { return reinterpret_cast<float*>(GA + d.off + (size_t)lo * act_bytes_per_image(fmode, d.C, d.H, d.W)); };
  auto sa = [&](const Act& d) { return SavedAct{FA + d.off + (size_t)lo * act_bytes_per_image(fmode, d.C, d.H, d.W), 0}; };
  hipLaunchKernelGGL(outc_bwd_kernel, g1(npix), dim3(256), 0, s, grad_out_s, pre_s, ctx->outc_w, sa(F.y[0]), gp(G.y[0]),
                     g_res_s, H, W, npix);
  PNPX_LAUNCH_CHECK();

  auto convT = [&](int li, const Act& gin, const Act& gout, const Act* saved) -> int {
    const float* dm = saved ? reinterpret_cast<const float*>(FA + saved->off + (size_t)lo * act_bytes_per_image(fmode, saved->C, saved->H, saved->W)) : nullptr;
    const char* dmh = nullptr;
    if (!hs && ctx->opt_fp32_winograd && ((ctx->opt_fp32_wino8 >> li) & 1) && ctx->conv_wino_u_bwd[li] && gout.C == ctx->conv_bwd[li].cout &&
        conv3x3_wino8_ok(gin.C, 0, gout.C, gout.H, gout.W))
      return launch_conv3x3_wino8_grad(ctx->conv_wino_u_bwd[li], ctx->zero_bias, gout.C, gp(gin), gin.C, gp(gout), dm, 0.2f, B, gout.H, gout.W, s);
    return launch_conv3x3_grad(ctx->conv_bwd[li], gp(gin), gp(gout), dm, B, gout.H, gout.W, s, dmh);
  };

  for (int l = 0; l <= 3; ++l) {
    const int li = 15 + 3 * (3 - l);
    PNPX_TRY(convT(li + 2, G.y[l], G.b[l], &F.db[l]));
    PNPX_TRY(convT(li + 1, G.b[l], G.a[l], &F.da[l]));
    PNPX_TRY(convT(li, G.a[l], G.cat[l], nullptr));
    const Act& below_f = (l == 3) ? F.x[4] : F.y[l + 1];
    const Act& below_g = (l == 3) ? G.x[4] : G.y[l + 1];
    const int h = below_f.H, w = below_f.W, Cb = below_f.C;
    const float sy = (2 * h > 1) ? (float)(h - 1) / (float)(2 * h - 1) : 0.f;
    const float sx = (2 * w > 1) ? (float)(w - 1) / (float)(2 * w - 1) : 0.f;
    const size_t n = (size_t)B * Cb * h * w;
    if (!hs && (size_t)B * Cb <= 65535) {
      if (w >= 64)
        hipLaunchKernelGGL(upsample_bwd_lds_kernel<64>, dim3((w + 63) / 64, (h + UBF_T - 1) / UBF_T, (unsigned)(B * Cb)), dim3(256), 0, s, gp(G.cat[l]),
                           G.cat[l].C, F.x[l].C, static_cast<const float*>(sa(below_f).p), gp(below_g), Cb, h, w, G.cat[l].H, G.cat[l].W, sy, sx);
      else
        hipLaunchKernelGGL(upsample_bwd_lds_kernel<16>, dim3((w + 15) / 16, (h + UBF_T - 1) / UBF_T, (unsigned)(B * Cb)), dim3(256), 0, s, gp(G.cat[l]),
                           G.cat[l].C, F.x[l].C, static_cast<const float*>(sa(below_f).p), gp(below_g), Cb, h, w, G.cat[l].H, G.cat[l].W, sy, sx);
    } else {
      hipLaunchKernelGGL(upsample_bwd_kernel, g1(n), dim3(256), 0, s, gp(G.cat[l]), G.cat[l].C, F.x[l].C, sa(below_f),
                         gp(below_g), Cb, h, w, G.cat[l].H, G.cat[l].W, sy, sx, n);
    }
    PNPX_LAUNCH_CHECK();
  }
  for (int l = 4; l >= 0; --l) {
    if (l < 4) {
      const size_t n = (size_t)B * F.x[l].C * F.x[l].H * F.x[l].W;
      if (F.x[l].H % 2 == 0 && F.x[l].W % 2 == 0) {
        hipLaunchKernelGGL(skip_pool_merge_f32_kernel, g1(n / 4), dim3(256), 0, s, gp(G.cat[l]), G.cat[l].C, gp(G.p[l + 1]),
                           static_cast<const float*>(sa(F.x[l]).p), gp(G.x[l]), F.x[l].C, F.x[l].H, F.x[l].W, n / 4);
      } else {
        hipLaunchKernelGGL(skip_pool_merge_kernel, g1(n), dim3(256), 0, s, gp(G.cat[l]), G.cat[l].C, gp(G.p[l + 1]),
                           sa(F.x[l]), gp(G.x[l]), F.x[l].C, F.x[l].H, F.x[l].W, n);
      }
      PNPX_LAUNCH_CHECK();
    }
    PNPX_TRY(convT(3 * l + 2, G.x[l], G.b[l], &F.b[l]));
    PNPX_TRY(convT(3 * l + 1, G.b[l], G.a[l], &F.a[l]));
    PNPX_TRY(convT(3 * l, G.a[l], l == 0 ? G.in0 : G.p[l], nullptr));
  }
  hipLaunchKernelGGL(input_grad_kernel, dim3(SIG_CHUNKS, B), dim3(256), 0, s, gp(G.in0), G.in0.C, g_res_s, grad_x_s, part_s, H,
                     W);
  PNPX_LAUNCH_CHECK();
  hipLaunchKernelGGL(sigma_grad_final_kernel, dim3((B + 63) / 64), dim3(64), 0, s, part_s, grad_sigma_s, B);
  PNPX_LAUNCH_CHECK();
  return PNPX_OK;
  };
  if (ctx->opt_fp32_chains >= 2 && B >= 2)
    return fan_out_chains(ctx, 2, B, s, [&](int lo, int hi, hipStream_t st) -> int { return run(lo, hi - lo, st); });
  return run(0, B, s);
}

}
```

Before: 114.1 iters/s.

## Use 16-byte halo gathers and reschedule weight DMA in 32-cout Winograd kernel

Adds an H16 variant of the 32-cout Winograd F(2x2,3x3) conv kernel. It pads the raw halo row width by two so the input tile can be staged with 16-byte global-to-LDS loads instead of 4-byte ones, cutting the number of DMA instructions. The raw DMA moves to earlier slots, and the next tile's weight (U) DMA is deferred to after the epilogue on the last chunk, with the exchange buffers remapped to fit. The path is on by default through a new fp32_halo16 option. It costs extra LDS per row, and the loads may be misaligned or over-read at the padded row edge.

New measurement: 115.5 iters/s (median of 3 runs). No clear change (+1.3%).

```diff
diff --git a/tfpnp_amd/csrc/api.hip b/tfpnp_amd/csrc/api.hip
--- a/tfpnp_amd/csrc/api.hip
+++ b/tfpnp_amd/csrc/api.hip
@@ -268,6 +268,10 @@
     ctx->opt_fp32_fuse_up = value;
     return PNPX_OK;
   }
+  if (is("fp32_halo16") && (value == 0 || value == 1)) {
+    ctx->opt_fp32_halo16 = value;
+    return PNPX_OK;
+  }
   if (is("fp32_ksplit") && value >= 0 && value <= 2) {
     ctx->opt_fp32_ksplit = value;
     return PNPX_OK;
@@ -347,6 +351,7 @@
   else if (is("fp32_winograd")) *value = ctx->opt_fp32_winograd;
   else if (is("fp32_wino8_layers")) *value = ctx->opt_fp32_wino8;
   else if (is("fp32_fuse_up")) *value = ctx->opt_fp32_fuse_up;
+  else if (is("fp32_halo16")) *value = ctx->opt_fp32_halo16;
   else if (is("fp32_ksplit")) *value = ctx->opt_fp32_ksplit;
   else if (is("fp32_ksplit_rule")) *value = ctx->opt_ksplit_rule;
   else if (is("fp32_chains")) *value = ctx->opt_fp32_chains;
diff --git a/tfpnp_amd/csrc/common.h b/tfpnp_amd/csrc/common.h
--- a/tfpnp_amd/csrc/common.h
+++ b/tfpnp_amd/csrc/common.h
@@ -176,6 +176,7 @@
   int opt_fp32_chains = 2;
   int opt_fp32_ksplit = 1;
   int opt_ksplit_rule = 1;
+  int opt_fp32_halo16 = 1;
   int opt_fp32_fuse_up = 1;
   pnpx::ConvLayer conv_bwd[27];
   pnpx::ConvLayerHsDev conv_hs_bwd[27];
diff --git a/tfpnp_amd/csrc/conv3x3.h b/tfpnp_amd/csrc/conv3x3.h
--- a/tfpnp_amd/csrc/conv3x3.h
+++ b/tfpnp_amd/csrc/conv3x3.h
@@ -43,16 +43,16 @@
 bool conv3x3_wino8_ok(int C0, int C1, int cout, int H, int W);
 int launch_conv3x3_wino8(const float* u, const float* bias, int cout, const float* in0, int C0, const float* in1, int C1,
                          float* out, int B, int H, int W, hipStream_t s, float slope = 0.2f, const float* res = nullptr,
-                         float* pool_out = nullptr, float* ks_part = nullptr, int ks_rule = 1);
+                         float* pool_out = nullptr, float* ks_part = nullptr, int ks_rule = 1, int halo16 = 1);
 int conv3x3_wino8_ksplit(int C0, int C1, int cout, int H, int W, int rule = 1);
 size_t conv3x3_wino8_ksplit_bytes_per_image();
 int launch_conv3x3_wino8_grad(const float* u, const float* zero_bias, int cout, const float* gin, int cin, float* gout, const float* dmask,
-                              float mask_slope, int B, int H, int W, hipStream_t s);
+                              float mask_slope, int B, int H, int W, hipStream_t s, int halo16 = 1);
 bool conv3x3_wino8_ups_ok(int C0, int C1, int cout, int H, int W);
 int launch_conv3x3_wino8_ups(const float* u, const float* bias, int cout, const float* in0, int C0, const float* in1_lowres, int C1,
-                             float* out, int B, int H, int W, hipStream_t s, float slope = 0.2f);
+                             float* out, int B, int H, int W, hipStream_t s, float slope = 0.2f, int halo16 = 1);
 int launch_conv3x3_wino8_outc(const float* u, const float* bias, const float* in0, int cin, const float* outc_w, const float* outc_b,
-                              const float* x_img, float* img, float* img_pre, int B, int H, int W, hipStream_t s);
+                              const float* x_img, float* img, float* img_pre, int B, int H, int W, hipStream_t s, int halo16 = 1);
 void pack_conv_weights_transposed(const float* w, int cout, int cin, int cout_pad, int mt, int cc, float* dst);
 
 }
diff --git a/tfpnp_amd/csrc/conv3x3_wino8.hip b/tfpnp_amd/csrc/conv3x3_wino8.hip
--- a/tfpnp_amd/csrc/conv3x3_wino8.hip
+++ b/tfpnp_amd/csrc/conv3x3_wino8.hip
@@ -12,9 +12,11 @@
 
 using namespace wino;
 
-template <int CT_>
+template <int CT_, int H16_ = 0>
 struct Cfg8 {
   static constexpr int CT = CT_;
+  static constexpr int H16 = H16_;
+  static_assert(!H16 || CT == 32, "16-byte halo gathers: the 32-cout tile");
   static constexpr int CK = (CT == 64) ? 16 : 8;
   static constexpr int HALVES = CK / 8;
   static constexpr int KS = CK / 2;
@@ -25,13 +27,16 @@
   static_assert(NM == 16, "the side-work schedule below is written for 16 MFMA slots per stage");
   static constexpr int RPXW = (CT == 64) ? 16 : 32;
   static constexpr int TX = RPXW / 2, NT = 8 * TX;
-  static constexpr int RW = RPXW + 2, RPX = 18 * RW;
+  static constexpr int HW = RPXW + 2;
+  static constexpr int RW = H16 ? HW + 2 : HW, RPX = 18 * RW;
   static constexpr int RPXL = (CT == 64) ? 328 : RPX;
   static constexpr int RAW_ELEMS = CK * RPXL;
-  static constexpr int RAW_INSTR = (RAW_ELEMS + 63) / 64;
-  static constexpr int RAW_BYTES = RAW_INSTR * 256;
+  static constexpr int RAW_GRAN = H16 ? 4 : 1;
+  static constexpr int RAW_INSTR = (RAW_ELEMS / RAW_GRAN + 63) / 64;
+  static constexpr int RAW_IBYTES = 256 * RAW_GRAN;
+  static constexpr int RAW_BYTES = RAW_INSTR * RAW_IBYTES;
   static constexpr int RAW_PER_WAVE = (RAW_INSTR + 7) / 8;
-  static constexpr int NRAW = RAW_INSTR / 8;
+  static constexpr int NRAW = H16 ? RAW_PER_WAVE : RAW_INSTR / 8;
   static constexpr int UQ = 16 * CK * CT;
   static constexpr int USTG = RS * UQ;
   static constexpr int NUW = USTG / 8192;
@@ -48,7 +53,7 @@
   static constexpr int ST_PER_WAVE = (ST_INSTR + 7) / 8, NSW = ST_INSTR / 8;
   static constexpr int OFF_ST = LDS_USED, OFF_TAB = OFF_ST + 2 * ST_STRIDE;
   static constexpr int LDS_USED_UPS = OFF_TAB + (18 + RW) * 16;
-  static constexpr int NPOSI = 18 * RW;
+  static constexpr int NPOSI = 18 * HW;
 };
 constexpr int LDS_REQ8 = 160 * 1024;
 
@@ -91,9 +96,9 @@
 #define WINO8_STAMP(tag)
 #endif
 
-template <bool RAWDMA_, bool STDMA_, int IQ_>
+template <bool RAWDMA_, bool STDMA_, int IQ_, bool UDMA_ = true>
 struct StageKind {
-  static constexpr bool RAWDMA = RAWDMA_, STDMA = STDMA_;
+  static constexpr bool RAWDMA = RAWDMA_, STDMA = STDMA_, UDMA = UDMA_;
   static constexpr int IQ = IQ_;
 };
 
@@ -104,14 +109,14 @@
 using Yes = std::true_type;
 using No = std::false_type;
 
-template <int CT, bool FUSE_OUTC, bool RES, bool UPS, bool KSPLIT>
+template <int CT, bool FUSE_OUTC, bool RES, bool UPS, bool KSPLIT, int H16>
 __global__ __launch_bounds__(512, 1) void conv3x3_wino8_f32_kernel(WinoArgs a) {
   static_assert(!FUSE_OUTC || CT == 32, "the fused out-conv needs all 32 couts of a pixel in one SIMD's wave pair");
   static_assert(!UPS || (!FUSE_OUTC && !RES), "the up-sampling instances are the UNet's plain decoder entries");
   static_assert(!KSPLIT || (CT == 64 && !FUSE_OUTC && !RES && !UPS), "K-split: the plain 64-cout instance (the deep levels' layers)");
-  using C = Cfg8<CT>;
+  using C = Cfg8<CT, H16>;
   constexpr int CK = C::CK, HALVES = C::HALVES, KS = C::KS, RS = C::RS, NSTG = C::NSTG, NPOS = C::NPOS;
-  constexpr int TX = C::TX, NT = C::NT, RW = C::RW, RPX = C::RPX, RPXL = C::RPXL;
+  constexpr int TX = C::TX, NT = C::NT, HW = C::HW, RW = C::RW, RPX = C::RPX, RPXL = C::RPXL;
   constexpr int RAW_BYTES = C::RAW_BYTES, RAW_PER_WAVE = C::RAW_PER_WAVE;
   constexpr int UQ = C::UQ, USTG = C::USTG, NUW = C::NUW, VROW = C::VROW, VSTG = C::VSTG;
   constexpr int OFF_U = C::OFF_U, OFF_V = C::OFF_V, OFF_RAW = C::OFF_RAW, BAR = C::BAR;
@@ -198,7 +203,13 @@
     unsigned roff[RAW_PER_WAVE];
 #pragma unroll
     for (int k = 0; k < RAW_PER_WAVE; ++k) {
-      const int idx = (wave + 8 * k) * 64 + lane;
+      const int idx = ((H16 && wave + 8 * k >= C::RAW_INSTR) ? wave + 8 * k - 8 : wave + 8 * k) * 64 + lane;
+      if (H16) {
+        const int c = idx / (RPXL / 4), r = idx - c * (RPXL / 4);
+        const int hy = r / (RW / 4), g = r - hy * (RW / 4);
+        roff[k] = (c < CK) ? 4u * (unsigned)(c * HpWp + hy * a.Wp + 4 * g) : 0u;
+        continue;
+      }
       const int c = idx / RPXL, r = idx - c * RPXL;
       const int hy = r / RW, hx = r - hy * RW;
       roff[k] = (c < CK && r < RPX) ? 4u * (unsigned)(c * HpWp + hy * a.Wp + hx) : 0u;
@@ -212,11 +223,12 @@
     };
     auto dma_raw = [&](const float* src, int rbuf, int k0, int k1) {
       if (WINO8_ABL & 4) return;
-      const unsigned dst = lds0 + OFF_RAW + rbuf * RAW_BYTES + wave * 256;
+      const unsigned dst = lds0 + OFF_RAW + rbuf * RAW_BYTES + wave * C::RAW_IBYTES;
 #pragma unroll
       for (int k = k0; k < k1; ++k)
         if (k < RAW_PER_WAVE) {
-          if (k < C::NRAW || wave + 8 * k < C::RAW_INSTR) glds4(src, roff[k], dst + k * 2048);
+          if (H16) glds16(src, roff[k], dst + ((wave + 8 * k < C::RAW_INSTR) ? k : k - 1) * (8 * C::RAW_IBYTES));
+          else if (k < C::NRAW || wave + 8 * k < C::RAW_INSTR) glds4(src, roff[k], dst + k * 2048);
         }
     };
 
@@ -265,8 +277,9 @@
       int base;
       f32x4 v00, v01, v10, v11;
     };
-    const int ipos = tid < NPOSI ? tid : NPOSI - 1;
-    const int ipos_b = (512 + (tid >> 2) < NPOSI) ? 512 + (tid >> 2) : NPOSI - 1;
+    auto halo_pos = [&](int p) { return (RW == HW) ? p : (p / HW) * RW + p % HW; };
+    const int ipos = halo_pos(tid < NPOSI ? tid : NPOSI - 1);
+    const int ipos_b = halo_pos((512 + (tid >> 2) < NPOSI) ? 512 + (tid >> 2) : NPOSI - 1);
     auto interp_tables = [&](int pp, Ip& ip) {
       const int hyi = pp / RW, hxi = pp - hyi * RW;
       const f32x4 rt = *reinterpret_cast<const f32x4*>(lds + OFF_TAB + hyi * 16);
@@ -447,9 +460,12 @@
           else if (sl == 7) tslice(8), tslice(9), islice(0);
           else if (sl == 8) tslice(10), tslice(11), islice(1);
           else if (sl == 9) islice(2), islice(3), imini(0);
-          else if (sl == 10) islice(4), islice(5), imini(1), dma_u(sd.u_src, sd.u_dst);
-          else if (sl == 11) imini(2);
-          if (RAWST && sl >= 6 && sl < 11) dma_raw(sd.raw_src, sd.raw_buf, 2 * (sl - 6), 2 * (sl - 6) + 2);
+          else if (sl == 10) {
+            islice(4), islice(5), imini(1);
+            if (K::UDMA) dma_u(sd.u_src, sd.u_dst);
+          } else if (sl == 11) imini(2);
+          if (RAWST && !H16 && sl >= 6 && sl < 11) dma_raw(sd.raw_src, sd.raw_buf, 2 * (sl - 6), 2 * (sl - 6) + 2);
+          if (RAWST && H16 && sl < 3) dma_raw(sd.raw_src, sd.raw_buf, sl, sl + 1);
           if (STST && sl == 9) dma_st(sd.st_src, sd.st_buf);
         }
         if (sl == BAR) {
@@ -664,8 +680,10 @@
     read_operand(I0{}, 0, 0, 0);
     read_operand(I0{}, 0, 1, 0);
 
-    auto chunk = [&](auto first_tag, auto k1_tag, auto k2_tag, auto k3_tag, const float* w_c, const float* nu, const float* nu2,
+    auto chunk = [&](auto first_tag, auto last_tag, auto k1_tag, auto k2_tag, auto k3_tag, const float* w_c, const float* nu, const float* nu2,
                      const float* nraw, const float* nst, int cc) {
+      constexpr bool LAST = H16 && decltype(last_tag)::value;
+      static_assert(!LAST || !decltype(first_tag)::value, "nch >= 2");
       constexpr int EPI = decltype(first_tag)::value ? NST : 0;
       constexpr bool K1 = UPS && decltype(k1_tag)::value, K2 = UPS && decltype(k2_tag)::value, K3 = UPS && decltype(k3_tag)::value;
       constexpr int NSW = C::NSW;
@@ -685,15 +703,17 @@
         stage(I3{}, first_tag, std::integral_constant<int, 2 * NUW>{}, Pre{}, S3k{}, Side{rnext, 3, 0, nu + 2 * (UQ / 4), 2, nullptr, 0, nullptr, 0, rcur, rcur});
       } else {
         using S0k = StageKind<false, false, K1 ? 1 : -1>;
-        using S1k = StageKind<!K2, K3, K2 ? 0 : -1>;
+        using S1k = StageKind<!K2, K3, K2 ? 0 : -1, !LAST>;
+        constexpr int DEFER = (H16 && decltype(first_tag)::value) ? NUW : 0;
         const int u0 = 2 * rcur, n0 = 2 * rnext;
-        stage(I0{}, first_tag, std::integral_constant<int, NUW + EPI>{}, Yes{}, S0k{},
+        stage(I0{}, first_tag, std::integral_constant<int, NUW + EPI + DEFER>{}, Yes{}, S0k{},
               Side{rcur, u0, u0 + 1, nu + (USTG / 4), n0 + 1, nullptr, 0, nullptr, 0, rnext, rnext});
-        stage(I1{}, first_tag, std::integral_constant<int, 2 * NUW + EPI + (K2 ? 0 : NRAW) + (K3 ? NSW : 0)>{}, Pre{}, S1k{},
+        stage(I1{}, first_tag, std::integral_constant<int, (LAST ? NUW : 2 * NUW) + (H16 ? 0 : EPI) + (K2 ? 0 : NRAW) + (K3 ? NSW : 0)>{}, Pre{}, S1k{},
               Side{rnext, u0 + 1, n0, nu2, u0, nraw, rcur, nst, rnext, rcur, rcur});
       }
     };
 
+    using H16t = std::bool_constant<H16 != 0>;
     int cc = 0;
     for (;;) {
       Tile Tn = decode(k + 1);
@@ -706,8 +726,9 @@
         constexpr int AH = (CT == 64) ? 1 : 2;
         const float* nraw = (c + AH < a.nch) ? raw_of(T, c + AH) : raw_of(Tn, c + AH - a.nch);
         if constexpr (!UPS) {
-          if (c == 0) chunk(Yes{}, No{}, No{}, No{}, w_c, nu, nu2, nraw, nullptr, cc);
-          else chunk(No{}, No{}, No{}, No{}, w_c, nu, nu2, nraw, nullptr, cc);
+          if (c == 0) chunk(Yes{}, No{}, No{}, No{}, No{}, w_c, nu, nu2, nraw, nullptr, cc);
+          else if (H16 && c + 1 == a.nch) chunk(No{}, H16t{}, No{}, No{}, No{}, w_c, nu, nu2, nraw, nullptr, cc);
+          else chunk(No{}, No{}, No{}, No{}, No{}, w_c, nu, nu2, nraw, nullptr, cc);
         } else {
           const int cu = a.C0 / CK;
           auto ups = [&](int j) { return c + j < a.nch && c + j >= cu; };
@@ -715,29 +736,32 @@
           const float* nst = T.s1u + (size_t)CK * (c + AH + 1) * hpwp_lo;
           if (c == 0) {
             write_tables(T);
-            chunk(Yes{}, No{}, No{}, No{}, w_c, nu, nu2, nraw, nst, cc);
+            chunk(Yes{}, No{}, No{}, No{}, No{}, w_c, nu, nu2, nraw, nst, cc);
           } else if constexpr (CT == 64) {
-            if (!k1 && !k2) chunk(No{}, No{}, No{}, No{}, w_c, nu, nu2, nraw, nst, cc);
-            else if (!k1 && k2) chunk(No{}, No{}, Yes{}, No{}, w_c, nu, nu2, nraw, nst, cc);
-            else if (k1 && k2) chunk(No{}, Yes{}, Yes{}, No{}, w_c, nu, nu2, nraw, nst, cc);
-            else chunk(No{}, Yes{}, No{}, No{}, w_c, nu, nu2, nraw, nst, cc);
+            if (!k1 && !k2) chunk(No{}, No{}, No{}, No{}, No{}, w_c, nu, nu2, nraw, nst, cc);
+            else if (!k1 && k2) chunk(No{}, No{}, No{}, Yes{}, No{}, w_c, nu, nu2, nraw, nst, cc);
+            else if (k1 && k2) chunk(No{}, No{}, Yes{}, Yes{}, No{}, w_c, nu, nu2, nraw, nst, cc);
+            else chunk(No{}, No{}, Yes{}, No{}, No{}, w_c, nu, nu2, nraw, nst, cc);
           } else {
-            if (!k1 && !k2 && !k3) chunk(No{}, No{}, No{}, No{}, w_c, nu, nu2, nraw, nst, cc);
-            else if (!k1 && !k2) chunk(No{}, No{}, No{}, Yes{}, w_c, nu, nu2, nraw, nst, cc);
-            else if (!k1 && k3) chunk(No{}, No{}, Yes{}, Yes{}, w_c, nu, nu2, nraw, nst, cc);
-            else if (k1 && k2 && k3) chunk(No{}, Yes{}, Yes{}, Yes{}, w_c, nu, nu2, nraw, nst, cc);
-            else if (k1 && k2) chunk(No{}, Yes{}, Yes{}, No{}, w_c, nu, nu2, nraw, nst, cc);
-            else if (k1) chunk(No{}, Yes{}, No{}, No{}, w_c, nu, nu2, nraw, nst, cc);
-            else chunk(No{}, No{}, Yes{}, No{}, w_c, nu, nu2, nraw, nst, cc);
+            if (H16 && c + 1 == a.nch) chunk(No{}, H16t{}, No{}, No{}, No{}, w_c, nu, nu2, nraw, nst, cc);
+            else if (!k1 && !k2 && !k3) chunk(No{}, No{}, No{}, No{}, No{}, w_c, nu, nu2, nraw, nst, cc);
+            else if (!k1 && !k2) chunk(No{}, No{}, No{}, No{}, Yes{}, w_c, nu, nu2, nraw, nst, cc);
+            else if (!k1 && k3) chunk(No{}, No{}, No{}, Yes{}, Yes{}, w_c, nu, nu2, nraw, nst, cc);
+            else if (k1 && k2 && k3) chunk(No{}, No{}, Yes{}, Yes{}, Yes{}, w_c, nu, nu2, nraw, nst, cc);
+            else if (k1 && k2) chunk(No{}, No{}, Yes{}, Yes{}, No{}, w_c, nu, nu2, nraw, nst, cc);
+            else if (k1) chunk(No{}, No{}, Yes{}, No{}, No{}, w_c, nu, nu2, nraw, nst, cc);
+            else chunk(No{}, No{}, No{}, Yes{}, No{}, w_c, nu, nu2, nraw, nst, cc);
           }
         }
       }
       const int rl = (cc - 1) & 1;
       const int bufA = (CT == 64) ? ((sw < 2) ? OFF_U + 3 * USTG + sw * 8192 : OFF_V + VSTG + (sw - 2) * 8192) : OFF_V + VSTG + sw * 8192;
       const int bufB = (CT == 64) ? ((sw < 2) ? OFF_RAW + rl * RAW_BYTES + sw * 8192 : C::LDS_USED + (sw - 2) * 8192)
+                       : H16      ? ((sw < 2) ? OFF_U + (2 * rl + 1 - sw) * USTG : C::LDS_USED + (sw - 2) * 8192)
                                   : ((sw < 1) ? OFF_U + (2 * rl + 1) * USTG : C::LDS_USED + (sw - 1) * 8192);
-      static_assert(C::LDS_USED + (CT == 64 ? 2 : 3) * 8192 <= LDS_REQ8 && 2 * 8192 <= RAW_BYTES && USTG >= 8192, "exchange buffers");
+      static_assert(C::LDS_USED + ((CT == 64 || H16) ? 2 : 3) * 8192 <= LDS_REQ8 && 2 * 8192 <= RAW_BYTES && USTG >= 8192, "exchange buffers");
       epilogue(T, P == 1 ? bufA : bufB, P == 1 ? bufB : bufA, bufB);
+      if (H16) dma_u(Tn.w + 4 * (UQ / 4), 2 * rl);
       if (!more) break;
       T = Tn;
       ++k;
@@ -811,9 +835,9 @@
 }
 size_t conv3x3_wino8_ksplit_bytes_per_image() { return (size_t)32 * 8 * 2048 * sizeof(float); }
 
-template <int CT, bool FUSE_OUTC, bool RES, bool UPS = false, bool KSPLIT = false>
+template <int CT, bool FUSE_OUTC, bool RES, bool UPS = false, bool KSPLIT = false, int H16 = 0>
 static int launch_wino8(WinoArgs a, hipStream_t s) {
-  using C = Cfg8<CT>;
+  using C = Cfg8<CT, H16>;
   static_assert(C::LDS_USED <= LDS_REQ8 && C::LDS_USED_UPS <= LDS_REQ8, "LDS budget");
   a.nct = a.Cout / CT;
   a.nch = (a.C0 + a.C1) / C::CK;
@@ -828,7 +852,7 @@
   if (dev >= 0 && dev < 64) {
     hipError_t e = hipSuccess;
     std::call_once(attr_once[dev], [&] {
-      e = hipFuncSetAttribute(reinterpret_cast<const void*>(&conv3x3_wino8_f32_kernel<CT, FUSE_OUTC, RES, UPS, KSPLIT>), hipFuncAttributeMaxDynamicSharedMemorySize, LDS_REQ8);
+      e = hipFuncSetAttribute(reinterpret_cast<const void*>(&conv3x3_wino8_f32_kernel<CT, FUSE_OUTC, RES, UPS, KSPLIT, H16>), hipFuncAttributeMaxDynamicSharedMemorySize, LDS_REQ8);
     });
     PNPX_HIP(e);
   }
@@ -837,7 +861,7 @@
   long long grid = 256;
   if (grid >= ntiles) grid = ntiles;
   else if ((grid / 8) % vnct != 0 && grid >= 8LL * vnct) grid -= grid % (8 * vnct);
-  hipLaunchKernelGGL((conv3x3_wino8_f32_kernel<CT, FUSE_OUTC, RES, UPS, KSPLIT>), dim3((unsigned)grid), dim3(512), LDS_REQ8, s, a);
+  hipLaunchKernelGGL((conv3x3_wino8_f32_kernel<CT, FUSE_OUTC, RES, UPS, KSPLIT, H16>), dim3((unsigned)grid), dim3(512), LDS_REQ8, s, a);
   PNPX_LAUNCH_CHECK();
   if (KSPLIT) {
     hipLaunchKernelGGL(wino8_ksplit_finish_kernel, dim3((unsigned)(nreg * a.nct)), dim3(512), 0, s, a);
@@ -846,8 +870,13 @@
   return PNPX_OK;
 }
 
+template <bool FUSE_OUTC, bool RES, bool UPS = false>
+static int launch_wino8_ct32(const WinoArgs& a, hipStream_t s, int halo16) {
+  return halo16 ? launch_wino8<32, FUSE_OUTC, RES, UPS, false, 1>(a, s) : launch_wino8<32, FUSE_OUTC, RES, UPS, false, 0>(a, s);
+}
+
 int launch_conv3x3_wino8_outc(const float* u, const float* bias, const float* in0, int cin, const float* outc_w, const float* outc_b,
-                              const float* x_img, float* img, float* img_pre, int B, int H, int W, hipStream_t s) {
+                              const float* x_img, float* img, float* img_pre, int B, int H, int W, hipStream_t s, int halo16) {
   if (wino8_ct(cin, 0, 32, H, W) != 32) {
     set_error("conv3x3_wino8_outc: unsupported geometry (%d -> 32 channels, %d x %d)", cin, H, W);
     return PNPX_ERR_SHAPE;
@@ -872,7 +901,7 @@
   a.C1 = 0;
   a.Cout = 32;
   a.slope = 0.2f;
-  return launch_wino8<32, true, false>(a, s);
+  return launch_wino8_ct32<true, false>(a, s, halo16);
 }
 
 bool conv3x3_wino8_ups_ok(int C0, int C1, int cout, int H, int W) {
@@ -884,7 +913,7 @@
 }
 
 int launch_conv3x3_wino8_ups(const float* u, const float* bias, int cout, const float* in0, int C0, const float* in1_lowres, int C1,
-                             float* out, int B, int H, int W, hipStream_t s, float slope) {
+                             float* out, int B, int H, int W, hipStream_t s, float slope, int halo16) {
   if (!conv3x3_wino8_ups_ok(C0, C1, cout, H, W)) {
     set_error("conv3x3_wino8_ups: unsupported geometry (%d + up(%d) -> %d channels, %d x %d)", C0, C1, cout, H, W);
     return PNPX_ERR_SHAPE;
@@ -908,11 +937,11 @@
   a.ups_w = W / 2;
   a.ups_sy = (H > 1) ? (float)(H / 2 - 1) / (float)(H - 1) : 0.f;
   a.ups_sx = (W > 1) ? (float)(W / 2 - 1) / (float)(W - 1) : 0.f;
-  return wino8_ct(C0, C1, cout, H, W) == 64 ? launch_wino8<64, false, false, true>(a, s) : launch_wino8<32, false, false, true>(a, s);
+  return wino8_ct(C0, C1, cout, H, W) == 64 ? launch_wino8<64, false, false, true>(a, s) : launch_wino8_ct32<false, false, true>(a, s, halo16);
 }
 
 int launch_conv3x3_wino8_grad(const float* u, const float* zero_bias, int cout, const float* gin, int cin, float* gout, const float* dmask,
-                              float mask_slope, int B, int H, int W, hipStream_t s) {
+                              float mask_slope, int B, int H, int W, hipStream_t s, int halo16) {
   const int ct = wino8_ct(cin, 0, cout, H, W);
   if (!ct) {
     set_error("conv3x3_wino8_grad: unsupported geometry (%d -> %d channels, %d x %d)", cin, cout, H, W);
@@ -936,13 +965,13 @@
   a.C1 = 0;
   a.Cout = cout;
   a.slope = 1.0f;
-  if (dmask) return ct == 64 ? launch_wino8<64, false, true>(a, s) : launch_wino8<32, false, true>(a, s);
-  return ct == 64 ? launch_wino8<64, false, false>(a, s) : launch_wino8<32, false, false>(a, s);
+  if (dmask) return ct == 64 ? launch_wino8<64, false, true>(a, s) : launch_wino8_ct32<false, true>(a, s, halo16);
+  return ct == 64 ? launch_wino8<64, false, false>(a, s) : launch_wino8_ct32<false, false>(a, s, halo16);
 }
 
 int launch_conv3x3_wino8(const float* u, const float* bias, int cout, const float* in0, int C0, const float* in1, int C1,
                          float* out, int B, int H, int W, hipStream_t s, float slope, const float* res, float* pool_out, float* ks_part,
-                         int ks_rule) {
+                         int ks_rule, int halo16) {
   const int ct = wino8_ct(C0, C1, cout, H, W);
   if (!ct) {
     set_error("conv3x3_wino8: unsupported geometry (%d + %d -> %d channels, %d x %d)", C0, C1, cout, H, W);
@@ -965,14 +994,14 @@
   a.C1 = C1;
   a.Cout = cout;
   a.slope = slope;
-  if (res) return ct == 64 ? launch_wino8<64, false, true>(a, s) : launch_wino8<32, false, true>(a, s);
+  if (res) return ct == 64 ? launch_wino8<64, false, true>(a, s) : launch_wino8_ct32<false, true>(a, s, halo16);
   const int g = ks_part ? conv3x3_wino8_ksplit(C0, C1, cout, H, W, ks_rule) : 1;
   if (g > 1) {
     a.ksplit = g;
     a.part = ks_part;
     return launch_wino8<64, false, false, false, true>(a, s);
   }
-  return ct == 64 ? launch_wino8<64, false, false>(a, s) : launch_wino8<32, false, false>(a, s);
+  return ct == 64 ? launch_wino8<64, false, false>(a, s) : launch_wino8_ct32<false, false>(a, s, halo16);
 }
 
 }
diff --git a/tfpnp_amd/csrc/drunet_f32.hip b/tfpnp_amd/csrc/drunet_f32.hip
--- a/tfpnp_amd/csrc/drunet_f32.hip
+++ b/tfpnp_amd/csrc/drunet_f32.hip
@@ -385,7 +385,7 @@
     if (u && ctx->opt_fp32_winograd && conv3x3_wino_ok(Lc.cin, 0, Lc.cout, h, w))
     {
       if (ctx->opt_fp32_wino8 && conv3x3_wino8_ok(Lc.cin, 0, Lc.cout, h, w))
-        return launch_conv3x3_wino8(u, Lc.b, Lc.cout, in, Lc.cin, nullptr, 0, outp, B, h, w, s, slope, res, nullptr);
+        return launch_conv3x3_wino8(u, Lc.b, Lc.cout, in, Lc.cin, nullptr, 0, outp, B, h, w, s, slope, res, nullptr, nullptr, 1, ctx->opt_fp32_halo16);
       return launch_conv3x3_wino(u, Lc.b, Lc.cout, in, Lc.cin, nullptr, 0, outp, B, h, w, s, slope, res, nullptr);
     }
     return launch_conv3x3_act(Lc, in, Lc.cin, nullptr, 0, outp, B, h, w, slope, res, s);
@@ -500,8 +500,8 @@
     if (kind == 3 || kind == 4) return launch_conv1x1_act(Lc, in, outp, B, h, w, 1.f, res, s);
     const float* u = N.f32_wino_bwd[li];
     if (u && ctx->opt_fp32_winograd && ctx->opt_fp32_wino8 && conv3x3_wino8_ok(Lc.cin, 0, Lc.cout, h, w)) {
-      if (dmask) return launch_conv3x3_wino8_grad(u, Lc.b, Lc.cout, in, Lc.cin, outp, dmask, 0.f, B, h, w, s);
-      return launch_conv3x3_wino8(u, Lc.b, Lc.cout, in, Lc.cin, nullptr, 0, outp, B, h, w, s, 1.f, res, nullptr);
+      if (dmask) return launch_conv3x3_wino8_grad(u, Lc.b, Lc.cout, in, Lc.cin, outp, dmask, 0.f, B, h, w, s, ctx->opt_fp32_halo16);
+      return launch_conv3x3_wino8(u, Lc.b, Lc.cout, in, Lc.cin, nullptr, 0, outp, B, h, w, s, 1.f, res, nullptr, nullptr, 1, ctx->opt_fp32_halo16);
     }
     if (dmask) return launch_conv3x3_grad(Lc, in, outp, dmask, B, h, w, s, nullptr, 0.f);
     return launch_conv3x3_act(Lc, in, Lc.cin, nullptr, 0, outp, B, h, w, 1.f, res, s);
diff --git a/tfpnp_amd/csrc/unet.hip b/tfpnp_amd/csrc/unet.hip
--- a/tfpnp_amd/csrc/unet.hip
+++ b/tfpnp_amd/csrc/unet.hip
@@ -571,7 +571,7 @@
       if (w8) {
         const bool ks = ks_on(L.cout, o.H, o.W);
         PNPX_TRY(launch_conv3x3_wino8(ctx->conv_wino_u[li], L.b, L.cout, fptr(i0), i0.C, i1 ? fptr(*i1) : nullptr, C1, fptr(o), B, o.H, o.W, s, 0.2f,
-                                      nullptr, pooled ? fptr(*pooled) : nullptr, ks ? ks_part0 : nullptr, ctx->opt_ksplit_rule));
+                                      nullptr, pooled ? fptr(*pooled) : nullptr, ks ? ks_part0 : nullptr, ctx->opt_ksplit_rule, ctx->opt_fp32_halo16));
       }
       else
         PNPX_TRY(launch_conv3x3_wino(ctx->conv_wino_u[li], L.b, L.cout, fptr(i0), i0.C, i1 ? fptr(*i1) : nullptr, C1, fptr(o), B, o.H, o.W, s, 0.2f,
@@ -619,7 +619,7 @@
             return launch_conv3x3_wino8(ctx->conv_wino_u[li], L.b, L.cout, fptr(i) + (size_t)lo * i.C * padded_h(i.H) * padded_w(i.W), i.C, nullptr, 0,
                                         fptr(o) + (size_t)lo * o.C * padded_h(o.H) * padded_w(o.W), hi - lo, o.H, o.W, st, 0.2f, nullptr, nullptr,
                                         ks_on(o.C, o.H, o.W) ? ks_part0 + (size_t)lo * (P.ks_part_per_image / sizeof(float)) : nullptr,
-                                        ctx->opt_ksplit_rule);
+                                        ctx->opt_ksplit_rule, ctx->opt_fp32_halo16);
           };
           PNPX_TRY(slice(12, P.p[4], P.a[4]));
           PNPX_TRY(slice(13, P.a[4], P.b[4]));
@@ -658,7 +658,7 @@
     auto entry = [&](const Act& ta) -> int {
       if (!ups_fused) return conv(li0, P.x[l], &P.u[l], ta);
       const ConvLayer& L = ctx->conv[li0];
-      PNPX_TRY(launch_conv3x3_wino8_ups(ctx->conv_wino_u[li0], L.b, L.cout, fptr(P.x[l]), P.x[l].C, fptr(*below), below->C, fptr(ta), B, 2 * h, 2 * w, s));
+      PNPX_TRY(launch_conv3x3_wino8_ups(ctx->conv_wino_u[li0], L.b, L.cout, fptr(P.x[l]), P.x[l].C, fptr(*below), below->C, fptr(ta), B, 2 * h, 2 * w, s, 0.2f, ctx->opt_fp32_halo16));
       return rec.mark("conv3x3_wino", 2.0 * 9.0 * L.cin * L.cout * (double)(2 * h) * (2 * w) * B);
     };
     const bool fuse_outc = l == 0 && !keep_all && ctx->opt_fuse_outc && ctx->opt_fp32_winograd && ctx->conv_wino_u[26] &&
@@ -667,8 +667,12 @@
       PNPX_TRY(entry(P.da[0]));
       PNPX_TRY(conv(25, P.da[0], nullptr, P.db[0]));
       const bool w8 = ((ctx->opt_fp32_wino8 >> 26) & 1) && conv3x3_wino8_ok(ctx->conv[26].cin, 0, ctx->conv[26].cout, H, W);
-      PNPX_TRY((w8 ? launch_conv3x3_wino8_outc : launch_conv3x3_wino_outc)(ctx->conv_wino_u[26], ctx->conv[26].b, fptr(P.db[0]), ctx->conv[26].cin,
-                                                                          ctx->outc_w, ctx->outc_b, x, out, out_pre, B, H, W, s));
+      if (w8)
+        PNPX_TRY(launch_conv3x3_wino8_outc(ctx->conv_wino_u[26], ctx->conv[26].b, fptr(P.db[0]), ctx->conv[26].cin, ctx->outc_w, ctx->outc_b, x, out, out_pre,
+                                           B, H, W, s, ctx->opt_fp32_halo16));
+      else
+        PNPX_TRY(launch_conv3x3_wino_outc(ctx->conv_wino_u[26], ctx->conv[26].b, fptr(P.db[0]), ctx->conv[26].cin, ctx->outc_w, ctx->outc_b, x, out, out_pre,
+                                          B, H, W, s));
       return rec.mark("conv3x3_wino", 2.0 * 9.0 * ctx->conv[26].cin * ctx->conv[26].cout * (double)H * W * B);
     }
     PNPX_TRY(entry(P.da[l]));
diff --git a/tfpnp_amd/csrc/unet_bwd.hip b/tfpnp_amd/csrc/unet_bwd.hip
--- a/tfpnp_amd/csrc/unet_bwd.hip
+++ b/tfpnp_amd/csrc/unet_bwd.hip
@@ -602,7 +602,7 @@
     const char* dmh = nullptr;
     if (!hs && ctx->opt_fp32_winograd && ((ctx->opt_fp32_wino8 >> li) & 1) && ctx->conv_wino_u_bwd[li] && gout.C == ctx->conv_bwd[li].cout &&
         conv3x3_wino8_ok(gin.C, 0, gout.C, gout.H, gout.W))
-      return launch_conv3x3_wino8_grad(ctx->conv_wino_u_bwd[li], ctx->zero_bias, gout.C, gp(gin), gin.C, gp(gout), dm, 0.2f, B, gout.H, gout.W, s);
+      return launch_conv3x3_wino8_grad(ctx->conv_wino_u_bwd[li], ctx->zero_bias, gout.C, gp(gin), gin.C, gp(gout), dm, 0.2f, B, gout.H, gout.W, s, ctx->opt_fp32_halo16);
     return launch_conv3x3_grad(ctx->conv_bwd[li], gp(gin), gp(gout), dm, B, gout.H, gout.W, s, dmh);
   };
 
```
